# cloudinary/fuif

Measured on AMD Instinct MI355X. Metric: Mpixels/s decode (4K Squeeze+YCoCg), higher is better.
Workload: dtype int32; 1 GPU; C2: batch of 1024 3840x2160 8-bit photographic YCoCg+Squeeze lossless per GPU; images_per_gpu=1024, distinct_images=16, group_index=FGIX trailer behind each stream: one wavefront per channel group, status_ok_and_replicas_agree=True

## Files before the change

fuif_amd/__init__.py:

```python
import ctypes as C
import os
import subprocess

import numpy as np

_HERE = os.path.dirname(os.path.abspath(__file__))
_LIB_PATH = os.environ.get("FUIF_AMD_LIB") or os.path.join(_HERE, "libfuifgpu.so")
_SOURCES = ["plan.cpp", "index.cpp", "writer.cpp", "maniac_decode.hip", "maniac_encode.hip", "transforms.hip", "capi.hip"]
_lib = None


class FuifGpuError(RuntimeError):
    def __init__(self, code, msg):
        super().__init__("fuifgpu error %d: %s" % (code, msg))
        self.code = code


HIPCC_FLAGS = ["--offload-arch=gfx950", "-O3", "-std=c++17", "-ffp-contract=off", "-Wno-unused-value"]


def build(force=False, verbose=False):
    srcs = [os.path.join(_HERE, "csrc", s) for s in _SOURCES]
    deps = srcs + [os.path.join(_HERE, "csrc", h) for h in ("fuifgpu_internal.h", "maniac_decode.h", "maniac_encode.h", "transforms.h", "squeeze_arith.h")]
    deps.append(os.path.join(_HERE, "..", "include", "fuifgpu.h"))
# ... 20 lines not shown
    return out


class ImageInfo(C.Structure):
    _fields_ = [("w", C.c_int32), ("h", C.c_int32), ("bit_depth", C.c_int32), ("maxval", C.c_int32),
                ("nb_channels", C.c_int32), ("colormodel", C.c_int32), ("max_properties", C.c_int32),
                ("nb_frames", C.c_int32), ("nb_transforms", C.c_int32), ("nb_coded_channels", C.c_int32),
                ("nb_output_channels", C.c_int32), ("nb_ops", C.c_int32), ("responsive_offsets", C.c_int32 * 5),
                ("data_start", C.c_int32), ("coef_elems", C.c_int64), ("out_elems", C.c_int64),
                ("tmp_elems", C.c_int64), ("signature", C.c_uint64)]


class ChannelDesc(C.Structure):
    _fields_ = [("w", C.c_int32), ("h", C.c_int32), ("hshift", C.c_int32), ("vshift", C.c_int32),
                ("hcshift", C.c_int32), ("vcshift", C.c_int32), ("component", C.c_int32), ("reserved", C.c_int32),
                ("offset", C.c_int64)]


class EncodeOptions(C.Structure):
    _fields_ = [("struct_size", C.c_uint32), ("ycocg", C.c_int32), ("squeeze", C.c_int32), ("max_properties", C.c_int32), ("tree_mode", C.c_int32),
                ("max_tree_nodes", C.c_int32), ("emit_index", C.c_int32), ("split_bits", C.c_int32), ("gpu_forward", C.c_int32), ("gpu_entropy", C.c_int32)]


class LossyOptions(C.Structure):
    _fields_ = [("struct_size", C.c_uint32), ("quality", C.c_float), ("chroma_quality", C.c_float)]


class PaletteOptions(C.Structure):
    _fields_ = [("struct_size", C.c_uint32), ("palette_colors", C.c_int32), ("compact_post_percent", C.c_float), ("compact_pre_percent", C.c_float)]


def make_palette_options(palette_colors=0, compact_post=0.0, compact_pre=0.0):
    if not palette_colors and not compact_post and not compact_pre:
        return None
    return PaletteOptions(C.sizeof(PaletteOptions), int(palette_colors), float(compact_post), float(compact_pre))


def make_lossy_options(quality=None, chroma_quality=None):
    return LossyOptions(C.sizeof(LossyOptions), 100.0 if quality is None else float(quality), 101.0 if chroma_quality is None else float(chroma_quality))


def make_encode_options(*fields):
    return EncodeOptions(C.sizeof(EncodeOptions), *fields)


ABI_SYMBOLS = [
    "fuifgpu_strerror", "fuifgpu_last_error", "fuifgpu_abi_version", "fuifgpu_plan_create", "fuifgpu_plan_destroy",
    "fuifgpu_plan_info", "fuifgpu_plan_coded_channel", "fuifgpu_plan_output_channel", "fuifgpu_plan_transform",
    "fuifgpu_build_chance_table", "fuifgpu_batch_create", "fuifgpu_batch_create_sibling", "fuifgpu_dev_mem_info", "fuifgpu_encode_images", "fuifgpu_batch_destroy", "fuifgpu_batch_upload",
    "fuifgpu_batch_decode", "fuifgpu_batch_undo_transforms", "fuifgpu_batch_sync", "fuifgpu_batch_status",
    "fuifgpu_batch_create_streaming", "fuifgpu_batch_undo_transforms_to", "fuifgpu_batch_channel_meta", "fuifgpu_batch_coef_ptr", "fuifgpu_batch_out_ptr", "fuifgpu_batch_download_coef",
    "fuifgpu_batch_download_out", "fuifgpu_batch_last_timing", "fuifgpu_batch_profile", "fuifgpu_batch_tile_log", "fuifgpu_batch_sched_stats", "fuifgpu_inv_hsqueeze", "fuifgpu_inv_vsqueeze",
    "fuifgpu_inv_ycocg", "fuifgpu_inv_ycbcr", "fuifgpu_inv_quantize", "fuifgpu_idct8x8", "fuifgpu_upsample", "fuifgpu_inv_palette", "fuifgpu_inv_approximate", "fuifgpu_inv_match", "fuifgpu_fwd_ycocg", "fuifgpu_fwd_hsqueeze", "fuifgpu_fwd_vsqueeze", "fuifgpu_fwd_quantize", "fuifgpu_encode_image", "fuifgpu_encode_channels", "fuifgpu_free_blob",
    "fuifgpu_index_parse", "fuifgpu_index_append", "fuifgpu_batch_group_index", "fuifgpu_batch_set_group_parallel",
    "fuifgpu_plan_packed_bytes", "fuifgpu_batch_pack_out", "fuifgpu_batch_download_packed",
    "fuifgpu_dev_alloc", "fuifgpu_dev_free", "fuifgpu_dev_upload", "fuifgpu_dev_download",
    "fuifgpu_encode_image_lossy", "fuifgpu_encode_images_lossy", "fuifgpu_quantization_constant",
    "fuifgpu_encode_images_device", "fuifgpu_channel_stats", "fuifgpu_encode_plane_traffic",
    "fuifgpu_encode_image_ex", "fuifgpu_encode_images_ex", "fuifgpu_fwd_palette",
    "fuifgpu_plane_checksums", "fuifgpu_device_count", "fuifgpu_set_device", "fuifgpu_get_device", "fuifgpu_batch_device", "fuifgpu_peer_copy", "fuifgpu_batch_set_in_flight",
]


def _preload_hip_runtime():
    import importlib.util
    try:
        spec = importlib.util.find_spec("torch")
    except (ImportError, ValueError):
        spec = None
    if spec is None or not spec.submodule_search_locations:
        return
    cand = os.path.join(list(spec.submodule_search_locations)[0], "lib", "libamdhip64.so")
    if os.path.exists(cand):
        try:
            global _hip_runtime
            _hip_runtime = C.CDLL(cand, mode=C.RTLD_GLOBAL)
        except OSError:
            pass


_hip_runtime = None


def hip_runtime():
    lib()
    return _hip_runtime if _hip_runtime is not None else C.CDLL("libamdhip64.so")


def lib():
    global _lib
    if _lib is not None:
        return _lib
    if not os.path.exists(_LIB_PATH):
        raise ImportError("fuif_amd/libfuifgpu.so is missing: run `python -c 'import __graft_entry__ as g; g.build()'` "
                          "(hipcc --offload-arch=gfx950). There is no CPU fallback.")
    _preload_hip_runtime()
    L = C.CDLL(_LIB_PATH)
    vp, i32p, u8p = C.c_void_p, C.POINTER(C.c_int32), C.POINTER(C.c_uint8)
    L.fuifgpu_strerror.restype = C.c_char_p; L.fuifgpu_strerror.argtypes = [C.c_int]
    L.fuifgpu_last_error.restype = C.c_char_p; L.fuifgpu_last_error.argtypes = []
    L.fuifgpu_abi_version.restype = C.c_int
    L.fuifgpu_plan_create.argtypes = [C.c_char_p, C.c_size_t, C.POINTER(vp)]
    L.fuifgpu_plan_destroy.argtypes = [vp]; L.fuifgpu_plan_destroy.restype = None
    L.fuifgpu_plan_info.argtypes = [vp, C.POINTER(ImageInfo)]
    L.fuifgpu_plan_coded_channel.argtypes = [vp, C.c_int, C.POINTER(ChannelDesc)]
    L.fuifgpu_plan_output_channel.argtypes = [vp, C.c_int, C.POINTER(ChannelDesc)]
    L.fuifgpu_plan_transform.argtypes = [vp, C.c_int, i32p, vp, C.c_int, i32p]
    L.fuifgpu_build_chance_table.argtypes = [vp, C.c_uint32, C.c_int]; L.fuifgpu_build_chance_table.restype = None
    L.fuifgpu_batch_create.argtypes = [vp, C.c_int, C.c_size_t, vp, vp, C.c_int, C.POINTER(vp)]
    L.fuifgpu_batch_create_sibling.argtypes = [vp, C.c_size_t, C.POINTER(vp)]
    L.fuifgpu_batch_destroy.argtypes = [vp]; L.fuifgpu_batch_destroy.restype = None
    L.fuifgpu_batch_upload.argtypes = [vp, C.POINTER(C.c_char_p), C.POINTER(C.c_size_t), C.c_int, C.c_int, vp]
    L.fuifgpu_batch_decode.argtypes = [vp, vp]
    L.fuifgpu_batch_undo_transforms.argtypes = [vp, vp]
    L.fuifgpu_batch_create_streaming.argtypes = [vp, C.c_int, C.c_size_t, C.c_int, C.POINTER(vp)]
    L.fuifgpu_batch_undo_transforms_to.argtypes = [vp, C.c_int, C.c_int, vp, vp]
    L.fuifgpu_batch_sync.argtypes = [vp, vp]
    L.fuifgpu_batch_status.argtypes = [vp, vp, vp]
    L.fuifgpu_batch_channel_meta.argtypes = [vp, C.c_int, vp]
    L.fuifgpu_batch_coef_ptr.argtypes = [vp, C.c_int]; L.fuifgpu_batch_coef_ptr.restype = vp
    L.fuifgpu_batch_out_ptr.argtypes = [vp, C.c_int]; L.fuifgpu_batch_out_ptr.restype = vp
    L.fuifgpu_batch_download_coef.argtypes = [vp, C.c_int, vp, vp]
    L.fuifgpu_batch_download_out.argtypes = [vp, C.c_int, vp, vp]
    L.fuifgpu_device_count.argtypes = [C.POINTER(C.c_int)]
    L.fuifgpu_set_device.argtypes = [C.c_int]
    L.fuifgpu_get_device.argtypes = [C.POINTER(C.c_int)]
    L.fuifgpu_batch_device.argtypes = [vp, C.POINTER(C.c_int)]
    L.fuifgpu_peer_copy.argtypes = [vp, C.c_int, vp, C.c_int, C.c_size_t, vp]
    L.fuifgpu_plane_checksums.argtypes = [vp, C.c_int64, C.c_int64, C.c_int, vp, vp]
    L.fuifgpu_batch_last_timing.argtypes = [vp, C.POINTER(C.c_float), C.POINTER(C.c_float)]
    L.fuifgpu_batch_profile.argtypes = [vp, vp]
    L.fuifgpu_batch_tile_log.argtypes = [vp, vp, C.c_int, C.POINTER(C.c_int)]
    L.fuifgpu_batch_sched_stats.argtypes = [vp, vp]
    L.fuifgpu_inv_hsqueeze.argtypes = [vp, C.c_int, vp, C.c_int, C.c_int, vp, C.c_int, C.c_int64, C.c_int64, C.c_int64, vp]
    L.fuifgpu_inv_vsqueeze.argtypes = [vp, C.c_int, vp, C.c_int, C.c_int, vp, C.c_int, C.c_int64, C.c_int64, C.c_int64, vp]
    L.fuifgpu_inv_ycocg.argtypes = [vp, vp, vp, C.c_int, C.c_int, C.c_int, C.c_int, C.c_int, C.c_int, vp]
    L.fuifgpu_inv_ycbcr.argtypes = [vp, vp, vp, C.c_int, C.c_int, C.c_int, C.c_int, C.c_int, C.c_int, C.c_int, vp]
    L.fuifgpu_inv_quantize.argtypes = [vp, C.c_int64, C.c_int, vp]
    L.fuifgpu_idct8x8.argtypes = [C.POINTER(vp), C.c_int, C.c_int, vp, C.c_int, vp]
    L.fuifgpu_upsample.argtypes = [vp, C.c_int, C.c_int, C.c_int, C.c_int, vp, vp]
    L.fuifgpu_inv_palette.argtypes = [vp, C.c_int, C.c_int, vp, C.c_int, vp, vp]
    L.fuifgpu_inv_approximate.argtypes = [vp, vp, C.c_int64, C.c_int, vp]
    L.fuifgpu_inv_match.argtypes = [vp, C.c_int, C.c_int, C.POINTER(vp), C.c_int, C.c_int, C.c_int, C.c_int, C.c_int, vp]
    L.fuifgpu_fwd_ycocg.argtypes = [vp, vp, vp, C.c_int, C.c_int, vp]
    L.fuifgpu_fwd_hsqueeze.argtypes = [vp, C.c_int, C.c_int, vp, vp, vp]
    L.fuifgpu_fwd_vsqueeze.argtypes = [vp, C.c_int, C.c_int, vp, vp, vp]
    L.fuifgpu_dev_alloc.argtypes = [C.c_size_t]; L.fuifgpu_dev_alloc.restype = vp
    L.fuifgpu_dev_free.argtypes = [vp]; L.fuifgpu_dev_free.restype = None
    L.fuifgpu_dev_upload.argtypes = [vp, vp, C.c_size_t]
    L.fuifgpu_dev_download.argtypes = [vp, vp, C.c_size_t]
    L.fuifgpu_fwd_quantize.argtypes = [vp, C.c_int64, C.c_int, vp, vp]
    L.fuifgpu_encode_image_lossy.argtypes = [vp, C.c_int, C.c_int, C.c_int, C.c_int, C.POINTER(EncodeOptions), C.POINTER(LossyOptions), C.POINTER(vp), C.POINTER(C.c_size_t)]
    L.fuifgpu_encode_images_lossy.argtypes = [C.POINTER(vp), C.c_int, C.c_int, C.c_int, C.c_int, C.c_int, C.POINTER(EncodeOptions), C.POINTER(LossyOptions), C.POINTER(vp), C.POINTER(C.c_size_t)]
    L.fuifgpu_encode_images_device.argtypes = [C.POINTER(vp), C.c_int, C.c_int, C.c_int, C.c_int, C.c_int, C.POINTER(EncodeOptions), C.POINTER(LossyOptions), C.POINTER(vp), C.POINTER(C.c_size_t)]
    L.fuifgpu_channel_stats.argtypes = [vp, C.c_int64, vp, vp]
    L.fuifgpu_encode_image_ex.argtypes = [vp, C.c_int, C.c_int, C.c_int, C.c_int, C.POINTER(EncodeOptions), C.POINTER(LossyOptions), C.POINTER(PaletteOptions), C.POINTER(vp), C.POINTER(C.c_size_t)]
    L.fuifgpu_encode_images_ex.argtypes = [C.POINTER(vp), C.c_int, C.c_int, C.c_int, C.c_int, C.c_int, C.c_int, C.POINTER(EncodeOptions), C.POINTER(LossyOptions), C.POINTER(PaletteOptions), C.POINTER(vp), C.POINTER(C.c_size_t)]
    L.fuifgpu_fwd_palette.argtypes = [C.POINTER(vp), C.c_int, C.c_int64, C.c_int, vp, vp, C.POINTER(C.c_int), vp]
    L.fuifgpu_encode_plane_traffic.argtypes = [C.POINTER(C.c_uint64), C.POINTER(C.c_uint64)]
    L.fuifgpu_quantization_constant.argtypes = [C.c_float, C.c_float, C.c_int, C.c_int, C.c_int]
    L.fuifgpu_encode_image.argtypes = [vp, C.c_int, C.c_int, C.c_int, C.c_int, C.POINTER(EncodeOptions), C.POINTER(vp), C.POINTER(C.c_size_t)]
    L.fuifgpu_encode_images.argtypes = [C.POINTER(vp), C.c_int, C.c_int, C.c_int, C.c_int, C.c_int, C.POINTER(EncodeOptions), C.POINTER(vp), C.POINTER(C.c_size_t)]
    L.fuifgpu_free_blob.argtypes = [vp]; L.fuifgpu_free_blob.restype = None
    L.fuifgpu_index_parse.argtypes = [C.c_char_p, C.c_size_t, vp, vp, C.c_int, C.POINTER(C.c_int)]
    L.fuifgpu_index_append.argtypes = [C.c_char_p, C.c_size_t, vp, vp, C.c_int, C.POINTER(vp), C.POINTER(C.c_size_t)]
    L.fuifgpu_batch_group_index.argtypes = [vp, C.c_int, vp, vp, C.c_int, C.POINTER(C.c_int)]
    L.fuifgpu_batch_set_group_parallel.argtypes = [vp, C.c_int]
    L.fuifgpu_batch_set_in_flight.argtypes = [vp, C.c_int]
    L.fuifgpu_plan_packed_bytes.argtypes = [vp, C.c_int]; L.fuifgpu_plan_packed_bytes.restype = C.c_size_t
    L.fuifgpu_batch_pack_out.argtypes = [vp, C.c_int, C.c_int, C.c_int, vp, vp]
    L.fuifgpu_batch_download_packed.argtypes = [vp, C.c_int, C.c_int, vp, vp]
    _lib = L
    return L


def _check(code):
    if code != 0:
        L = lib()
        msg = L.fuifgpu_strerror(code).decode()
        last = L.fuifgpu_last_error().decode()
        raise FuifGpuError(code, msg + (" (" + last + ")" if last else ""))


class Plan:

    def __init__(self, blob):
        L = lib()
        self._h = C.c_void_p()
        _check(L.fuifgpu_plan_create(bytes(blob[:65536]) if len(blob) > 65536 else bytes(blob), min(len(blob), 65536), C.byref(self._h)))
        self.info = ImageInfo()
        _check(L.fuifgpu_plan_info(self._h, C.byref(self.info)))

    def __del__(self):
        if getattr(self, "_h", None) and _lib is not None:
            _lib.fuifgpu_plan_destroy(self._h)
            self._h = None

    def _channels(self, fn, n):
        out = []
        for i in range(n):
            d = ChannelDesc()
            _check(fn(self._h, i, C.byref(d)))
            out.append({k: int(getattr(d, k)) for k, _ in ChannelDesc._fields_ if k != "reserved"})
        return out

    @property
    def coded_channels(self):
        return self._channels(lib().fuifgpu_plan_coded_channel, self.info.nb_coded_channels)

    @property
    def output_channels(self):
        return self._channels(lib().fuifgpu_plan_output_channel, self.info.nb_output_channels)

    @property
    def transforms(self):
        out = []
        for i in range(self.info.nb_transforms):
# ... 247 lines not shown
        ptrs = [int(p) if p else 0 for p in planes]
        if w is None or h is None or nch is None:
            raise FuifGpuError(4, "encode_images_device: w, h and nch go with a list of device pointers")
    n = len(ptrs)
    opt = make_encode_options(int(ycocg), int(squeeze), max_properties, tree_mode, max_tree_nodes, int(index), int(split_bits), 1, 1)
    lossy = None if quality is None and chroma_quality is None else C.byref(make_lossy_options(quality, chroma_quality))
    arr = (C.c_void_p * max(n, 1))(*ptrs)
    outs = (C.c_void_p * max(n, 1))()
    sizes = (C.c_size_t * max(n, 1))()
    pal = make_palette_options(palette_colors, compact_post, compact_pre)
    if pal is not None:
        _check(lib().fuifgpu_encode_images_ex(arr, 1, n, int(w), int(h), int(nch), bit_depth, C.byref(opt), lossy, C.byref(pal), outs, sizes))
    else:
        _check(lib().fuifgpu_encode_images_device(arr, n, int(w), int(h), int(nch), bit_depth, C.byref(opt), lossy, outs, sizes))
    blobs = []
    for k in range(n):
        blobs.append(C.string_at(outs[k], sizes[k]))
        lib().fuifgpu_free_blob(C.c_void_p(outs[k]))
    return blobs


def channel_stats(plane_device_ptr, n_samples, stats_device_ptr, stream=None):
    _check(lib().fuifgpu_channel_stats(plane_device_ptr, int(n_samples), stats_device_ptr, stream))


def encode_plane_traffic():
    a, b = C.c_uint64(0), C.c_uint64(0)
    _check(lib().fuifgpu_encode_plane_traffic(C.byref(a), C.byref(b)))
    return int(a.value), int(b.value)


def quantization_constant(quality, chroma_quality=None, squeeze=True, chroma_table=False, shift=0):
    q = lib().fuifgpu_quantization_constant(float(quality), 101.0 if chroma_quality is None else float(chroma_quality), int(bool(squeeze)), int(bool(chroma_table)), int(shift))
    if q < 1:
        _check(-q)
    return q


def fwd_quantize(plane_device_ptr, n_samples, q, minmax_device_ptr=None, stream=None):
    _check(lib().fuifgpu_fwd_quantize(plane_device_ptr, int(n_samples), int(q), minmax_device_ptr, stream))


def fwd_palette(plane_device_ptrs, n_samples, max_colors, index_device_ptr, stream=None):
    nb = len(plane_device_ptrs)
    ptrs = (C.c_void_p * max(nb, 1))(*[int(p) if p else 0 for p in plane_device_ptrs])
    pal = np.zeros((max(nb, 1), max(int(max_colors), 1)), dtype=np.int32)
    count = C.c_int(0)
    _check(lib().fuifgpu_fwd_palette(ptrs, nb, int(n_samples), int(max_colors), index_device_ptr, pal.ctypes.data, C.byref(count), stream))
    if count.value < 0:
        return None
    return np.ascontiguousarray(pal[:nb, :count.value])


def index_parse(blob):
    fc, st, n = np.zeros(4096, np.int32), np.zeros(4096, np.uint32), C.c_int(0)
    _check(lib().fuifgpu_index_parse(blob, len(blob), fc.ctypes.data, st.ctypes.data, 4096, C.byref(n)))
    return [(int(fc[i]), int(st[i])) for i in range(min(n.value, 4096))]


def index_append(blob, groups):
    fc = np.array([g[0] for g in groups], np.int32)
    st = np.array([g[1] for g in groups], np.uint32)
    out, n = C.c_void_p(), C.c_size_t(0)
    _check(lib().fuifgpu_index_append(blob, len(blob), fc.ctypes.data, st.ctypes.data, len(groups), C.byref(out), C.byref(n)))
    res = C.string_at(out.value, n.value)
    lib().fuifgpu_free_blob(out)
    return res


def add_group_index(blobs, hbm_budget_bytes=200 << 30):
    out = list(blobs)
    todo = []
    for i, b in enumerate(blobs):
        try:
            if not index_parse(b):
                Plan(b)
                todo.append(i)
        except FuifGpuError:
            pass
    for sig, (plan, idx) in group_by_signature([blobs[i] for i in todo]).items():
        idx = [todo[k] for k in idx]
        per = 2 * plan.info.coef_elems + 19 * (1 << 20) + max(len(blobs[i]) for i in idx)
        chunk = max(1, min(len(idx), int(hbm_budget_bytes // per), 65535))
        for c0 in range(0, len(idx), chunk):
            part = idx[c0:c0 + chunk]
            sub = [blobs[i] for i in part]
            batch = Batch(plan, len(sub), sum(len(b) for b in sub) + 4096 * len(sub), streaming=True, tmp_images=1)
            try:
                batch.upload(sub)
                batch.decode()
                batch.sync()
                st, _ = batch.status()
                for k, i in enumerate(part):
                    if st[k] == 0:
                        out[i] = index_append(blobs[i], batch.group_index(k))
            finally:
                batch.close()
    return out


def group_by_signature(blobs):
    groups = {}
    for i, b in enumerate(blobs):
        p = Plan(b)
        sig = int(p.info.signature)
        if sig not in groups:
            groups[sig] = (p, [])
        groups[sig][1].append(i)
    return groups

# ... 28 lines not shown
```

fuif_amd/csrc/capi.hip:

```cpp
#include <hip/hip_runtime.h>

#include <algorithm>
#include <cstdio>
#include <cstring>
#include <string>
#include <vector>

#include "../../include/fuifgpu.h"
#include "fuifgpu_internal.h"
#include "maniac_decode.h"
#include "transforms.h"

using namespace fuifgpu;

struct fuifgpu_plan {
    Plan plan;
};

struct fuifgpu_batch {
    Plan plan;
    int device = 0;
    int n = 0;
    int n_loaded = 0;
    uint8_t *d_blobs = nullptr;
    size_t blob_cap = 0;
    StreamJob *d_jobs = nullptr;
    ChannelGeom *d_geom = nullptr;
    ChannelMeta *d_meta = nullptr;
    int32_t *d_status = nullptr;
    uint32_t *d_consumed = nullptr;
    uint16_t *d_tables = nullptr;
    uint8_t *d_scratch = nullptr;
    size_t scratch_stride = 0, bfs_off = 0, leaves_off = 0, stack_off = 0, queue_off = 0, subtree_off = 0;
    int scratch_waves = 0;
    int max_waves[3] = {0, 0, 0};
    int in_flight = 1;
    int n_waves = 0, cfg = 1;
    bool group_parallel = true;
    Tile *d_tiles = nullptr;
    int tiles_cap = 0, n_tiles = 0;
    uint32_t *d_progress = nullptr, *d_group_start = nullptr;
    uint32_t *d_sched = nullptr, *d_layout = nullptr;
    size_t sched_words = 0, layout_cap = 0;
    int sched = 0, n_queues = 1, waves_per_simd = 4;
    uint8_t *d_ctx = nullptr;
    size_t ctx_bytes = 0;
    uint32_t ctx_units_per_queue = 0;
    int max_nodes = kMaxNodes;
    coef_t *d_coef = nullptr;
    int32_t *d_out = nullptr, *d_tmp = nullptr;
    int32_t *d_coef32 = nullptr;
    bool own_coef = false, own_out = false;
    int tmp_images = 0;
    PlaneRef *d_list = nullptr;
    int64_t *d_widen = nullptr;
    unsigned long long *d_prof = nullptr, *d_tile_log = nullptr;
    int tile_log_cap = 0; bool want_tile_log = false;
    uint8_t *h_blobs = nullptr;
    std::vector<StreamJob> jobs;
    hipEvent_t ev[4] = {nullptr, nullptr, nullptr, nullptr};
    bool decode_timed = false, transform_timed = false;
    bool no_out = false;
    std::vector<char> undone;
    bool coef_consumed = false;
    fuifgpu_batch *share = nullptr;
    std::vector<fuifgpu_batch *> siblings;
    bool orphan = false;
};
static inline const fuifgpu_batch *launch_res(const fuifgpu_batch *b) { return b->share ? b->share : b; }

static thread_local std::string g_last_error;

static int hip_fail(hipError_t e, const char *what) {
    g_last_error = std::string(what) + ": " + hipGetErrorString(e);
    return FUIFGPU_E_HIP;
}
static int fail_msg(int code, const char *what) {
    g_last_error = what;
    return code;
}
#define HIPCHK(call)                                      \
    do {                                                  \
        hipError_t e__ = (call);                          \
        if (e__ != hipSuccess) return hip_fail(e__, #call); \
    } while (0)

template <typename T, typename N>
static int grow(T *&ptr, N &cap, N need, size_t unit = sizeof(T), bool sync_first = false) {
    if (need <= cap) return FUIFGPU_OK;
    if (sync_first) HIPCHK(hipDeviceSynchronize());
    hipFree(ptr); ptr = nullptr; cap = 0;
    HIPCHK(hipMalloc((void **)&ptr, unit * (size_t)need));
    cap = need;
    return FUIFGPU_OK;
// ... 211 lines not shown
    }
    *out = p;
    return FUIFGPU_OK;
}
void fuifgpu_plan_destroy(fuifgpu_plan *plan) { delete plan; }

int fuifgpu_plan_info(const fuifgpu_plan *plan, fuifgpu_image_info *info) {
    if (!plan || !info) return FUIFGPU_E_ARG;
    const Plan &p = plan->plan;
    memset(info, 0, sizeof(*info));
    info->w = p.w; info->h = p.h; info->bit_depth = p.bit_depth; info->maxval = p.maxval; info->nb_channels = p.nb_channels;
    info->colormodel = p.colormodel; info->max_properties = p.max_properties; info->nb_frames = p.nb_frames;
    info->nb_transforms = (int)p.transforms.size(); info->nb_coded_channels = (int)p.coded.size();
    info->nb_output_channels = (int)p.outputs.size(); info->nb_ops = (int)p.ops.size();
    for (int s = 0; s < 5; s++) info->responsive_offsets[s] = p.responsive_offsets[s];
    info->data_start = (int)p.data_start;
    info->coef_elems = p.coef_elems; info->out_elems = p.out_elems; info->tmp_elems = p.tmp_elems;
    info->signature = p.signature;
    return FUIFGPU_OK;
}
int fuifgpu_plan_coded_channel(const fuifgpu_plan *plan, int index, fuifgpu_channel_desc *d) {
    if (!plan || !d || index < 0 || index >= (int)plan->plan.coded.size()) return FUIFGPU_E_ARG;
    const ChannelGeom &g = plan->plan.coded[index];
    d->w = g.w; d->h = g.h; d->hshift = g.hshift; d->vshift = g.vshift; d->hcshift = g.hcshift; d->vcshift = g.vcshift;
    d->component = g.component; d->reserved = 0; d->offset = g.coef_off;
    return FUIFGPU_OK;
}
int fuifgpu_plan_output_channel(const fuifgpu_plan *plan, int index, fuifgpu_channel_desc *d) {
    if (!plan || !d || index < 0 || index >= (int)plan->plan.outputs.size()) return FUIFGPU_E_ARG;
    const OutputChannel &o = plan->plan.outputs[index];
    d->w = o.plane.w; d->h = o.plane.h; d->hshift = o.hshift; d->vshift = o.vshift; d->hcshift = o.hcshift; d->vcshift = o.vcshift;
    d->component = o.component; d->reserved = 0; d->offset = o.plane.off;
    return FUIFGPU_OK;
}
int fuifgpu_plan_transform(const fuifgpu_plan *plan, int index, int32_t *id, int32_t *params_out, int cap, int32_t *nparams) {
    if (!plan || index < 0 || index >= (int)plan->plan.transforms.size()) return FUIFGPU_E_ARG;
    const TransformDesc &t = plan->plan.transforms[index];
    if (id) *id = t.id;
    if (nparams) *nparams = (int)t.params.size();
    if (params_out) for (int i = 0; i < (int)t.params.size() && i < cap; i++) params_out[i] = t.params[i];
    return FUIFGPU_OK;
}

void fuifgpu_batch_destroy(fuifgpu_batch *b) {
    if (!b) return;
    ON_BATCH_DEVICE(b);
    for (fuifgpu_batch *s : b->siblings) { s->share = nullptr; s->orphan = true; s->n_loaded = 0; s->d_coef = nullptr; s->d_out = nullptr; }
    if (b->share) {
        auto &v = b->share->siblings;
        v.erase(std::remove(v.begin(), v.end(), b), v.end());
    }
    hipFree(b->d_blobs); hipFree(b->d_jobs); hipFree(b->d_geom); hipFree(b->d_meta); hipFree(b->d_status); hipFree(b->d_consumed);
    hipFree(b->d_tables); hipFree(b->d_scratch); hipFree(b->d_tmp); hipFree(b->d_coef32); hipFree(b->d_list); hipFree(b->d_widen); hipFree(b->d_prof); hipFree(b->d_tile_log);
    hipFree(b->d_tiles); hipFree(b->d_progress); hipFree(b->d_group_start); hipFree(b->d_sched); hipFree(b->d_layout); hipFree(b->d_ctx);
    if (b->own_coef) hipFree(b->d_coef);
    if (b->own_out) hipFree(b->d_out);
    if (b->h_blobs) hipHostFree(b->h_blobs);
    for (int i = 0; i < 4; i++) if (b->ev[i]) hipEventDestroy(b->ev[i]);
    delete b;
}

static int32_t *const kNoOutSlab = reinterpret_cast<int32_t *>(~(uintptr_t)0);
static int batch_create_impl(const Plan &plan_in, int n_images, size_t blob_capacity_bytes, coef_t *coef_ext, int32_t *out_ext,
                             int tmp_images, fuifgpu_batch *share, fuifgpu_batch **out) {
    if (!out || n_images < 1 || n_images > 65535) return FUIFGPU_E_ARG;
    *out = nullptr;
    int ndev = 0;
    if (hipGetDeviceCount(&ndev) != hipSuccess || ndev < 1) {
        g_last_error = "no HIP device visible: libfuifgpu has no CPU fallback";
        return FUIFGPU_E_HIP;
    }
    fuifgpu_batch *b = new fuifgpu_batch();
    if (share) b->device = share->device;
    else if (hipGetDevice(&b->device) != hipSuccess) b->device = 0;
    b->plan = plan_in;
    b->n = n_images;
    b->share = share;
    const Plan &p = b->plan;
    const int nch = (int)p.coded.size();
    b->blob_cap = blob_capacity_bytes + (size_t)n_images * 32 + 1024;
#define CHK(call)                                                        \
    do {                                                                 \
        hipError_t e__ = (call);                                         \
        if (e__ != hipSuccess) { int rc = hip_fail(e__, #call); fuifgpu_batch_destroy(b); return rc; } \
    } while (0)
    CHK(hipMalloc((void **)&b->d_blobs, b->blob_cap));
    CHK(hipMalloc((void **)&b->d_jobs, sizeof(StreamJob) * n_images));
    CHK(hipMalloc((void **)&b->d_geom, sizeof(ChannelGeom) * std::max(nch, 1)));
    CHK(hipMemcpy(b->d_geom, p.coded.data(), sizeof(ChannelGeom) * nch, hipMemcpyHostToDevice));
    CHK(hipMalloc((void **)&b->d_meta, sizeof(ChannelMeta) * (size_t)n_images * std::max(nch, 1)));
    CHK(hipMalloc((void **)&b->d_status, sizeof(int32_t) * n_images));
    CHK(hipMalloc((void **)&b->d_consumed, sizeof(uint32_t) * n_images));
    {
        std::vector<uint16_t> tables(16384);
        build_chance_table(tables.data(), 0xFFFFFFFFu / 19, 2);
        build_chance_table(tables.data() + 8192, 0x0d000000u, 6);
        CHK(hipMalloc((void **)&b->d_tables, tables.size() * 2));
        CHK(hipMemcpy(b->d_tables, tables.data(), tables.size() * 2, hipMemcpyHostToDevice));
    }
    b->scratch_stride = maniac_scratch_bytes(b->max_nodes, &b->bfs_off, &b->leaves_off, &b->stack_off, &b->queue_off, &b->subtree_off);
    b->max_waves[0] = maniac_max_waves(0);
    b->max_waves[1] = maniac_max_waves(1, &b->waves_per_simd);
    b->max_waves[2] = maniac_max_waves(2);
    if (const char *e = getenv("FUIFGPU_IN_FLIGHT")) b->in_flight = std::max(1, atoi(e));
    if (b->max_waves[0] < 1 || b->max_waves[1] < 1 || b->max_waves[2] < 1) { g_last_error = "cannot query the device occupancy of the entropy kernel"; fuifgpu_batch_destroy(b); return FUIFGPU_E_HIP; }
    CHK(hipMalloc((void **)&b->d_progress, sizeof(uint32_t) * (size_t)n_images * std::max(nch, 1)));
    CHK(hipMalloc((void **)&b->d_group_start, sizeof(uint32_t) * (size_t)n_images * std::max(nch, 1)));
    if (coef_ext) b->d_coef = coef_ext;
    else { CHK(hipMalloc((void **)&b->d_coef, sizeof(coef_t) * (size_t)std::max<int64_t>(p.coef_elems, 1) * n_images)); b->own_coef = true; }
    if (out_ext == kNoOutSlab) { b->d_out = nullptr; b->no_out = true; }
    else if (out_ext) b->d_out = out_ext;
    else { CHK(hipMalloc((void **)&b->d_out, sizeof(int32_t) * (size_t)std::max<int64_t>(p.out_elems, 1) * n_images)); b->own_out = true; }
    if (tmp_images <= 0) {
        int64_t per = (std::max<int64_t>(p.tmp_elems, 1) + std::max<int64_t>(p.coef_elems, 1)) * 4;
        tmp_images = (int)std::max<int64_t>(1, std::min<int64_t>(n_images, (12LL << 30) / per));
    }
    b->tmp_images = std::min(tmp_images, n_images);
    if (!share) {
        CHK(hipMalloc((void **)&b->d_tmp, sizeof(int32_t) * (size_t)std::max<int64_t>(p.tmp_elems, 1) * b->tmp_images));
        CHK(hipMalloc((void **)&b->d_coef32, sizeof(int32_t) * (size_t)std::max<int64_t>(p.coef_elems, 1) * b->tmp_images));
    }
    if (!p.idct_src.empty()) {
        CHK(hipMalloc((void **)&b->d_list, sizeof(PlaneRef) * p.idct_src.size()));
        CHK(hipMemcpy(b->d_list, p.idct_src.data(), sizeof(PlaneRef) * p.idct_src.size(), hipMemcpyHostToDevice));
    }
    if (!p.widen.empty()) {
        CHK(hipMalloc((void **)&b->d_widen, sizeof(int64_t) * p.widen.size()));
        CHK(hipMemcpy(b->d_widen, p.widen.data(), sizeof(int64_t) * p.widen.size(), hipMemcpyHostToDevice));
    }
    CHK(hipMalloc((void **)&b->d_prof, sizeof(unsigned long long) * 8 * n_images));
    CHK(hipMemset(b->d_prof, 0, sizeof(unsigned long long) * 8 * n_images));
    for (int i = 0; i < 4; i++) CHK(hipEventCreate(&b->ev[i]));
#undef CHK
    *out = b;
    return FUIFGPU_OK;
}

int fuifgpu_batch_create(const fuifgpu_plan *plan, int n_images, size_t blob_capacity_bytes, int16_t *coef_ext, int32_t *out_ext,
                         int tmp_images, fuifgpu_batch **out) {
    if (!plan) return FUIFGPU_E_ARG;
    return batch_create_impl(plan->plan, n_images, blob_capacity_bytes, coef_ext, out_ext, tmp_images, nullptr, out);
}

static size_t ctx_arena_budget(const fuifgpu_batch *b, size_t images) {
    size_t per_image = 16u << 20;
    if (const char *e = getenv("FUIFGPU_CTX_MB")) per_image = (size_t)std::max(1, atoi(e)) << 20;
    if (const char *e = getenv("FUIFGPU_CTX_KB")) per_image = (size_t)std::max(0, atoi(e)) << 10;
    size_t want = per_image * images, free_b = 0, total_b = 0;
    if (hipMemGetInfo(&free_b, &total_b) == hipSuccess) want = std::min(want, (free_b + b->ctx_bytes) / 2);
    return want / 256 * 256;
}
static uint32_t ctx_units_per_queue(size_t arena_bytes, int n_queues) {
    const size_t q = (size_t)std::max(n_queues, 1);
    return (uint32_t)std::min(arena_bytes / q / 256, (size_t)0xFFFFFF00u / q);
}
static int freeze_launch_resources(fuifgpu_batch *b) {
    const int64_t cap = std::max(std::max(b->max_waves[0], b->max_waves[1]), b->max_waves[2]);
    const int waves = (int)std::max<int64_t>(1, std::min<int64_t>(cap, (int64_t)b->n * std::max<int64_t>((int64_t)b->plan.coded.size(), 1)));
    OKCHK(grow(b->d_scratch, b->scratch_waves, waves, b->scratch_stride, true));
    return grow(b->d_ctx, b->ctx_bytes, ctx_arena_budget(b, (size_t)b->n), 1, true);
}

int fuifgpu_batch_create_streaming(const fuifgpu_plan *plan, int n_images, size_t blob_capacity_bytes, int tmp_images, fuifgpu_batch **out) {
    if (!plan) return FUIFGPU_E_ARG;
    return batch_create_impl(plan->plan, n_images, blob_capacity_bytes, nullptr, kNoOutSlab, tmp_images, nullptr, out);
}

int fuifgpu_batch_create_sibling(fuifgpu_batch *primary, size_t blob_capacity_bytes, fuifgpu_batch **out) {
    if (!primary || primary->share || primary->no_out) return FUIFGPU_E_ARG;
    ON_BATCH_DEVICE(primary);
    if (primary->siblings.empty()) OKCHK(freeze_launch_resources(primary));
    const int rc = batch_create_impl(primary->plan, primary->n, blob_capacity_bytes, primary->d_coef, primary->d_out, primary->tmp_images, primary, out);
    if (rc == FUIFGPU_OK) primary->siblings.push_back(*out);
    return rc;
}

static int stage_streams(fuifgpu_batch *b, const uint8_t *const *blobs, const size_t *sizes, int n_images, int preview, hipStream_t st,
                         std::vector<std::vector<GroupEntry>> &groups, std::vector<int> &group_of) {
    b->jobs.assign(n_images, StreamJob{});
    size_t off = 0;
    Plan tmp;
    std::vector<std::pair<const uint8_t *, int>> seen;
    const int nch = (int)b->plan.coded.size();
    group_of.assign(n_images, -1);
    HIPCHK(hipStreamSynchronize(st));
    for (int i = 0; i < n_images; i++) {
        if (sizes[i] > 0xFFFFFFF0ull) return FUIFGPU_E_ARG;
        int src = -1;
        for (auto &sp : seen) if (sp.first == blobs[i] && b->jobs[sp.second].blob_size == sizes[i]) { src = sp.second; break; }
        size_t padded = (sizes[i] + 15) / 16 * 16 + 16;
        if (off + padded + 256 > b->blob_cap) { g_last_error = "blob capacity exceeded"; return FUIFGPU_E_NOMEM; }
        StreamJob &j = b->jobs[i];
        if (src < 0) {
            int r = parse_and_plan(blobs[i], sizes[i], tmp);
            if (r != FUIFGPU_OK) { g_last_error = tmp.message; return r; }
            if (tmp.signature != b->plan.signature) { g_last_error = "image " + std::to_string(i) + " has a different geometry/transform chain"; return FUIFGPU_E_MISMATCH; }
            std::vector<GroupEntry> idx;
            if (b->group_parallel) parse_index_trailer(blobs[i], sizes[i], tmp.data_start, nch, idx, nullptr);
            if (idx.empty()) idx.push_back(GroupEntry{(uint32_t)tmp.data_start, 0});
            groups.push_back(std::move(idx));
            group_of[i] = (int)groups.size() - 1;
            HIPCHK(hipMemsetAsync(b->d_blobs + off + (padded - 32), 0, 32, st));
            HIPCHK(hipMemcpyAsync(b->d_blobs + off, blobs[i], sizes[i], hipMemcpyHostToDevice, st));
            j.data_start = (uint32_t)tmp.data_start;
            j.limit = preview >= 0 ? (uint32_t)tmp.responsive_offsets[preview] : 0u;
            seen.emplace_back(blobs[i], i);
        } else {
            HIPCHK(hipMemcpyAsync(b->d_blobs + off, b->d_blobs + b->jobs[src].blob_off, padded, hipMemcpyDeviceToDevice, st));
            j.data_start = b->jobs[src].data_start;
            j.limit = b->jobs[src].limit;
            group_of[i] = group_of[src];
        }
        j.blob_off = off; j.blob_size = (uint32_t)sizes[i];
        j.flags = 0;
        off += padded;
    }
    HIPCHK(hipMemcpyAsync(b->d_jobs, b->jobs.data(), sizeof(StreamJob) * n_images, hipMemcpyHostToDevice, st));
    return FUIFGPU_OK;
}

struct WorkList {
    int cfg = 1, n_waves = 0, sched = 0, n_queues = 1;
    std::vector<Tile> tiles;
    std::vector<uint32_t> layout;
};
static WorkList plan_work_list(const Plan &plan, const std::vector<std::vector<GroupEntry>> &groups, const std::vector<int> &group_of, const size_t *sizes,
                               const int *max_waves, int waves_per_simd, int in_flight, bool group_order) {
    WorkList wl;
    const int n_images = (int)group_of.size(), nch = (int)plan.coded.size();
    size_t total_tiles = 0, deepest = 0;
    for (int i = 0; i < n_images; i++) total_tiles += groups[group_of[i]].size();
    for (auto &g : groups) deepest = std::max(deepest, g.size());
    const int wide_cfg = in_flight > 1 ? 0 : 2;
    const bool dense = (int64_t)total_tiles > max_waves[wide_cfg];
    wl.cfg = dense ? 1 : wide_cfg;
    wl.n_waves = (int)std::max<int64_t>(1, std::min<int64_t>((int64_t)total_tiles, max_waves[wl.cfg]));
    std::vector<char> suspendable(groups.size(), 0);
    for (size_t gi = 0; gi < groups.size(); gi++) {
        const std::vector<GroupEntry> &g = groups[gi];
        bool ok = g.size() > 1;
        for (size_t k = 0; k < g.size() && ok; k++) {
            const int first = k == 0 ? 0 : g[k].first_channel, last = k + 1 < g.size() ? g[k + 1].first_channel - 1 : nch - 1;
            int nonempty = 0;
            for (int c = first; c <= last; c++) nonempty += (int64_t)plan.coded[c].w * plan.coded[c].h > 0 ? 1 : 0;
            ok = nonempty <= 1;
        }
        suspendable[gi] = ok ? 1 : 0;
    }
    int64_t image_samples = 0;
    for (int c = 0; c < nch; c++) image_samples += (int64_t)plan.coded[c].w * plan.coded[c].h;
    auto push_tile = [&](int i, size_t k) {
        const std::vector<GroupEntry> &g = groups[group_of[i]];
        if (k >= g.size()) return;
        Tile t;
        t.image = (uint32_t)i;
        t.start = g[k].start;
        t.first_channel = k == 0 ? 0 : g[k].first_channel;
        t.last_channel = k + 1 < g.size() ? g[k + 1].first_channel - 1 : nch - 1;
        t.end = k + 1 < g.size() ? g[k + 1].start : 0u;
        t.flags = suspendable[group_of[i]] ? kTileSuspendable : 0u;
        int64_t mine = 0;
        for (int c = (int)t.first_channel; c <= (int)t.last_channel; c++) mine += (int64_t)plan.coded[c].w * plan.coded[c].h;
        uint32_t cls = 15;
        if (mine > 0) { cls = 0; while (cls < 15 && (mine << (cls + 1)) <= image_samples) cls++; }
        t.flags |= cls << kTileSizeClassShift;
        wl.tiles.push_back(t);
    };
    wl.sched = dense && (int64_t)total_tiles > wl.n_waves && !group_order ? 1 : 0;
    if (!wl.sched) {
        for (size_t k = 0; k < deepest; k++)
            for (int i = 0; i < n_images; i++) push_tile(i, k);
        return wl;
    }
    const int waves_per_cu = (int)kSimdsPerCu * std::max(1, waves_per_simd);
    const int Q = wl.n_queues = std::max(1, std::min(n_images, wl.n_waves / waves_per_cu));
    const QueueLayout L = queue_layout(Q, n_images);
    wl.layout.resize(L.words);
    uint32_t *qib = wl.layout.data() + L.q_img_begin, *qim = wl.layout.data() + L.q_images, *itb = wl.layout.data() + L.img_tile_begin;
    std::vector<int> by_size(n_images);
    for (int i = 0; i < n_images; i++) by_size[i] = i;
    std::stable_sort(by_size.begin(), by_size.end(), [&](int x, int y) { return sizes[x] > sizes[y]; });
    std::vector<std::vector<uint32_t>> dealt(Q);
    for (int k = 0; k < n_images; k++) {
        const int round = k / Q, at = k % Q;
        dealt[(round & 1) ? Q - 1 - at : at].push_back((uint32_t)by_size[k]);
    }
    uint32_t pos = 0;
    for (int q = 0; q < Q; q++) {
        qib[q] = pos;
        std::sort(dealt[q].begin(), dealt[q].end());
        for (uint32_t i : dealt[q]) qim[pos++] = i;
    }
    qib[Q] = pos;
    for (int i = 0; i < n_images; i++) {
        itb[i] = (uint32_t)wl.tiles.size();
        for (size_t k = 0; k < groups[group_of[i]].size(); k++) push_tile(i, k);
    }
    itb[n_images] = (uint32_t)wl.tiles.size();
    return wl;
}

static int reserve_launch_buffers(fuifgpu_batch *b, int n_images, size_t layout_words) {
    OKCHK(grow(b->d_sched, b->sched_words, sched_layout(n_images, b->n_queues, b->sched ? b->n_tiles : 0)));
    OKCHK(grow(b->d_layout, b->layout_cap, layout_words));
    OKCHK(grow(b->d_tiles, b->tiles_cap, b->n_tiles));
    if (b->sched && !b->share) {
        const size_t images_per_queue = ((size_t)n_images + b->n_queues - 1) / b->n_queues;
        size_t arena = ctx_arena_budget(b, images_per_queue * (size_t)b->n_queues);
        if (!b->siblings.empty()) arena = std::min(arena, b->ctx_bytes);
        b->ctx_units_per_queue = ctx_units_per_queue(arena, b->n_queues);
        OKCHK(grow(b->d_ctx, b->ctx_bytes, (size_t)b->ctx_units_per_queue * 256 * (size_t)b->n_queues));
    }
    if (b->share) {
        if (b->n_waves > b->share->scratch_waves) { g_last_error = "sibling batch: more wavefronts than the primary's decoder scratch was sized for"; return FUIFGPU_E_ARG; }
        return FUIFGPU_OK;
    }
    if (b->n_waves > b->scratch_waves && !b->siblings.empty()) { g_last_error = "primary batch with siblings: decoder scratch cannot grow (internal sizing error)"; return FUIFGPU_E_ARG; }
    return grow(b->d_scratch, b->scratch_waves, b->n_waves, b->scratch_stride);
}

int fuifgpu_batch_upload(fuifgpu_batch *b, const uint8_t *const *blobs, const size_t *sizes, int n_images, int preview, void *stream) {
    ON_BATCH_DEVICE(b);
    if (!b || !blobs || !sizes || n_images < 1 || n_images > b->n || preview < -1 || preview > 4) return FUIFGPU_E_ARG;
    if (b->orphan) { g_last_error = "sibling batch: its primary has been destroyed"; return FUIFGPU_E_ARG; }
    hipStream_t st = (hipStream_t)stream;
    std::vector<std::vector<GroupEntry>> groups;
    std::vector<int> group_of;
    OKCHK(stage_streams(b, blobs, sizes, n_images, preview, st, groups, group_of));
    const char *ord = getenv("FUIFGPU_TILE_ORDER");
    const WorkList wl = plan_work_list(b->plan, groups, group_of, sizes, b->max_waves, b->waves_per_simd, b->in_flight, ord && !strcmp(ord, "group"));
    b->cfg = wl.cfg; b->n_waves = wl.n_waves; b->sched = wl.sched; b->n_queues = wl.n_queues; b->n_tiles = (int)wl.tiles.size();
    OKCHK(reserve_launch_buffers(b, n_images, wl.layout.size()));
    if (!wl.layout.empty()) HIPCHK(hipMemcpyAsync(b->d_layout, wl.layout.data(), wl.layout.size() * 4, hipMemcpyHostToDevice, st));
    if (b->n_tiles) HIPCHK(hipMemcpyAsync(b->d_tiles, wl.tiles.data(), sizeof(Tile) * (size_t)b->n_tiles, hipMemcpyHostToDevice, st));
    HIPCHK(hipStreamSynchronize(st));
    b->n_loaded = n_images;
    if (getenv("FUIFGPU_VERBOSE"))
        fprintf(stderr, "fuifgpu: %d images, %d tiles, %s configuration, %d persistent wavefronts (%d per SIMD), %d queues, context scheduler %s\n", n_images, b->n_tiles,
                b->cfg == 1 ? "dense" : b->cfg == 2 ? "wide" : "wide (two batches in flight)", b->n_waves, b->waves_per_simd, b->n_queues, b->sched ? "on" : "off");
    return FUIFGPU_OK;
}

int fuifgpu_batch_decode(fuifgpu_batch *b, void *stream) {
    ON_BATCH_DEVICE(b);
    if (!b || b->n_loaded < 1) return FUIFGPU_E_ARG;
    hipStream_t st = (hipStream_t)stream;
    const int nch = (int)b->plan.coded.size();
    HIPCHK(hipMemsetAsync(b->d_meta, 0, sizeof(ChannelMeta) * (size_t)b->n_loaded * std::max(nch, 1), st));
    HIPCHK(hipMemsetAsync(b->d_progress, 0, sizeof(uint32_t) * (size_t)b->n_loaded * std::max(nch, 1), st));
    HIPCHK(hipMemsetAsync(b->d_group_start, 0, sizeof(uint32_t) * (size_t)b->n_loaded * std::max(nch, 1), st));
    HIPCHK(hipMemsetAsync(b->d_sched, 0, b->sched_words * 4, st));
    HIPCHK(hipMemsetAsync(b->d_status, 0, sizeof(int32_t) * b->n_loaded, st));
    HIPCHK(hipMemsetAsync(b->d_consumed, 0, sizeof(uint32_t) * b->n_loaded, st));
    HIPCHK(hipMemsetAsync(b->d_prof, 0, sizeof(unsigned long long) * 8 * b->n_loaded, st));
    DecodeParams P{};
    P.blobs = b->d_blobs; P.jobs = b->d_jobs; P.n_images = b->n_loaded; P.n_channels = nch; P.geom = b->d_geom;
    P.coef = b->d_coef; P.coef_stride = b->plan.coef_elems; P.meta = b->d_meta; P.status = b->d_status; P.consumed = b->d_consumed;
    const fuifgpu_batch *r = launch_res(b);
    P.tables = b->d_tables; P.scratch = r->d_scratch; P.scratch_stride = b->scratch_stride; P.bfs_off = b->bfs_off; P.leaves_off = b->leaves_off;
    P.stack_off = b->stack_off; P.queue_off = b->queue_off; P.subtree_off = b->subtree_off; P.max_properties = b->plan.max_properties; P.max_nodes = b->max_nodes; P.max_super = maniac_max_supernodes(b->max_nodes); P.prof = b->d_prof;
    if (b->want_tile_log) OKCHK(grow(b->d_tile_log, b->tile_log_cap, b->n_tiles, sizeof(unsigned long long) * 4));
    P.tile_log = b->want_tile_log ? b->d_tile_log : nullptr;
    if (P.tile_log) HIPCHK(hipMemsetAsync(b->d_tile_log, 0, sizeof(unsigned long long) * 4 * (size_t)b->n_tiles, st));
    P.tiles = b->d_tiles; P.n_tiles = b->n_tiles; P.sched = b->sched; P.n_queues = b->n_queues;
    sched_layout(b->n_loaded, b->n_queues, b->sched ? b->n_tiles : 0, b->d_sched, &P);
    P.yield_slack = 4;
    if (const char *e = getenv("FUIFGPU_YIELD_SLACK")) P.yield_slack = (uint32_t)std::max(0, atoi(e));
    P.prio_base = kDefaultPrioBase;
    if (const char *e = getenv("FUIFGPU_PRIO_BASE")) P.prio_base = atoi(e);
    P.long_per_simd = 3;
    if (const char *e = getenv("FUIFGPU_LONG_PER_SIMD")) P.long_per_simd = std::max(0, atoi(e));
    const QueueLayout L = queue_layout(b->n_queues, b->n_loaded);
    P.q_img_begin = b->d_layout + L.q_img_begin; P.q_images = b->d_layout + L.q_images; P.img_tile_begin = b->d_layout + L.img_tile_begin;
    P.ctx_scratch = r->d_ctx;
    P.ctx_units_per_queue = b->share ? ctx_units_per_queue(r->ctx_bytes, b->n_queues) : b->ctx_units_per_queue;
    P.progress = b->d_progress; P.group_start = b->d_group_start;
    HIPCHK(hipEventRecord(b->ev[0], st));
    launch_maniac_decode(P, b->n_waves, b->cfg, b->n_tiles > b->n_loaded ? 1 : 0, st);
    HIPCHK(hipGetLastError());
    HIPCHK(hipEventRecord(b->ev[1], st));
    b->decode_timed = true;
    b->coef_consumed = false;
    b->undone.clear();
    return FUIFGPU_OK;
}

static int undo_range(fuifgpu_batch *b, int first, int count, int32_t *out_base, hipStream_t st) {
    const Plan &p = b->plan;
    const int nch = (int)p.coded.size();
    const fuifgpu_batch *r = launch_res(b);
    for (int i0 = first; i0 < first + count; i0 += r->tmp_images) {
        const int cnt = std::min(r->tmp_images, first + count - i0);
        Bases bases{};
        {
            int64_t widest = 0;
            for (size_t k = 1; k < p.widen.size(); k += 2) widest = std::max(widest, p.widen[k]);
            launch_widen_planes(b->d_coef + (int64_t)i0 * p.coef_elems, r->d_coef32, p.coef_elems, b->d_widen, (int)(p.widen.size() / 2), widest, cnt, st);
        }
        bases.base[BUF_COEF] = r->d_coef32; bases.stride[BUF_COEF] = p.coef_elems;
        bases.c16 = b->d_coef + (int64_t)i0 * p.coef_elems;
        bases.base[BUF_OUT] = out_base + (int64_t)(i0 - first) * p.out_elems; bases.stride[BUF_OUT] = p.out_elems;
        bases.base[BUF_TMP] = r->d_tmp; bases.stride[BUF_TMP] = p.tmp_elems;
        for (const Op &op : p.ops) launch_op(op, bases, b->d_list, b->d_meta, nch, i0, cnt, st, b->d_status);
    }
    HIPCHK(hipGetLastError());
    return FUIFGPU_OK;
}

int fuifgpu_batch_undo_transforms_to(fuifgpu_batch *b, int first_image, int n_images, int32_t *out_device, void *stream) {
    ON_BATCH_DEVICE(b);
    if (!b || b->orphan || !out_device || first_image < 0 || n_images < 1 || first_image + n_images > b->n_loaded) return FUIFGPU_E_ARG;
    if (b->coef_consumed) { g_last_error = "fuifgpu_batch_undo_transforms_to: fuifgpu_batch_undo_transforms already ran on this decode"; return FUIFGPU_E_ARG; }
    if ((int)b->undone.size() != b->n_loaded) b->undone.assign((size_t)b->n_loaded, 0);
    for (int i = first_image; i < first_image + n_images; i++)
        if (b->undone[i]) { g_last_error = "fuifgpu_batch_undo_transforms_to: an image of the range has been through the inverse transforms already (once per decode)"; return FUIFGPU_E_ARG; }
    hipStream_t st = (hipStream_t)stream;
    HIPCHK(hipEventRecord(b->ev[2], st));
    const int rc = undo_range(b, first_image, n_images, out_device, st);
    if (rc != FUIFGPU_OK) return rc;
    for (int i = first_image; i < first_image + n_images; i++) b->undone[i] = 1;
    HIPCHK(hipEventRecord(b->ev[3], st));
    b->transform_timed = true;
    return FUIFGPU_OK;
}

int fuifgpu_batch_undo_transforms(fuifgpu_batch *b, void *stream) {
    ON_BATCH_DEVICE(b);
    if (!b || b->n_loaded < 1) return FUIFGPU_E_ARG;
    if (b->no_out) { g_last_error = "fuifgpu_batch_undo_transforms: a streaming batch has no output slab (fuifgpu_batch_undo_transforms_to)"; return FUIFGPU_E_ARG; }
// ... 142 lines not shown
    return FUIFGPU_OK;
}

int fuifgpu_plane_checksums(const int32_t *planes_device, int64_t elems_per_image, int64_t image_stride, int n_images, uint64_t *sums_device, void *stream) {
    if (!planes_device || !sums_device || elems_per_image < 0 || image_stride < elems_per_image || n_images < 1 || n_images > 65535 ||
        ((uintptr_t)planes_device & 15) || (image_stride & 3)) return FUIFGPU_E_ARG;
    launch_plane_checksums(planes_device, elems_per_image, image_stride, n_images, (unsigned long long *)sums_device, (hipStream_t)stream);
    HIPCHK(hipGetLastError());
    return FUIFGPU_OK;
}

int fuifgpu_batch_last_timing(fuifgpu_batch *b, float *decode_ms, float *transform_ms) {
    ON_BATCH_DEVICE(b);
    if (!b) return FUIFGPU_E_ARG;
    if (decode_ms) {
        *decode_ms = -1.f;
        if (b->decode_timed) { HIPCHK(hipEventSynchronize(b->ev[1])); HIPCHK(hipEventElapsedTime(decode_ms, b->ev[0], b->ev[1])); }
    }
    if (transform_ms) {
        *transform_ms = -1.f;
        if (b->transform_timed) { HIPCHK(hipEventSynchronize(b->ev[3])); HIPCHK(hipEventElapsedTime(transform_ms, b->ev[2], b->ev[3])); }
    }
    return FUIFGPU_OK;
}

int fuifgpu_batch_profile(fuifgpu_batch *b, uint64_t *out8_per_image) {
    ON_BATCH_DEVICE(b);
    if (!b || !out8_per_image || b->n_loaded < 1) return FUIFGPU_E_ARG;
    HIPCHK(hipDeviceSynchronize());
    HIPCHK(hipMemcpy(out8_per_image, b->d_prof, sizeof(unsigned long long) * 8 * b->n_loaded, hipMemcpyDeviceToHost));
    return FUIFGPU_OK;
}

int fuifgpu_batch_tile_log(fuifgpu_batch *b, uint64_t *out4_per_tile, int cap, int *n_tiles) {
    ON_BATCH_DEVICE(b);
    if (!b || !n_tiles) return FUIFGPU_E_ARG;
#if !defined(FUIF_STATS) && !defined(FUIF_PROF) && !defined(FUIF_TILELOG)
    *n_tiles = 0;
    g_last_error = "fuifgpu_batch_tile_log: this build of libfuifgpu carries no scheduler statistics (build with -DFUIF_STATS)";
    return FUIFGPU_E_UNSUPPORTED;
#endif
    const bool had = b->want_tile_log && b->d_tile_log && b->tile_log_cap >= b->n_tiles;
    b->want_tile_log = true;
    *n_tiles = had ? b->n_tiles : 0;
    if (!had || !out4_per_tile) return FUIFGPU_OK;
    HIPCHK(hipDeviceSynchronize());
    HIPCHK(hipMemcpy(out4_per_tile, b->d_tile_log, sizeof(unsigned long long) * 4 * (size_t)std::min(cap, b->n_tiles), hipMemcpyDeviceToHost));
    return FUIFGPU_OK;
}

int fuifgpu_batch_sched_stats(fuifgpu_batch *b, uint64_t *out8) {
    ON_BATCH_DEVICE(b);
    if (!b || !out8 || !b->d_sched) return FUIFGPU_E_ARG;
#ifndef FUIF_STATS
    g_last_error = "fuifgpu_batch_sched_stats: this build of libfuifgpu carries no scheduler statistics (build with -DFUIF_STATS)";
    return FUIFGPU_E_UNSUPPORTED;
#endif
    HIPCHK(hipDeviceSynchronize());
    HIPCHK(hipMemcpy(out8, (const uint8_t *)b->d_sched + offsetof(SchedHeader, sched_stats), sizeof(SchedHeader::sched_stats), hipMemcpyDeviceToHost));
    return FUIFGPU_OK;
}

int fuifgpu_device_count(int *n_devices) {
    if (!n_devices) return FUIFGPU_E_ARG;
    int n = 0;
    if (hipGetDeviceCount(&n) != hipSuccess || n < 1) { *n_devices = 0; g_last_error = "no HIP device visible: libfuifgpu has no CPU fallback"; return FUIFGPU_E_HIP; }
    *n_devices = n;
    return FUIFGPU_OK;
}
int fuifgpu_set_device(int device) {
    int n = 0;
    const int rc = fuifgpu_device_count(&n);
    if (rc != FUIFGPU_OK) return rc;
    if (device < 0 || device >= n) { g_last_error = "fuifgpu_set_device: no such device"; return FUIFGPU_E_ARG; }
    HIPCHK(hipSetDevice(device));
    return FUIFGPU_OK;
}
int fuifgpu_get_device(int *device) {
    if (!device) return FUIFGPU_E_ARG;
    HIPCHK(hipGetDevice(device));
    return FUIFGPU_OK;
}
int fuifgpu_batch_device(const fuifgpu_batch *b, int *device) {
    if (!b || !device) return FUIFGPU_E_ARG;
    *device = b->device;
    return FUIFGPU_OK;
}
int fuifgpu_peer_copy(void *dst_device_ptr, int dst_device, const void *src_device_ptr, int src_device, size_t bytes, void *stream) {
    if ((!dst_device_ptr || !src_device_ptr) && bytes) return FUIFGPU_E_ARG;
    int n = 0;
    const int rc = fuifgpu_device_count(&n);
    if (rc != FUIFGPU_OK) return rc;
    if (dst_device < 0 || dst_device >= n || src_device < 0 || src_device >= n) { g_last_error = "fuifgpu_peer_copy: no such device"; return FUIFGPU_E_ARG; }
    if (!bytes) return FUIFGPU_OK;
    if (dst_device == src_device) {
        DeviceGuard g(dst_device);
        HIPCHK(hipMemcpyAsync(dst_device_ptr, src_device_ptr, bytes, hipMemcpyDeviceToDevice, (hipStream_t)stream));
        return FUIFGPU_OK;
    }
    {
        DeviceGuard g(dst_device);
        int can = 0;
        if (hipDeviceCanAccessPeer(&can, dst_device, src_device) == hipSuccess && can) {
            const hipError_t e = hipDeviceEnablePeerAccess(src_device, 0);
            if (e != hipSuccess && e != hipErrorPeerAccessAlreadyEnabled) (void)hipGetLastError();
            else (void)hipGetLastError();
        }
    }
    HIPCHK(hipMemcpyPeerAsync(dst_device_ptr, dst_device, src_device_ptr, src_device, bytes, (hipStream_t)stream));
    return FUIFGPU_OK;
// ... 268 lines not shown
```

fuif_amd/csrc/fuifgpu_internal.h:

```cpp
#pragma once
#include <cstddef>
#include <cstdint>
#include <string>
#include <vector>

namespace fuifgpu {

enum : int {
    TR_YCBCR = 0, TR_YCOCG = 1, TR_SUBSAMPLE = 3, TR_DCT = 4, TR_QUANTIZE = 5,
    TR_PALETTE = 6, TR_SQUEEZE = 7, TR_2DMATCH = 8, TR_PERMUTE = 9, TR_APPROXIMATE = 10
};

constexpr int kMaxBitDepth = 15;
constexpr int kNonRefProps = 13;
constexpr int kMaxProps = 64;
constexpr int kMaxRefs = 25;
constexpr int kFastRefs = 9;
constexpr int kMaxNodes = 65535;
constexpr int kLeafStride = 32;
constexpr int kTreeStackDepth = 2048;
constexpr int kPlaneAlign = 128;
using coef_t = int16_t;

enum : int {
    ST_OK = 0,
    ST_TRUNCATED = 1,
    ST_CORRUPT = 2,
    ST_UNSUPPORTED = 4,
    ST_STALLED = 8,
};

struct ChannelGeom {
    int32_t w, h;
    int32_t hshift, vshift, hcshift, vcshift;
    int32_t component;
    int32_t ctor_data;
    int64_t coef_off;
};

struct ChannelMeta {
    int32_t minval, maxval, q, decoded;
};

struct StreamJob {
    uint64_t blob_off;
    uint32_t blob_size;
    uint32_t data_start;
    uint32_t limit;
    uint32_t flags;
};

struct Tile {
    uint32_t image;
    uint32_t start;
    int32_t first_channel, last_channel;
    uint32_t end;
    uint32_t flags;
};
constexpr uint32_t kTileSuspendable = 1u;
constexpr uint32_t kTileSizeClassShift = 4;
constexpr int kDefaultPrioBase = 2;

enum : int { BUF_COEF = 0, BUF_OUT = 1, BUF_TMP = 2,
              BUF_COEF16Q = 3 };
struct PlaneRef {
    int32_t buf;
    int32_t w, h;
    int32_t qsrc;
    int64_t off;
};
enum : int {
    OP_HSQUEEZE = 1, OP_VSQUEEZE = 2, OP_YCOCG = 3, OP_YCBCR = 4, OP_QUANT = 5, OP_IDCT = 6,
    OP_UPSAMPLE = 7, OP_COPY_CLAMP = 8, OP_CLAMP = 9,
    OP_PALETTE = 10,
    OP_APPROX = 11,
    OP_MATCH = 12,
    OP_MATCH_INIT = 13,
    OP_MATCH_JUMP = 14,
    OP_MATCH_APPLY = 15,
    OP_PERMUTE = 16,
    OP_HSQ2_YCOCG = 17,
    OP_UPS2_YCBCR = 18
};
struct Op {
    int32_t kind;
    int32_t clamp_out;
    int32_t lo, hi;
    int32_t p0, p1;
    PlaneRef src[3];
    PlaneRef dst[3];
    int32_t idct_first;
    int32_t pad;
    PlaneRef ext[1];
    int32_t r16;
    int32_t pad2;
};

struct TransformDesc {
    int id;
    std::vector<int> params;
};

struct OutputChannel {
    PlaneRef plane;
    int32_t hshift, vshift, hcshift, vcshift, component;
};

struct Plan {
    int w = 0, h = 0, bit_depth = 0, maxval = 0, minval = 0;
    int nb_channels = 0, colormodel = 0, nb_frames = 1, max_properties = 0;
    int responsive_offsets[5] = {0, 0, 0, 0, 0};
    size_t data_start = 0;
    std::vector<TransformDesc> transforms;
    std::vector<ChannelGeom> coded;
    int64_t coef_elems = 0;
    std::vector<Op> ops;
    std::vector<PlaneRef> idct_src;
    std::vector<int64_t> widen;
    std::vector<OutputChannel> outputs;
    int64_t out_elems = 0, tmp_elems = 0;
    uint64_t signature = 0;
    int error = 0;
    std::string message;
};

struct QuantChan {
    int32_t *plane;
    int64_t n;
    int32_t q, slot;
    int32_t first_block, n_blocks;
};
int fwd_quantize_channels_gpu(const QuantChan *channels, int n_channels, int32_t *minmax_host);

struct StatsRec {
    const int32_t *plane;
    int64_t n;
    int32_t first_block, n_blocks;
};
int channel_stats_gpu(const StatsRec *recs, int n_recs, int32_t *stats_host);
int fwd_palette_gpu(const int32_t *const *planes_device, int nb, int64_t n, int max_colors, int32_t *index_device, std::vector<int32_t> &rows,
                    int *n_colors, void *stream = nullptr);
int dev_copy(void *dst_device, const void *src_device, size_t bytes);

struct GroupEntry {
    uint32_t start;
    int32_t first_channel;
};
void build_index_trailer(const std::vector<GroupEntry> &groups, std::vector<uint8_t> &out);
bool parse_index_trailer(const uint8_t *blob, size_t n, size_t data_start, int nch, std::vector<GroupEntry> &groups, size_t *stream_end);

int parse_and_plan(const uint8_t *blob, size_t n, Plan &plan);
void build_chance_table(uint16_t *table8192, uint32_t alpha, int cut);

}
```

fuif_amd/csrc/index.cpp:

```cpp
#include <cstdlib>
#include <cstring>

#include "../../include/fuifgpu.h"
#include "fuifgpu_internal.h"

namespace fuifgpu {

namespace {
void put_varint(std::vector<uint8_t> &b, uint64_t v) {
    uint8_t tmp[10];
    int n = 0;
    tmp[n++] = (uint8_t)(v & 127);
    v >>= 7;
    while (v) { tmp[n++] = (uint8_t)(128 | (v & 127)); v >>= 7; }
    while (n) b.push_back(tmp[--n]);
}
bool get_varint(const uint8_t *p, size_t n, size_t &pos, uint64_t &out) {
    uint64_t r = 0;
    for (int k = 0; k < 10; k++) {
        if (pos >= n) return false;
        const uint8_t c = p[pos++];
        if (r >> 57) return false;
        r = (r << 7) | (c & 127);
        if (c < 128) { out = r; return true; }
    }
    return false;
}
}

void build_index_trailer(const std::vector<GroupEntry> &groups, std::vector<uint8_t> &out) {
    std::vector<uint8_t> payload;
    put_varint(payload, 1);
    put_varint(payload, groups.size());
    uint32_t pc = 0, ps = 0;
    for (const GroupEntry &g : groups) {
        put_varint(payload, (uint32_t)g.first_channel - pc);
        put_varint(payload, g.start - ps);
        pc = (uint32_t)g.first_channel; ps = g.start;
    }
    out = payload;
    const uint32_t len = (uint32_t)payload.size();
    for (int k = 0; k < 4; k++) out.push_back((uint8_t)(len >> (8 * k)));
    out.push_back('F'); out.push_back('G'); out.push_back('I'); out.push_back('X');
}

bool parse_index_trailer(const uint8_t *blob, size_t n, size_t data_start, int nch, std::vector<GroupEntry> &groups, size_t *stream_end) {
    groups.clear();
    if (n < 8 + 3 || memcmp(blob + n - 4, "FGIX", 4) != 0) return false;
    uint32_t len = 0;
    for (int k = 0; k < 4; k++) len |= (uint32_t)blob[n - 8 + k] << (8 * k);
    if (len < 2 || (size_t)len + 8 > n) return false;
    const size_t begin = n - 8 - len;
    const uint8_t *p = blob + begin;
    size_t pos = 0;
    uint64_t version = 0, count = 0;
    if (!get_varint(p, len, pos, version) || version != 1) return false;
    if (!get_varint(p, len, pos, count) || count < 1 || count > (uint64_t)nch) return false;
    uint64_t c = 0, s = 0;
    for (uint64_t g = 0; g < count; g++) {
        uint64_t dc = 0, ds = 0;
        if (!get_varint(p, len, pos, dc) || !get_varint(p, len, pos, ds)) return false;
        if (g && (dc == 0 || ds == 0)) return false;
        if (dc >= (uint64_t)nch || ds >= begin) return false;
        c += dc; s += ds;
        if (c >= (uint64_t)nch || s >= begin) return false;
        groups.push_back(GroupEntry{(uint32_t)s, (int32_t)c});
    }
    if (pos != len || groups[0].start != data_start) { groups.clear(); return false; }
    if (stream_end) *stream_end = begin;
    return true;
}

}

using namespace fuifgpu;

extern "C" {

int fuifgpu_index_parse(const uint8_t *blob, size_t size, int32_t *first_channel, uint32_t *start, int cap, int *n_groups) {
    if (!blob || !n_groups) return FUIFGPU_E_ARG;
    *n_groups = 0;
    Plan plan;
    int r = parse_and_plan(blob, size, plan);
    if (r != FUIFGPU_OK) return r;
    std::vector<GroupEntry> groups;
    if (!parse_index_trailer(blob, size, plan.data_start, (int)plan.coded.size(), groups, nullptr)) return FUIFGPU_OK;
    *n_groups = (int)groups.size();
    for (int g = 0; g < (int)groups.size() && g < cap; g++) {
        if (first_channel) first_channel[g] = groups[g].first_channel;
        if (start) start[g] = groups[g].start;
    }
    return FUIFGPU_OK;
}

int fuifgpu_index_append(const uint8_t *blob, size_t size, const int32_t *first_channel, const uint32_t *start, int n_groups,
                         uint8_t **blob_out, size_t *size_out) {
    if (!blob || !first_channel || !start || n_groups < 1 || !blob_out || !size_out) return FUIFGPU_E_ARG;
    Plan plan;
    int r = parse_and_plan(blob, size, plan);
    if (r != FUIFGPU_OK) return r;
    std::vector<GroupEntry> old;
    size_t stream_end = size;
    parse_index_trailer(blob, size, plan.data_start, (int)plan.coded.size(), old, &stream_end);
    std::vector<GroupEntry> groups(n_groups);
    for (int g = 0; g < n_groups; g++) {
        groups[g] = GroupEntry{start[g], first_channel[g]};
        const bool ascending = g == 0 || (first_channel[g] > first_channel[g - 1] && start[g] > start[g - 1]);
        if (!ascending || first_channel[g] < 0 || first_channel[g] >= (int)plan.coded.size() || start[g] >= stream_end) return FUIFGPU_E_ARG;
    }
    if (groups[0].start != plan.data_start) return FUIFGPU_E_ARG;
    std::vector<uint8_t> trailer;
    build_index_trailer(groups, trailer);
    uint8_t *out = (uint8_t *)malloc(stream_end + trailer.size());
    if (!out) return FUIFGPU_E_NOMEM;
    memcpy(out, blob, stream_end);
    memcpy(out + stream_end, trailer.data(), trailer.size());
    *blob_out = out;
    *size_out = stream_end + trailer.size();
    return FUIFGPU_OK;
}

}
```

fuif_amd/csrc/maniac_decode.h:

```cpp
#pragma once
#include <hip/hip_runtime.h>

#include <cstddef>

#include "fuifgpu_internal.h"

namespace fuifgpu {

enum : uint32_t { TS_NEW = 0, TS_READY = 1, TS_RUNNING = 2, TS_DONE = 3 };
struct TileRec {
    uint32_t state;
    uint32_t wait_chan, wait_val;
    uint32_t y;
    uint32_t range, low, pos;
    uint32_t flags;
    uint32_t ctx, ctx_leaves;
    uint32_t tree_size, n_super, cur_leaf;
    uint32_t t_first_lo, t_first_hi, run_ticks;
    uint32_t pin;
    uint32_t foreign;
    uint32_t pad;
    uint32_t owner;
};

struct DecodeParams {
    const uint8_t *blobs;
    const StreamJob *jobs;
    int32_t n_images;
    int32_t n_channels;
    const ChannelGeom *geom;
    coef_t *coef;
    int64_t coef_stride;
    ChannelMeta *meta;
    int32_t *status;
    uint32_t *consumed;
    const uint16_t *tables;
    const Tile *tiles;
    int32_t n_tiles;
    int32_t sched;
    int32_t prio_base;
    uint32_t yield_slack;
    int32_t n_queues;
    uint32_t *q_head;
    const uint32_t *q_img_begin;
    const uint32_t *q_images;
    const uint32_t *img_tile_begin;
    uint32_t *img_next;
    uint32_t *img_done;
    uint32_t *q_turn;
    uint32_t *done_total;
    uint32_t *started_total;
    uint32_t *heartbeat;
    uint32_t *cu_alive;
    uint32_t *cu_live;
    uint32_t *cu_foreign;
    uint32_t *simd_long;
    int32_t long_per_simd;
    TileRec *tile_rec;
    uint8_t *ctx_scratch;
    uint32_t ctx_units_per_queue;
    unsigned long long *ctx_used;
    unsigned long long *sched_stats;
    uint32_t *simd_claim;
    uint32_t *progress;
    uint32_t *group_start;
    uint8_t *scratch;
    size_t scratch_stride, bfs_off, leaves_off, stack_off, queue_off, subtree_off;
    int32_t max_properties;
    int32_t max_nodes;
    int32_t max_super;
    unsigned long long *prof;
    unsigned long long *tile_log;
};

constexpr uint32_t kCuKeys = 4096;
constexpr uint32_t kSimdsPerCu = 4;
constexpr uint32_t kSchedStatWords = 8;
struct SchedHeader {
    uint32_t q_head, done_total;
    unsigned long long sched_stats[kSchedStatWords];
    uint32_t started_total, heartbeat;
    unsigned long long ctx_used, pad;
};
static_assert(sizeof(SchedHeader) == 96, "the scheduler header is 24 words");
static_assert(offsetof(SchedHeader, sched_stats) % 8 == 0 && offsetof(SchedHeader, ctx_used) % 8 == 0, "64-bit atomics");
inline size_t sched_layout(int n_images, int n_queues, int n_tile_recs, uint32_t *base = nullptr, DecodeParams *P = nullptr) {
    DecodeParams count_only;
    if (!P) { P = &count_only; base = nullptr; }
    size_t w = sizeof(SchedHeader) / 4;
    auto take = [&](size_t n) { uint32_t *p = base ? base + w : nullptr; w += n; return p; };
    P->simd_claim = take(2 * kCuKeys + 1); P->cu_alive = take(kCuKeys); P->cu_live = take(kCuKeys); P->cu_foreign = take(kCuKeys);
    P->simd_long = take(kSimdsPerCu * kCuKeys); P->img_next = take(n_images); P->img_done = take(n_images); P->q_turn = take(n_queues);
    P->tile_rec = reinterpret_cast<TileRec *>(take((size_t)n_tile_recs * (sizeof(TileRec) / 4)));
    if (SchedHeader *h = reinterpret_cast<SchedHeader *>(base)) {
        P->q_head = &h->q_head; P->done_total = &h->done_total; P->sched_stats = h->sched_stats;
        P->started_total = &h->started_total; P->heartbeat = &h->heartbeat; P->ctx_used = &h->ctx_used;
    }
    return w;
}
struct QueueLayout { size_t q_img_begin, q_images, img_tile_begin, words; };
inline QueueLayout queue_layout(size_t n_queues, size_t n_images) { return {0, n_queues + 1, n_queues + 1 + n_images, n_queues + 1 + 2 * n_images + 1}; }

int maniac_max_supernodes(int max_nodes);
size_t maniac_scratch_bytes(int max_nodes, size_t *bfs_off, size_t *leaves_off, size_t *stack_off, size_t *queue_off, size_t *subtree_off);
int maniac_max_waves(int config, int *per_simd = nullptr);
void launch_maniac_decode(const DecodeParams &P, int n_waves, int config, int hand_off, hipStream_t stream);

}
```

fuif_amd/csrc/maniac_decode.hip:

```cpp
#include <hip/hip_runtime.h>

#include <type_traits>

#include "fuifgpu_internal.h"
#include "maniac_decode.h"

namespace fuifgpu {

namespace {

#define DEV __device__ __forceinline__

#ifdef FUIF_PROF_BY_CHANNEL
#define PROF_ROW first_c
#else
#define PROF_ROW img
#endif
#ifdef FUIF_PROF
#define PROF_DECL unsigned long long prof_t0 = 0, prof_acc[8] = {0, 0, 0, 0, 0, 0, 0, 0}
#define PROF_START() prof_t0 = __builtin_readcyclecounter()
#define PROF_LAP(k) do { unsigned long long t__ = __builtin_readcyclecounter(); prof_acc[k] += t__ - prof_t0; prof_t0 = t__; } while (0)
#else
#define PROF_DECL
#define PROF_START()
// ... 667 lines not shown
                uint32_t v = 0;
                while ((v = ld_agent(&P.simd_claim[2 * key + 1])) == 0u) __builtin_amdgcn_s_sleep(2);
                idx = v - 1u;
            }
        }
        home_q = (int)(rflu(idx) % (uint32_t)n_queues);
    }
    constexpr uint32_t kNoWork = 0xFFFFFFFFu, kResume = 0x80000000u;
    const uint32_t my_pin = (uint32_t)blockIdx.x + 1u;
    uint32_t pinned_tix = kNoWork;
    uint32_t my_turn = (uint32_t)blockIdx.x;
    auto scan_queue = [&](int q, bool fresh_ok, bool resume_ok, bool patient) -> uint32_t {
        const uint32_t ib = P.q_img_begin[q], ie = P.q_img_begin[q + 1];
        const bool simd_full = patient && P.long_per_simd > 0 && rflu(ld_agent(&P.simd_long[simd_slot])) >= (uint32_t)P.long_per_simd;
        uint32_t active = 0, k_end = ib;
        for (uint32_t k = ib; k < ie && active < kActiveImages; k++) {
            const uint32_t im = P.q_images[k];
            const uint32_t tb = P.img_tile_begin[im], tn = P.img_tile_begin[im + 1] - tb;
            k_end = k + 1;
            if (rflu(ld_agent(&P.img_done[im])) >= tn) continue;
            active++;
            uint32_t fresh = kNoWork;
            uint32_t peek = lane == 0 ? ld_agent(&P.img_next[im]) : 0u;
            peek = rflu(peek);
            const bool next_is_long = simd_full && peek < tn && ((rflu(P.tiles[tb + peek].flags) >> kTileSizeClassShift) & 15u) <= kLongClass;
            if (fresh_ok && !next_is_long && lane == 0 && peek < tn) {
                const uint32_t n = atomicAdd(&P.img_next[im], 1u);
                if (n < tn) {
                    fresh = tb + n;
                    uint32_t seen = atomicAdd(&P.cu_live[simd_key], 1u);
                    if (q != home_q) { seen |= atomicAdd(&P.cu_foreign[simd_key], 1u); P.tile_rec[fresh].foreign = 1u; }
                    if (seen != 0xFFFFFFFFu) atomicAdd(P.started_total, 1u);
                }
            }
            fresh = rflu(fresh);
            if (fresh != kNoWork) return fresh;
        }
        if (!resume_ok) return kNoWork;
        const uint32_t turn = my_turn++;
        const uint32_t nwin = k_end - ib;
        for (uint32_t j = 0; j < nwin; j++) {
            const uint32_t k = ib + (turn + j) % nwin;
            const uint32_t im = P.q_images[k];
            const uint32_t tb = P.img_tile_begin[im], tn = P.img_tile_begin[im + 1] - tb;
            if (rflu(ld_agent(&P.img_done[im])) >= tn) continue;
            for (uint32_t t0 = (tn - 1u) & ~63u;; t0 -= 64) {
                bool run = false;
                if (t0 + lane < tn) {
                    TileRec *r = P.tile_rec + tb + t0 + lane;
                    if (ld_agent(&r->state) == TS_READY && ld_agent(&r->owner) == simd_key + 1u) {
                        const uint32_t pin = ld_agent(&r->pin);
                        if ((pin == 0u || pin == my_pin) && !(simd_full && (ld_agent(&r->flags) & kRecLong))) {
                            const uint32_t wc = ld_agent(&r->wait_chan), wv = ld_agent(&r->wait_val);
                            run = ld_agent(&P.progress[(size_t)im * nch + wc]) >= wv;
                        }
                    }
                }
                unsigned long long m = __ballot(run);
                while (m) {
                    const int l = 63 - __builtin_clzll(m);
                    uint32_t ok = 0;
                    if (lane == 0) ok = atomicCAS(&P.tile_rec[tb + t0 + l].state, (uint32_t)TS_READY, (uint32_t)TS_RUNNING) == TS_READY ? 1u : 0u;
                    if (rflu(ok)) return (tb + t0 + (uint32_t)l) | kResume;
                    m &= ~(1ull << l);
                }
                if (t0 == 0) break;
            }
        }
        return kNoWork;
    };
    uint32_t idle_rounds = 0, stale_looks = 0, last_beat = 0;
    STATS(unsigned long long st_idle = 0, st_picks = 0, st_yields = 0, st_scan = 0, st_spin = 0, st_noctx = 0, st_busy = 0, st_pick_t = 0, st_t0 = realtime();
          const unsigned long long st_begin = st_t0;)
    for (;;) {
    uint32_t tix = kNoWork;
    bool resumed = false;
#ifndef FUIF_EMU
    __builtin_amdgcn_s_setprio(0);
#endif
    if (!sched) {
        if (lane == 0) { const uint32_t k = atomicAdd(&P.q_head[0], 1u); if (k < (uint32_t)P.n_tiles) tix = k; }
        tix = rflu(tix);
        if (tix == kNoWork) break;
    } else {
        STATS(const unsigned long long sc0 = realtime(); if (st_pick_t) { st_busy += sc0 - st_pick_t; st_pick_t = 0; })
        const bool can_start = pinned_tix == kNoWork;
        const bool patient = idle_rounds < 8u;
        tix = scan_queue(home_q, can_start, true, patient);
        const bool all_started = rflu(ld_agent(P.started_total)) >= (uint32_t)P.n_tiles;
        if (tix == kNoWork && idle_rounds > 4096u) {
            const bool foreign_mine = rflu(ld_agent(&P.cu_foreign[simd_key])) != 0u;
            if ((!all_started && can_start) || foreign_mine)
                for (int d = 1; d < n_queues && tix == kNoWork; d++)
                    tix = scan_queue(home_q + d < n_queues ? home_q + d : home_q + d - n_queues, can_start && !all_started, foreign_mine, false);
        }
        if (tix == kNoWork) {
            STATS(if (idle_rounds == 0) st_t0 = sc0;)
            if (rflu(ld_agent(P.done_total)) >= (uint32_t)P.n_tiles) { STATS(st_idle += realtime() - st_t0;) break; }
            if (all_started && can_start) {
                uint32_t gone = 0;
                if (lane == 0) {
                    const uint32_t w = ld_agent(&P.cu_alive[simd_key]), l = ld_agent(&P.cu_live[simd_key]);
                    if (w > l && atomicCAS(&P.cu_alive[simd_key], w, w - 1u) == w) gone = 1u;
                }
                if (rflu(gone)) { STATS(st_idle += realtime() - st_t0;) break; }
            }
            const uint32_t naps = idle_rounds < 8u ? 1u : (idle_rounds < 64u ? 4u : 32u);
            idle_rounds += naps;
            if (naps == 32u) {
                const uint32_t beat = rflu(ld_agent(P.heartbeat)) + rflu(ld_agent(P.done_total));
                stale_looks = beat == last_beat ? stale_looks + 1u : 0u;
                last_beat = beat;
                if (stale_looks > kIdleStaleLooks) {
                    for (uint32_t k = P.q_img_begin[home_q]; k < P.q_img_begin[home_q + 1]; k++) {
                        const uint32_t im = P.q_images[k];
                        if (lane == 0 && ld_agent(&P.img_done[im]) < P.img_tile_begin[im + 1] - P.img_tile_begin[im]) atomicOr(&P.status[im], ST_STALLED | ST_CORRUPT);
                    }
                    break;
                }
            }
            for (uint32_t k = 0; k < naps; k++) __builtin_amdgcn_s_sleep(127);
            continue;
        }
        STATS(if (idle_rounds) st_idle += sc0 - st_t0; st_pick_t = realtime(); st_scan += st_pick_t - sc0; st_picks++;)
        idle_rounds = 0; stale_looks = 0;
        resumed = (tix & kResume) != 0u;
        tix &= ~kResume;
    }
    const Tile tile = P.tiles[tix];
    const bool long_tile = sched && ((rflu(tile.flags) >> kTileSizeClassShift) & 15u) <= kLongClass;
    if (long_tile && lane == 0) atomicAdd(&P.simd_long[simd_slot], 1u);
    TLOG(const unsigned long long tile_t0 = realtime();)
#ifndef FUIF_EMU
    {
        const int cls = (int)((rflu(tile.flags) >> kTileSizeClassShift) & 15u), over = cls - P.prio_base;
        const int prio = P.prio_base < 0 ? 0 : over <= 0 ? 3 : over >= 3 ? 0 : 3 - over;
        if (prio == 3) __builtin_amdgcn_s_setprio(3);
        if (prio == 2) __builtin_amdgcn_s_setprio(2);
        if (prio == 1) __builtin_amdgcn_s_setprio(1);
        if (prio == 0) __builtin_amdgcn_s_setprio(0);
    }
#endif
    STATS(unsigned long long waited = 0;)
    const int img = rfl((int)tile.image);
    const int first_c = rfl(tile.first_channel), last_c = rfl(tile.last_channel);

    const StreamJob job = P.jobs[img];
    Stream s;
    s.p = P.blobs + job.blob_off;
    s.size = rflu(job.blob_size);
    s.pos = rflu(tile.start);
    s.limit = rflu(job.limit);
    s.win_base = 0xFFFFFF00u;
    s.win = 0;
    s.eof_flag = 0;
    s.blob_mode = rfl((int)(job.flags & 1u));

    coef_t *coef = P.coef + (int64_t)img * P.coef_stride;
    ChannelMeta *meta = P.meta + (int64_t)img * P.n_channels;
    uint32_t *progress = P.progress + (size_t)img * nch;
    int status = 0;
    bool stalled = false;
    TileRec *const rec = sched ? P.tile_rec + tix : nullptr;
    uint2 *snodes_g = snodes_w;
    uint16_t *leaves = leaves_w;
    int ctx_slot = -1;
    bool can_yield = false;
    uint32_t ctx_leaves_units = 0;
    bool yielded = false;
    uint32_t yield_chan = 0, yield_val = 0, resume_y = 0;
    if (resumed) {
        s.pos = rflu(rec->pos);
        const uint32_t fl = rflu(rec->flags);
        status = (int)(fl & 0xFFu);
        s.eof_flag = (int)((fl >> 8) & 1u);
        ctx_slot = rfl((int)rec->ctx);
        resume_y = rflu(rec->y);
        ctx_leaves_units = rflu(rec->ctx_leaves);
        can_yield = true;
        if (ctx_slot >= 0) {
            uint8_t *cb = P.ctx_scratch + (size_t)(uint32_t)ctx_slot * 256u;
            snodes_g = reinterpret_cast<uint2 *>(cb);
            leaves = reinterpret_cast<uint16_t *>(cb + (size_t)ctx_leaves_units * 256u);
        }
    }
    uint32_t stale = 0, beat_seen = 0;
    auto spin_nap = [&](uint32_t &spins) {
        __builtin_amdgcn_s_sleep(8);
        if ((++spins & (kStaleCheck - 1u)) == 0u) {
            const uint32_t beat = rflu(ld_agent(P.heartbeat)) + rflu(ld_agent(P.done_total));
            stale = beat == beat_seen ? stale + 1u : 0u;
            beat_seen = beat;
            if (stale > kStaleLimit) { stalled = true; status |= ST_STALLED | ST_CORRUPT; }
        }
    };
    PROF_DECL;
#ifdef FUIF_PROF
    const unsigned long long prof_rt0 = realtime();
    const unsigned long long prof_seg0 = __builtin_readcyclecounter();
#endif
    auto publish = [&](int c, uint32_t v) {
        if (kHandOff) {
            drain_stores();
            if (lane == 0) {
                st_agent(progress + c, v);
                if ((v & 31u) == 0u) atomicAdd(P.heartbeat, 1u);
            }
        }
    };
    auto wait_header = [&](int c) {
        uint32_t spins = 0;
        if (!stalled && rflu(ld_agent(progress + c)) == 0u) {
            STATS(const unsigned long long w0 = realtime();)
            while (!stalled && rflu(ld_agent(progress + c)) == 0u) spin_nap(spins);
            STATS(waited += realtime() - w0;)
        }
    };

    for (int ci = resumed ? last_c : first_c; ci <= last_c; ci++) {
        int beginc = ci, endc = ci, compress = 1, predictor = 0, firstrealc = ci;
        if (resumed) predictor = (int)((rflu(rec->flags) >> 9) & 7u);
        if (!resumed) {
        if (!((s.limit == 0 || s.pos < s.limit) && !s_eof(s))) break;
        if (!rfl(geom[ci].w) || !rfl(geom[ci].h)) continue;

        if (s_limit_hit(s)) continue;
        const uint32_t group_pos = s.pos;
        int firstbyte = s_varint(s, lane);
        if (s_limit_hit(s)) continue;
        endc = beginc + (firstbyte >> 4);
        compress = firstbyte & 1;
        predictor = (firstbyte & 14) >> 1;
        int global_minv = 1 - s_varint(s, lane);
        if (s_limit_hit(s)) continue;
        if (global_minv == 1) global_minv = s_varint(s, lane);
        if (s_limit_hit(s)) continue;
        const int global_maxv = global_minv + s_varint(s, lane);
        if (s_limit_hit(s)) continue;
        if (endc > last_c || endc < beginc) { status |= ST_CORRUPT; break; }
        if (lane == 0) P.group_start[(size_t)img * nch + beginc] = group_pos + 1u;

        firstrealc = beginc;
        bool fatal = false, early = false;
        for (int i = beginc; i <= endc; i++) {
            const int gw = rfl(geom[i].w), gh = rfl(geom[i].h);
            const int64_t goff = geom[i].coef_off;
            if ((int64_t)gw * gh <= 0) { publish(i, 1u); continue; }
            int minv = global_minv, maxv = global_maxv;
            if (endc > beginc && global_minv < global_maxv) {
                minv += s_varint(s, lane);
                maxv = minv + s_varint(s, lane);
            }
            int q = 1;
            if (minv == maxv) {
                fill_plane<kHandOff>(coef + goff, 0, (int64_t)gw * gh, minv, lane);
                firstrealc++;
            }
            bool have_q = !(minv == 0 && maxv == 0);
            if (have_q) q = s_varint(s, lane);
            if (lane == 0) { st_agent(&meta[i].minval, minv); st_agent(&meta[i].maxval, maxv); st_agent(&meta[i].q, q); st_agent(&meta[i].decoded, (minv == maxv) ? 1 : 0); }
            publish(i, (minv == maxv) ? (uint32_t)gh + 1u : 1u);
            if (!have_q) continue;
            if (s_limit_hit(s)) {
                fill_plane<kHandOff>(coef + goff, 0, (int64_t)gw * gh, 0, lane);
                if (lane == 0) st_agent(&meta[i].decoded, 1);
                publish(i, (uint32_t)gh + 1u);
                status |= ST_TRUNCATED;
                early = true;
                break;
            }
            if (maxv < minv) { fatal = true; break; }
            if (compress && !check_bit_depth(minv, maxv, predictor)) { fatal = true; break; }
        }
        __syncthreads();
        if (fatal) { status |= ST_UNSUPPORTED | ST_CORRUPT; break; }
        if (early) continue;
        if (firstrealc > endc) { ci = endc; continue; }
        }

        int nrefs = 0;
        int nprops = 0;
        {
            int offset = 0;
            for (int j = beginc - 1; j >= 0 && offset < P.max_properties; j--) {
                if (j < first_c) wait_header(j);
                const int jmin = rfl(ld_agent(&meta[j].minval)), jmax = rfl(ld_agent(&meta[j].maxval));
                if (jmin == jmax) continue;
                if (rfl(geom[j].hshift) < 0) continue;
                int mn = jmin; if (mn > 0) mn = 0;
                int mx = jmax; if (mx < 0) mx = 0;
                if (lane == 0) {
                    sh.lo[nprops] = 0; sh.hi[nprops] = iabs(mx > -mn ? mx : mn);
                    sh.lo[nprops + 1] = slog(mn); sh.hi[nprops + 1] = slog(mx);
                    RefChan rc;
                    rc.off = geom[j].coef_off;
                    rc.w = geom[j].w; rc.h = geom[j].h; rc.hshift = geom[j].hshift; rc.vshift = geom[j].vshift;
                    rc.chan = j; rc.pad = 0;
                    sh.refs[nrefs] = rc;
                }
                nprops += 2; offset += 2;
                nrefs++;
            }
            int mn = 0x7FFFFFFF, mx = (int)0x80000001, maxh = 0, maxw = 0;
            for (int j = beginc; j <= endc; j++) {
                const int jmin = rfl(ld_agent(&meta[j].minval)), jmax = rfl(ld_agent(&meta[j].maxval));
                if (jmin < mn) mn = jmin;
                if (jmax > mx) mx = jmax;
                const int jh = rfl(geom[j].h), jw = rfl(geom[j].w);
                if (jh > maxh) maxh = jh;
                if (jw > maxw) maxw = jw;
            }
            if (mn > 0) mn = 0;
            if (mx < 0) mx = 0;
            const int amax = iabs(mn) > iabs(mx) ? iabs(mn) : iabs(mx);
            if (lane == 0) {
                int n = nprops;
                sh.lo[n] = 0; sh.hi[n] = amax; n++;
                sh.lo[n] = 0; sh.hi[n] = amax; n++;
                sh.lo[n] = slog(mn); sh.hi[n] = slog(mx); n++;
                sh.lo[n] = slog(mn); sh.hi[n] = slog(mx); n++;
                sh.lo[n] = 0; sh.hi[n] = maxh - 1; n++;
                sh.lo[n] = 0; sh.hi[n] = maxw - 1; n++;
                sh.lo[n] = mn + mn - mx; sh.hi[n] = mx + mx - mn; n++;
                sh.lo[n] = mn + mn - mx; sh.hi[n] = mx + mx - mn; n++;
                for (int k = 0; k < 5; k++) { sh.lo[n] = slog(mn - mx); sh.hi[n] = slog(mx - mn); n++; }
            }
            nprops += kNonRefProps;
        }
        const int nrefprops = nprops - kNonRefProps;
        const bool wide_props = nprops > 32;
        const int prop_pitch = wide_props ? kPropPitchWide : kPropPitch;
        const int prop_mask = wide_props ? 63 : 31;
        const int chunk_px = wide_props ? kChunk / 2 : kChunk;

        int predictability = 2048;
        Rac rac;
        int tree_size = 1, n_super = 1, cur_leaf = 0;
        bool narrow = false;
        bool compact = false;
        if (resumed) {
            rac.range = rflu(rec->range); rac.low = rflu(rec->low);
            tree_size = rfl((int)rec->tree_size); n_super = rfl((int)rec->n_super); cur_leaf = rfl((int)rec->cur_leaf);
            narrow = (rflu(rec->flags) & kRecNarrow) != 0u;
            compact = (rflu(rec->flags) & kRecCompact) != 0u;
            if (ctx_slot < 0) leaves = reinterpret_cast<uint16_t *>(reinterpret_cast<uint8_t *>(snodes_w) + (size_t)n_super * (narrow ? 256u : 512u));
            if (narrow) for (int sn = 1; sn <= kLdsN && sn < n_super; sn++) lds_narrow[(sn - 1) * 64 + lane] = reinterpret_cast<const uint32_t *>(snodes_g)[(size_t)sn * 64 + lane];
            else for (int sn = 1; sn <= kLdsSuper && sn < n_super; sn++) sh.snodes[(sn - 1) * 64 + lane] = snodes_g[(size_t)sn * 64 + lane];
            __syncthreads();
        }
        if (!resumed) {
        if (predictor == 0 && compress) {
            int rounded = s_varint(s, lane);
            if (rounded < 1 || rounded > 127) {
                if (s_limit_hit(s)) {
                    fill_plane<kHandOff>(coef + geom[firstrealc].coef_off, 0, (int64_t)geom[firstrealc].w * geom[firstrealc].h, 0, lane);
                    if (lane == 0) st_agent(&meta[firstrealc].decoded, 1);
                    publish(firstrealc, (uint32_t)rfl(geom[firstrealc].h) + 1u);
                    status |= ST_TRUNCATED;
                    continue;
                }
                status |= ST_CORRUPT;
                break;
            }
            predictability = rounded * 32;
        }

        rac_init(rac, s, lane);

        if (!compress) {
            for (int i = beginc; i <= endc; i++) {
                const int gw = rfl(geom[i].w), gh = rfl(geom[i].h);
                const int minv = rfl(ld_agent(&meta[i].minval)), maxv = rfl(ld_agent(&meta[i].maxval));
                if (minv == maxv) continue;
                coef_t *plane = coef + geom[i].coef_off;
                const int zero = minv > 0 ? minv : (maxv < 0 ? maxv : 0);
                int y = 0;
                for (; y < gh; y++) {
                    if (s_limit_hit(s)) break;
                    for (int x0 = 0; x0 < gw; x0 += 64) {
                        const int nx = min(64, gw - x0);
                        int rowv = 0;
                        for (int j = 0; j < nx; j++) rowv = wrlane(uniform_read(rac, s, lane, minv, maxv - minv), j, rowv);
                        if (lane < nx) st_plane<kHandOff>(plane + (int64_t)y * gw + x0 + lane, rowv);
                    }
                    publish(i, (uint32_t)y + 2u);
                }
                if (y < gh) { fill_plane<kHandOff>(plane, (int64_t)y * gw, (int64_t)(gh - y) * gw, rfl(geom[i].ctor_data) ? 0 : zero, lane); status |= ST_TRUNCATED; }
                if (lane == 0) st_agent(&meta[i].decoded, 1);
                publish(i, (uint32_t)gh + 1u);
                if (s_limit_hit(s)) break;
            }
            __syncthreads();
            ci = endc;
            continue;
        }

        __syncthreads();
        const bool narrow_ok = nprops <= 32 && __ballot(lane < nprops && (sh.lo[lane] < -kNarrowSplitMax || sh.hi[lane] > kNarrowSplitMax)) == 0ull;
        for (int k = lane; k < 3 * 32; k += 64) sh.meta_ctx[k / 32][k % 32] = 0;
        __syncthreads();
        if (lane == 0) for (int k = 0; k < 3; k++) symbol_chance_init(sh.meta_ctx[k], 1024);
        __syncthreads();
        tree_size = 1;
        int leaf_count = 0;
        bool tree_ok = true;
        {
            int pos = 0, depth = 0;
            while (true) {
                int p = ctx_symbol2(rac, s, lane, sh.meta_ctx[0], tree_table, 0, nprops) - 1;
                if (p != -1) {
                    const int oldmin = rfl(sh.lo[p]), oldmax = rfl(sh.hi[p]);
                    if (oldmin >= oldmax) { tree_ok = false; break; }
                    const int splitval = ctx_symbol2(rac, s, lane, sh.meta_ctx[2], tree_table, oldmin, oldmax - 1);
                    const int child = tree_size;
                    if (tree_size + 2 > P.max_nodes || depth >= kTreeStackDepth) { tree_ok = false; status |= ST_UNSUPPORTED; break; }
                    if (lane == 0) {
                        Node n; n.property = (int16_t)p; n.child = (uint16_t)child; n.splitval = splitval;
                        nodes[pos] = n;
                        Frame f; f.p = p; f.oldmin = oldmin; f.oldmax = oldmax; f.splitval = splitval; f.child = child; f.stage = 0;
                        stack[depth] = f;
                        sh.lo[p] = splitval + 1;
// ... 142 lines not shown
                else if (inner) tgt = kSlowFlag | (uint32_t)t;
                else tgt = kLeafFlag | (uint32_t)n.child;
                n_super += __popcll(__ballot(admit));
                uint2 out;
                out.x = (uint32_t)(is_raw_slog_prop(st_prop[lane] - nrefprops) && st_split[lane] != 0x7FFFFFFF ? slog_threshold(st_split[lane]) : st_split[lane]);
                out.y = (((uint32_t)st_prop[lane] << 2) & 0xFFu) | (tgt << 8);
                if (narrow) {
                    const uint32_t w = pack_narrow((int)out.x, (uint32_t)st_prop[lane], inner ? (tgt & 0x1FFFu) : (kLeafFlagN | (uint32_t)n.child));
                    reinterpret_cast<uint32_t *>(snodes_g)[(size_t)sn * 64 + lane] = w;
                    if (sn >= 1 && sn <= kLdsN) lds_narrow[(sn - 1) * 64 + lane] = w;
                } else {
                    snodes_g[(size_t)sn * 64 + lane] = out;
                    if (sn >= 1 && sn <= kLdsSuper) sh.snodes[(sn - 1) * 64 + lane] = out;
                }
                __syncthreads();
            }
        }
        if (exact_area) {
            const uint32_t sn_units = narrow ? (uint32_t)n_super : (uint32_t)n_super * 2u;
            const uint32_t off = grant_area(sn_units + ((uint32_t)nleaves * leaf_bytes + 255u) / 256u);
            if (off != 0xFFFFFFFFu) {
                ctx_slot = (int)off;
                uint8_t *cb = P.ctx_scratch + (size_t)off * 256u;
                uint32_t *dst = reinterpret_cast<uint32_t *>(cb);
                const uint32_t *src = reinterpret_cast<const uint32_t *>(snodes_w);
                for (uint32_t k = (uint32_t)lane; k < sn_units * 64u; k += 64u) dst[k] = src[k];
                snodes_g = reinterpret_cast<uint2 *>(cb);
                leaves = reinterpret_cast<uint16_t *>(cb + (size_t)sn_units * 256u);
                ctx_leaves_units = sn_units;
                __syncthreads();
            } else {
                STATS(st_noctx++;)
                pinned_tix = tix;
            }
        }
        if (ctx_slot < 0) leaves = reinterpret_cast<uint16_t *>(reinterpret_cast<uint8_t *>(snodes_w) + (size_t)n_super * (narrow ? 256u : 512u));
        {
            if (lane == 0) {
                if (compact) {
                    uint16_t full[32];
                    symbol_chance_init(full, predictability);
                    for (int k = 0; k < kMantCompact; k++) leaves[k] = full[k];
                    for (int k = 0; k < 16 - kMantCompact; k++) leaves[kMantCompact + k] = full[CH_MANT + k];
                } else { symbol_chance_init(leaves, predictability); leaves[31] = 0; }
            }
            __syncthreads();
            const uint32_t *l0 = reinterpret_cast<const uint32_t *>(leaves);
            uint32_t *lw = reinterpret_cast<uint32_t *>(leaves);
            const int words = compact ? 8 : 16;
            const uint32_t mine = l0[lane & (words - 1)];
            for (int64_t i = words + lane; i < (int64_t)nleaves * words; i += 64) lw[i] = mine;
            __syncthreads();
        }
        }
        const uint2 root_nd = narrow ? uint2{0u, 0u} : snodes_g[lane];
        const uint32_t root_w = narrow ? reinterpret_cast<const uint32_t *>(snodes_g)[lane] : 0u;
        LeafRegs L;
        const uint32_t leaf_shift = compact ? 5u : 6u, leaf_l2 = (uint32_t)(lane & (compact ? 15 : 31)) * 2u;
        L.leafv = (int)*reinterpret_cast<const uint16_t *>(reinterpret_cast<const char *>(leaves) + (((uint32_t)cur_leaf << leaf_shift) + leaf_l2));
        uint32_t leaf_shift_v = leaf_shift;
#ifndef FUIF_EMU
        asm volatile("v_mov_b32 %0, %1" : "=v"(leaf_shift_v) : "s"(leaf_shift));
#endif
        L.touched = 0; L.bits = 0;
        L.mb = rfl(compact ? kMantCompact : CH_MANT); L.mirror = rflu(compact ? 0x10001u : 1u);
        auto switch_leaf = [&](int id) {
            if (LIKELY(id != cur_leaf)) {
                char *lb = reinterpret_cast<char *>(leaves);
                const uint32_t l2 = leaf_l2;
                const int fresh = (int)*reinterpret_cast<const uint16_t *>(lb + (((uint32_t)id << leaf_shift_v) + l2));
                *reinterpret_cast<uint16_t *>(lb + (((uint32_t)cur_leaf << leaf_shift_v) + l2)) = (uint16_t)L.leafv;
                L.leafv = fresh;
                cur_leaf = id;
            }
        };

        for (int i = beginc; i <= endc; i++) {
            const int w = rfl(geom[i].w), h = rfl(geom[i].h);
            const int ghs = rfl(geom[i].hshift), gvs = rfl(geom[i].vshift);
            const int minv = rfl(ld_agent(&meta[i].minval)), maxv = rfl(ld_agent(&meta[i].maxval));
            if (minv == maxv) continue;
            coef_t *plane = coef + geom[i].coef_off;
            const int zero = minv > 0 ? minv : (maxv < 0 ? maxv : 0);
            int y = resumed ? (int)resume_y : 0;
            uint32_t ref_seen = 0;
            if (tree_size == 1 && predictor == 0 && zero == 0) {
                for (; y < h; y++) {
                    if (s_limit_hit(s)) break;
                    for (int x0 = 0; x0 < w; x0 += 64) {
                        const int nx = min(64, w - x0);
                        int rowv = 0;
                        for (int j = 0; j < nx; j++) {
                            rowv = wrlane(leaf_symbol(rac, s, lane, L, minv, maxv), j, rowv);
                            leaf_commit(L, lane, pixel_table);
                        }
                        if (lane < nx) st_plane<kHandOff>(plane + (int64_t)y * w + x0 + lane, rowv);
                    }
                    publish(i, (uint32_t)y + 2u);
                }
            } else {
                FastSym fsym;
                fsym.amax_pos = maxv - zero; fsym.amax_neg = zero - minv;
                fsym.emax_pos = ilog2u((uint32_t)fsym.amax_pos); fsym.emax_neg = ilog2u((uint32_t)fsym.amax_neg);
                fsym.ilast_pos = rfl(fsym.emax_pos + 1); fsym.ilast_neg = rfl(fsym.emax_neg + 1);
                const bool sym_fast = minv < zero && zero < maxv;
                auto rows = [&](auto pred0_tag, auto narrow_tag) {
                    constexpr bool PRED0 = decltype(pred0_tag)::value;
                    constexpr bool NARROW = decltype(narrow_tag)::value;
                    for (; y < h; y++) {
                        if (s_limit_hit(s)) break;
                        __syncthreads();
                        if (kHandOff && nrefs) {
                            uint32_t need = 0;
                            const uint32_t *fp = progress;
                            if (lane < nrefs) {
                                const RefChan rc = sh.refs[lane];
                                int ry = (y << gvs) >> rc.vshift; if (ry >= rc.h) ry = rc.h - 1;
                                need = (uint32_t)ry + 2u;
                                fp = progress + rc.chan;
                            }
                            uint32_t spins = 0;
                            if (__any(ref_seen < need)) {
                                if (ref_seen < need) ref_seen = ld_agent(fp);
                                if (__any(ref_seen < need) && can_yield) {
                                    const int bl = __builtin_ctzll(__ballot(ref_seen < need));
                                    const RefChan rcb = sh.refs[bl];
                                    const uint32_t nb = (uint32_t)rdlane((int)need, bl) + P.yield_slack, fin = (uint32_t)rfl(rcb.h) + 1u;
                                    yield_chan = (uint32_t)rfl(rcb.chan); yield_val = nb < fin ? nb : fin;
                                    resume_y = (uint32_t)y;
                                    EMU_COUNT(3);
                                    yielded = true;
                                    break;
                                }
                                if (__any(ref_seen < need)) {
                                    STATS(const unsigned long long w0 = realtime();)
                                    while (__any(ref_seen < need) && !stalled) {
                                        spin_nap(spins);
                                        if (ref_seen < need) ref_seen = ld_agent(fp);
                                    }
                                    STATS(waited += realtime() - w0;)
                                }
                            }
                        }
                        const coef_t *row1 = plane + (int64_t)(y - 1) * w;
                        const coef_t *row2 = plane + (int64_t)(y - 2) * w;
                        int left = zero, leftleft = zero;
                        const int kloc = (lane & prop_mask) - nrefprops;
                        const bool f_abs = (kloc == 1);
                        const int m_left = ((kloc == 1) | (kloc == 3) | (kloc == 12) | (y ? ((kloc == 6) | (kloc == 8)) : ((kloc == 7) | (kloc == 9)))) ? -1 : 0;
                        const int m_ll = (kloc == 12) ? -1 : 0;
                        for (int x0 = 0; x0 < w; x0 += chunk_px) {
                            const int nx = min(chunk_px, w - x0);
                            PROF_START();
                            const int x = min(x0 + lane, w - 1);
                            const int vtop = y ? row1[x] : zero;
                            const int vtl = (y && x) ? row1[x - 1] : zero;
                            const int vtr = (x + 1 < w && y) ? row1[x + 1] : vtop;
                            const int vtt = y > 1 ? row2[x] : vtop;
                            if (lane < chunk_px) {
                                int32_t *cp = sh.cprops + lane * prop_pitch;
                                for (int k = kFastRefs; k < nrefs; k++) {
                                    const RefChan rc = sh.refs[k];
                                    int ry = (y << gvs) >> rc.vshift; if (ry >= rc.h) ry = rc.h - 1;
                                    int rx = ghs < 0 ? rc.w - 1 : (x << ghs) >> rc.hshift; if (rx >= rc.w) rx = rc.w - 1;
                                    const int v = ld_plane<kHandOff>(coef + rc.off + (int64_t)ry * rc.w + rx);
                                    cp[2 * k] = iabs(v); cp[2 * k + 1] = slog(v);
                                }
                                auto ref_sample = [&](int k) -> int {
                                    const RefChan rc = sh.refs[k < nrefs ? k : 0];
                                    int ry = (y << gvs) >> rc.vshift; if (ry >= rc.h) ry = rc.h - 1;
                                    int rx = ghs < 0 ? rc.w - 1 : (x << ghs) >> rc.hshift; if (rx >= rc.w) rx = rc.w - 1;
                                    return ld_plane<kHandOff>(coef + rc.off + (int64_t)ry * rc.w + rx);
                                };
                                static_assert(kFastRefs == 9, "the reference loads are issued in batches of 6 + 3");
                                if (nrefs > 0) {
                                    const int r0 = ref_sample(0), r1 = ref_sample(1), r2 = ref_sample(2), r3 = ref_sample(3), r4 = ref_sample(4), r5 = ref_sample(5);
                                    cp[0] = iabs(r0); cp[1] = slog(r0);
                                    if (nrefs > 1) { cp[2] = iabs(r1); cp[3] = slog(r1); }
                                    if (nrefs > 2) { cp[4] = iabs(r2); cp[5] = slog(r2); }
                                    if (nrefs > 3) { cp[6] = iabs(r3); cp[7] = slog(r3); }
                                    if (nrefs > 4) { cp[8] = iabs(r4); cp[9] = slog(r4); }
// ... 124 lines not shown
                                            s.win_base = s.pos & ~3u;
                                            s.win = reinterpret_cast<const uint32_t *>(s.p + s.win_base)[lane];
                                        }
                                        diff = fast_symbol(rac, s, L, fsym);
#else
                                        if constexpr (kChunkFast) {
                                            if (UNLIKELY(widx > 188u)) {
                                                s.pos = s.win_base + widx;
                                                s.win_base = s.pos & ~3u;
                                                widx = s.pos - s.win_base;
                                                s.win = reinterpret_cast<const uint32_t *>(s.p + s.win_base)[lane];
                                            }
                                            diff = fast_symbol_hw_w(rac, widx, s.win, L, fsym);
                                        } else {
                                            if (UNLIKELY(s.pos - s.win_base > 188u)) {
                                                s.win_base = s.pos & ~3u;
                                                s.win = reinterpret_cast<const uint32_t *>(s.p + s.win_base)[lane];
                                            }
                                            diff = fast_symbol_hw(rac, s, L, fsym);
                                        }
#endif
                                    } else diff = leaf_symbol(rac, s, lane, L, mn, mx);
                                    PROF_LAP(4);
                                    leaf_commit(L, lane, pixel_table);
                                }
                                const int v = diff + guess;
                                rowv = wrlane(v, j, rowv);
                                leftleft = l;
                                left = v;
                                PROF_LAP(5);
                            }
                            if (part == 0 && j_split) leftleft = left;
                            }
#ifndef FUIF_EMU
                            if constexpr (kChunkFast) s.pos = s.win_base + widx;
#endif
                            };
                            if (PRED0 && sym_fast && s.pos + 64u * (uint32_t)(nx + 1) <= s.size) pixels(std::true_type{}); else pixels(std::false_type{});
                            PROF_START();
                            if (lane < nx) st_plane<kHandOff>(plane + (int64_t)y * w + x0 + lane, rowv);
                            __syncthreads();
                            PROF_LAP(5);
                        }
                        publish(i, (uint32_t)y + 2u);
                    }
                };
                if (predictor == 0) { if (narrow) rows(std::true_type{}, std::true_type{}); else rows(std::true_type{}, std::false_type{}); }
                else { if (narrow) rows(std::false_type{}, std::true_type{}); else rows(std::false_type{}, std::false_type{}); }
            }
            if (yielded) break;
            if (y < h) { __syncthreads(); fill_plane<kHandOff>(plane, (int64_t)y * w, (int64_t)(h - y) * w, rfl(geom[i].ctor_data) ? 0 : zero, lane); status |= ST_TRUNCATED; }
            if (lane == 0) st_agent(&meta[i].decoded, 1);
            publish(i, (uint32_t)h + 1u);
            if (s_limit_hit(s)) break;
        }
        if (yielded) {
            if (lane < (compact ? 16 : 32)) leaves[((int64_t)cur_leaf << (leaf_shift - 1u)) + lane] = (uint16_t)L.leafv;
            if (lane == 0) {
                rec->wait_chan = yield_chan; rec->wait_val = yield_val; rec->y = resume_y;
                rec->range = rac.range; rec->low = rac.low; rec->pos = s.pos;
                rec->flags = ((uint32_t)status & 0xFFu) | ((uint32_t)(s.eof_flag & 1) << 8) | ((uint32_t)predictor << 9) | (long_tile ? kRecLong : 0u) | (narrow ? kRecNarrow : 0u) | (compact ? kRecCompact : 0u);
                if (long_tile) atomicAdd(&P.simd_long[simd_slot], 0xFFFFFFFFu);
                rec->ctx = (uint32_t)ctx_slot; rec->ctx_leaves = ctx_leaves_units; rec->tree_size = (uint32_t)tree_size; rec->n_super = (uint32_t)n_super; rec->cur_leaf = (uint32_t)cur_leaf;
                rec->pin = ctx_slot >= 0 ? 0u : my_pin;
                rec->owner = simd_key + 1u;
            }
            drain_stores();
            if (lane == 0) st_agent(&rec->state, (uint32_t)TS_READY);
            break;
        }
        __syncthreads();
        ci = endc;
    }
#ifdef FUIF_PROF
    if (yielded) { prof_acc[7] += __builtin_readcyclecounter() - prof_seg0; prof_acc[6] += realtime() - prof_rt0; }
    if (yielded && lane == 0 && P.prof) for (int k = 0; k < 8; k++) atomicAdd(&P.prof[(size_t)PROF_ROW * 8 + k], prof_acc[k]);
#endif
    TLOG(if (yielded && lane == 0 && P.tile_log) {
        unsigned long long *tl = P.tile_log + (size_t)tix * 4;
        if (!resumed) tl[1] = tile_t0;
        tl[3] = (tl[3] + (realtime() - tile_t0)) & 0xFFFFFFFFFFFFull;
    })
    if (yielded) { STATS(st_yields++;) __syncthreads(); continue; }
    if (s_limit_hit(s)) status |= ST_TRUNCATED;
    if (rflu(tile.end) != 0u && !(status & (ST_TRUNCATED | ST_CORRUPT)) && s.pos != rflu(tile.end)) status |= ST_CORRUPT;
    __syncthreads();
    for (int c = first_c; c <= last_c; c++) {
        const int gw = rfl(geom[c].w), gh = rfl(geom[c].h);
        const uint32_t done = (uint32_t)gh + 1u;
        if (!kHandOff || rflu(ld_agent(progress + c)) != done) {
            if ((int64_t)gw * gh > 0 && rfl(ld_agent(&meta[c].decoded)) == 0) fill_plane<kHandOff>(coef + geom[c].coef_off, 0, (int64_t)gw * gh, 0, lane);
            publish(c, done);
        }
    }
    if (lane == 0) { atomicOr(&P.status[img], status); atomicMax(&P.consumed[img], s.pos); }
    STATS(st_spin += waited;)
    if (sched) {
        if (pinned_tix == tix) pinned_tix = kNoWork;
        if (lane == 0) {
            st_agent(&rec->state, (uint32_t)TS_DONE);
            if (ld_agent(&rec->foreign)) atomicAdd(&P.cu_foreign[simd_key], 0xFFFFFFFFu);
            if (long_tile) atomicAdd(&P.simd_long[simd_slot], 0xFFFFFFFFu);
            atomicAdd(&P.cu_live[simd_key], 0xFFFFFFFFu);
            atomicAdd(&P.img_done[img], 1u);
            atomicAdd(P.done_total, 1u);
        }
    }
#if defined(FUIF_STATS) || defined(FUIF_PROF) || defined(FUIF_TILELOG)
    if (lane == 0 && P.tile_log) {
        unsigned long long *tl = P.tile_log + (size_t)tix * 4;
        const unsigned long long t_end = realtime();
        tl[0] = ((unsigned long long)(uint32_t)img << 32) | (uint32_t)first_c;
        if (!resumed) tl[1] = tile_t0;
        tl[2] = t_end;
#ifdef FUIF_EMU
        const unsigned long long simd_id = (unsigned long long)blockIdx.x & 3ull;
#else
        const unsigned long long simd_id = ((unsigned long long)__builtin_amdgcn_s_getreg((31 << 11) | 4) >> 4) & 3ull;
#endif
        tl[3] = ((tl[3] + (t_end - tile_t0)) & 0xFFFFFFFFFFFFull) | ((unsigned long long)simd_key << 48) | (simd_id << 60);
    }
#endif
#ifdef FUIF_PROF
    prof_acc[7] += __builtin_readcyclecounter() - prof_seg0; prof_acc[6] += realtime() - prof_rt0;
    if (lane == 0 && P.prof) for (int k = 0; k < 8; k++) atomicAdd(&P.prof[(size_t)PROF_ROW * 8 + k], prof_acc[k]);
#endif
    __syncthreads();
    }
#ifdef FUIF_STATS
    if (sched && lane == 0 && P.sched_stats) {
        atomicAdd(&P.sched_stats[0], st_idle); atomicAdd(&P.sched_stats[1], st_picks); atomicAdd(&P.sched_stats[2], st_yields); atomicAdd(&P.sched_stats[3], st_scan); atomicAdd(&P.sched_stats[4], st_spin); atomicAdd(&P.sched_stats[5], st_noctx); atomicAdd(&P.sched_stats[6], st_busy); atomicAdd(&P.sched_stats[7], realtime() - st_begin);
    }
#endif
}

int maniac_max_waves(int config, int *per_simd) {
    int dev = 0, per_cu = 0;
    hipDeviceProp_t prop;
    if (hipGetDevice(&dev) != hipSuccess || hipGetDeviceProperties(&prop, dev) != hipSuccess) return 0;
    hipError_t e = config == 1 ? hipOccupancyMaxActiveBlocksPerMultiprocessor(&per_cu, k_maniac_decode<kLdsDense, true>, 64, 0)
                 : config == 2 ? hipOccupancyMaxActiveBlocksPerMultiprocessor(&per_cu, k_maniac_decode<kLdsWideAlone, true>, 64, 0)
                               : hipOccupancyMaxActiveBlocksPerMultiprocessor(&per_cu, k_maniac_decode<kLdsWide, true>, 64, 0);
    if (e != hipSuccess || per_cu < 1) per_cu = 1;
    if (per_simd) *per_simd = per_cu / 4 > 0 ? per_cu / 4 : 1;
    return per_cu * prop.multiProcessorCount;
}

void launch_maniac_decode(const DecodeParams &P, int n_waves, int config, int hand_off, hipStream_t stream) {
    if (config == 1) hipLaunchKernelGGL((k_maniac_decode<kLdsDense, true>), dim3(n_waves), dim3(64), 0, stream, P);
    else if (config == 2 && hand_off) hipLaunchKernelGGL((k_maniac_decode<kLdsWideAlone, true>), dim3(n_waves), dim3(64), 0, stream, P);
    else if (config == 2) hipLaunchKernelGGL((k_maniac_decode<kLdsWideAlone, false>), dim3(n_waves), dim3(64), 0, stream, P);
    else if (hand_off) hipLaunchKernelGGL((k_maniac_decode<kLdsWide, true>), dim3(n_waves), dim3(64), 0, stream, P);
    else hipLaunchKernelGGL((k_maniac_decode<kLdsWide, false>), dim3(n_waves), dim3(64), 0, stream, P);
}

}


#ifdef FUIF_EMU
namespace fuifgpu { namespace { unsigned long long g_emu_stats[6]; } }
extern "C" void fuifgpu_emu_walk_stats(unsigned long long *out6, int reset) {
    for (int k = 0; k < 6; k++) { out6[k] = fuifgpu::g_emu_stats[k]; if (reset) fuifgpu::g_emu_stats[k] = 0; }
}
#endif
```

fuif_amd/csrc/writer.cpp:

```cpp
#include <algorithm>
#include <cmath>
#include <cstdlib>
#include <cstring>
#include <vector>

#include "../../include/fuifgpu.h"
#include "fuifgpu_internal.h"
#include "maniac_encode.h"

namespace fuifgpu {
namespace {

constexpr int CH_ZERO = 0, CH_SIGN = 1, CH_EXP = 2, CH_MANT = 16, CH_N = 31;

inline int ilog2u(uint32_t l) { return l == 0 ? 0 : 31 - __builtin_clz(l); }
inline int slog(int x) {
    if (x == 0) return 0;
    if (x > 0) return 32 - __builtin_clz((unsigned)x);
    return -(32 - __builtin_clz((unsigned)(-x)));
}
inline int iabs(int x) { return x < 0 ? -x : x; }
inline int median3(int a, int b, int c) {
    if (a < b) { if (b < c) return b; return a < c ? c : a; }
    if (a < c) return a;
    return b < c ? c : b;
}

struct Chan {
    std::vector<int32_t> data;
    int w = 0, h = 0, minval = 0, maxval = 0, zero = 0, q = 1;
    int hshift = 0, vshift = 0, hcshift = 0, vcshift = 0, component = -1;
    mutable int32_t *dev = nullptr;
    int64_t zeros = -1;
    bool resident() const { return dev && data.empty(); }
    void setzero() { zero = minval > 0 ? minval : (maxval < 0 ? maxval : 0); }
    void minmax() {
        int mn = 0x7FFFFFFF, mx = (int)0x80000001;
        for (int32_t v : data) { if (v < mn) mn = v; if (v > mx) mx = v; }
        minval = mn; maxval = mx;
    }
};

struct Bytes {
    std::vector<uint8_t> b;
    void put(int c) { b.push_back((uint8_t)c); }
    void varint(size_t number, bool done = true) {
        if (number < 128) put((int)(done ? number : number + 128));
        else { size_t lsb = number & 127; varint(number >> 7, false); varint(lsb, done); }
    }
};

struct RacEnc {
    Bytes &out;
// ... 540 lines not shown
    lp.stride = std::max<size_t>(1, npix / target);
    if (lp.stride > 1 && lp.stride % 2 == 0) lp.stride++;
    lp.n_samples = (npix + lp.stride - 1) / lp.stride;
    return lp;
}

void write_tree(RacEnc &rac, const Learner *L, std::vector<Range> ranges, const uint16_t *table, std::vector<TNode> &out) {
    uint16_t ctx[3][CH_N];
    for (int k = 0; k < 3; k++) chance_init(ctx[k], 1024);
    const int nprops = (int)ranges.size();
    out.assign(1, TNode());
    struct Rec {
        RacEnc &rac; const Learner *L; std::vector<Range> &rg; const uint16_t *table; std::vector<TNode> &out; uint16_t (*ctx)[CH_N]; int nprops;
        void go(int lnode, int pos) {
            int p = (L && lnode >= 0) ? L->nodes[lnode].prop : -1;
            write_symbol2(rac, ctx[0], table, 0, nprops, p + 1);
            out[pos].prop = p;
            if (p < 0) return;
            int oldmin = rg[p].lo, oldmax = rg[p].hi;
            int s = L->nodes[lnode].split;
            write_symbol2(rac, ctx[2], table, oldmin, oldmax - 1, s);
            out[pos].split = s;
            int child = (int)out.size();
            out[pos].child = child;
            out.push_back(TNode()); out.push_back(TNode());
            rg[p].lo = s + 1;
            go(L->nodes[lnode].gt, child);
            rg[p].lo = oldmin; rg[p].hi = s;
            go(L->nodes[lnode].le, child + 1);
            rg[p].hi = oldmax;
        }
    } rec{rac, L, ranges, table, out, ctx, nprops};
    rec.go(L ? 0 : -1, 0);
    int leaf = 0;
    for (auto &n : out) if (n.prop < 0) n.leaf = leaf++;
}

int build_enc_group(const Chan &c, const std::vector<RefInfo> &refs, int predictor, EncGroup &g) {
    int rc = ensure_dev(c);
    g = EncGroup{};
    g.w = c.w; g.h = c.h; g.hshift = c.hshift; g.vshift = c.vshift;
    g.minval = c.minval; g.maxval = c.maxval; g.zero = c.zero; g.predictor = predictor;
    g.nrefs = (int)refs.size();
    if (g.nrefs > kMaxRefs) rc = FUIFGPU_E_ARG;
    for (int k = 0; k < g.nrefs && rc == FUIFGPU_OK; k++) {
        const Chan &r = *refs[k].c;
        rc = ensure_dev(r);
        g.refs[k] = EncRef{r.dev, r.w, r.h, r.hshift, r.vshift};
    }
    g.plane = c.dev;
    return rc;
}

size_t encode_group(Bytes &io, Image &img, int ci, int predictor, bool compress, const GroupCoder &gc, size_t &header_pos, EncJob *defer = nullptr) {
    Chan &c = img.ch[ci];
    io.varint((size_t)((0 << 4) + (predictor << 1) + (compress ? 1 : 0)));
    if (c.minval <= 0) io.varint((size_t)(1 - c.minval));
    else { io.varint(0); io.varint((size_t)c.minval); }
    io.varint((size_t)(c.maxval - c.minval));
    if (!(c.minval == 0 && c.maxval == 0)) io.varint((size_t)c.q);
    c.setzero();
    header_pos = io.b.size();
    if (c.minval == c.maxval) return 0;

    std::vector<Range> ranges; std::vector<RefInfo> refs;
    const int nprops = init_properties(ranges, refs, img, ci, ci, gc.max_properties);
    int predictability = 2048;
    if (predictor == 0 && compress) {
        uint64_t zeroes = 0, pixels = (uint64_t)c.w * c.h;
        if (c.zeros >= 0) zeroes = (uint64_t)c.zeros;
        else for (int32_t v : c.data) zeroes += (v == 0);
        int rounded = (int)(zeroes * 128 / pixels);
        rounded = std::max(1, std::min(127, rounded));
        io.varint((size_t)rounded);
        predictability = rounded * 32;
    }
    RacEnc rac(io);
    if (!compress) {
        std::vector<int32_t> fetched;
        if (c.resident()) {
            fetched.resize((size_t)c.w * c.h);
            const int rc = plane_download(fetched.data(), c.dev, fetched.size());
            if (rc != FUIFGPU_OK && gc.gpu_rc && *gc.gpu_rc == FUIFGPU_OK) *gc.gpu_rc = rc;
        }
        for (int32_t v : c.resident() ? fetched : c.data) uniform_write(rac, c.minval, c.maxval - c.minval, v);
        rac.flush();
        return io.b.size() - header_pos;
    }
    std::vector<int32_t> props(nprops);
    Learner L;
    const Learner *use = nullptr;
    const size_t npix = (size_t)c.w * c.h;
    const LearnPlan lp = plan_learner(c, gc.tree_mode, gc.max_tree_nodes);
    if (lp.stride) {
        const size_t stride = lp.stride;
        L.max_depth = lp.max_depth; L.min_leaf = lp.min_leaf;
        L.nprops = nprops; L.scale = (double)stride; L.max_nodes = gc.max_tree_nodes;
        L.threshold_bits = (double)gc.split_bits;
        if (c.resident()) {
            const int job = gc.samples && gc.sample_job ? (*gc.sample_job)[(size_t)ci] : -1;
            if (job < 0) { if (gc.gpu_rc && *gc.gpu_rc == FUIFGPU_OK) *gc.gpu_rc = FUIFGPU_E_HIP; }
            else {
                L.props.assign(gc.samples->props((size_t)job), gc.samples->props((size_t)job) + lp.n_samples * (size_t)nprops);
                L.bucket.assign(gc.samples->bucket((size_t)job), gc.samples->bucket((size_t)job) + lp.n_samples);
            }
        } else for (size_t i = 0; i < npix; i += stride) {
            int y = (int)(i / c.w), x = (int)(i % c.w);
            int guess = props_and_guess(props.data(), c, refs, x, y, predictor);
            int d = c.data[i] - guess;
            L.props.insert(L.props.end(), props.begin(), props.end());
            L.bucket.push_back((uint8_t)(d == 0 ? 0 : ilog2u((uint32_t)iabs(d)) + 1));
        }
        std::vector<int> idx(L.bucket.size());
        for (size_t i = 0; i < idx.size(); i++) idx[i] = (int)i;
        L.nodes.assign(1, Learner::LNode());
        L.build(idx, 0, (int)idx.size(), 0, 0);
        if (L.nodes.size() > 1) use = &L;
    }
    std::vector<TNode> tree;
    write_tree(rac, use, ranges, gc.tree_table, tree);
    const int nleaves = ((int)tree.size() + 1) / 2;
    std::vector<uint16_t> leaves((size_t)nleaves * CH_N);
    chance_init(leaves.data(), predictability);
    for (int l = 1; l < nleaves; l++) memcpy(&leaves[(size_t)l * CH_N], leaves.data(), sizeof(uint16_t) * CH_N);
    if (defer) {
        const int rc = build_enc_group(c, refs, predictor, defer->g);
        defer->tree.resize(tree.size());
        for (size_t k = 0; k < tree.size(); k++) defer->tree[k] = EncNode{tree[k].prop, tree[k].split, tree[k].child, tree[k].leaf};
        defer->n_leaves = nleaves;
        memcpy(defer->leaf_init, leaves.data(), sizeof(uint16_t) * CH_N);
        defer->state = RacEncState{rac.range, rac.low, rac.delayed, rac.pending};
        if (rc != FUIFGPU_OK && gc.gpu_rc && *gc.gpu_rc == FUIFGPU_OK) *gc.gpu_rc = rc;
        return io.b.size() - header_pos;
    }
    if (gc.gpu_entropy) {
        EncGroup g{};
        int rc = build_enc_group(c, refs, predictor, g);
        if (rc == FUIFGPU_OK) {
            std::vector<EncNode> nodes(tree.size());
            for (size_t k = 0; k < tree.size(); k++) nodes[k] = EncNode{tree[k].prop, tree[k].split, tree[k].child, tree[k].leaf};
            RacEncState st{rac.range, rac.low, rac.delayed, rac.pending};
            rc = maniac_encode_group_gpu(g, nodes.data(), (int)nodes.size(), nleaves, leaves.data(), gc.pixel_table, &st, io.b, *gc.scratch);
            rac.range = st.range; rac.low = st.low; rac.delayed = st.delayed; rac.pending = st.pending;
        }
        if (rc != FUIFGPU_OK && gc.gpu_rc && *gc.gpu_rc == FUIFGPU_OK) *gc.gpu_rc = rc;
    } else if (tree.size() == 1 && predictor == 0 && c.zero == 0) {
        for (int32_t v : c.data) write_symbol(rac, leaves.data(), gc.pixel_table, c.minval, c.maxval, v);
    } else {
        for (int y = 0; y < c.h; y++)
            for (int x = 0; x < c.w; x++) {
                int guess = props_and_guess(props.data(), c, refs, x, y, predictor);
                int mn = c.minval - guess, mx = c.maxval - guess;
                if (mn == mx) continue;
                int pos = 0;
                while (tree[pos].prop >= 0) pos = (props[tree[pos].prop] > tree[pos].split) ? tree[pos].child : tree[pos].child + 1;
                write_symbol(rac, &leaves[(size_t)tree[pos].leaf * CH_N], gc.pixel_table, mn, mx, c.data[(size_t)y * c.w + x] - guess);
            }
    }
    rac.flush();
    return io.b.size() - header_pos;
}

}
}

using namespace fuifgpu;

namespace fuifgpu {
namespace {
int write_stream(Image &img, int nch, int bit_depth, bool squeezed, const fuifgpu_encode_options &o, uint8_t **blob_out, size_t *size_out,
                 bool dct_style = false);
}
}

static int build_transformed_image(const int32_t *planes, int w, int h, int nch, int bit_depth, const fuifgpu_encode_options &o,
                                   const fuifgpu::Lossy &lossy, fuifgpu::PaletteOpts pal, fuifgpu::Image &img, bool &squeezed, bool device_input = false) {
    using namespace fuifgpu;
    if (lossy.quality < 100.f && pal.colors > 0) pal = PaletteOpts();
    img.w = w; img.h = h; img.maxval = (1 << bit_depth) - 1; img.nb_channels = nch;
    img.ch.resize(nch);
    for (int c = 0; c < nch; c++) {
        Chan &ch = img.ch[c];
        ch.w = w; ch.h = h; ch.component = c; ch.minval = 0; ch.maxval = img.maxval;
        if (!device_input) ch.data.assign(planes + (size_t)c * w * h, planes + (size_t)(c + 1) * w * h);
    }
    const bool on_gpu = o.gpu_forward != 0 || device_input;
    int rc = FUIFGPU_OK;
    if (on_gpu) {
        for (int c = 0; c < nch && rc == FUIFGPU_OK; c++) {
            Chan &ch = img.ch[c];
            ch.dev = (int32_t *)fuifgpu_dev_alloc(sizeof(int32_t) * (size_t)w * h);
            if (!ch.dev) rc = FUIFGPU_E_HIP;
            else if (device_input) rc = dev_copy(ch.dev, planes + (size_t)c * w * h, sizeof(int32_t) * (size_t)w * h);
            else rc = plane_upload(ch.dev, ch.data.data(), (size_t)w * h);
            ch.data.clear();
        }
    }
    if (rc == FUIFGPU_OK && pal.pre > 0.f && o.ycocg) rc = compact_channels(img, pal.pre, true, on_gpu);
    if (rc == FUIFGPU_OK && o.ycocg && nch >= 3) {
        const int m = img.nb_meta;
        if (on_gpu) rc = fuifgpu_fwd_ycocg(img.ch[m].dev, img.ch[m + 1].dev, img.ch[m + 2].dev, w, h, nullptr);
        else fwd_ycocg(img);
        img.transforms.push_back({TR_YCOCG, {}});
    }
    if (rc == FUIFGPU_OK && pal.colors > 0) {
        if (img.nb_channels > 1) rc = try_palette(img, 0, img.nb_channels - 1, pal.colors, on_gpu);
        if (rc == FUIFGPU_OK && img.nb_channels > 3) rc = try_palette(img, 0, img.nb_channels - 2, pal.colors, on_gpu);
    }
    if (rc == FUIFGPU_OK && pal.post > 0.f) rc = compact_channels(img, pal.post, false, on_gpu);
    squeezed = false;
    if (rc == FUIFGPU_OK && o.squeeze && (int64_t)img.ch[0].w * img.ch[0].h > 20) {
        std::vector<int> params = default_squeeze_params(img);
        rc = fwd_squeeze(img, params, on_gpu);
        img.transforms.push_back({TR_SQUEEZE, {}});
        squeezed = true;
    }
    std::vector<char> all_zero(img.ch.size(), 0);
    if (rc == FUIFGPU_OK && lossy.active) rc = fwd_quantize(img, lossy, o.squeeze != 0, o.ycocg != 0, on_gpu, all_zero);
    if (on_gpu && (!device_input || rc != FUIFGPU_OK)) {
        for (size_t k = 0; k < img.ch.size(); k++) {
            Chan &ch = img.ch[k];
            if (rc == FUIFGPU_OK && ch.dev) {
                ch.data.assign((size_t)ch.w * ch.h, 0);
                if (!ch.data.empty() && !all_zero[k]) rc = plane_download(ch.data.data(), ch.dev, ch.data.size());
            }
            if (ch.dev) fuifgpu_dev_free(ch.dev);
            ch.dev = nullptr;
        }
    }
    return rc;
}

extern "C" {

void fuifgpu_free_blob(uint8_t *p) { free(p); }

static bool read_encode_options(const fuifgpu_encode_options *opt, fuifgpu_encode_options &o, int gpu_entropy_default) {
    memset(&o, 0, sizeof(o));
    if (!opt) {
        o.ycocg = 1; o.squeeze = 1; o.max_properties = 12; o.tree_mode = 1; o.max_tree_nodes = 4095; o.gpu_entropy = gpu_entropy_default;
    } else {
        const uint32_t sz = opt->struct_size;
        if (sz < 2 * sizeof(uint32_t) || (sz & 3u)) return false;
        memcpy(&o, opt, sz < sizeof(o) ? sz : sizeof(o));
    }
    o.struct_size = (uint32_t)sizeof(o);
    return true;
}

static bool read_lossy_options(const fuifgpu_lossy_options *lossy, Lossy &l) {
    l = Lossy();
    if (!lossy) return true;
    const uint32_t sz = lossy->struct_size;
    if (sz < sizeof(uint32_t) + sizeof(float) || (sz & 3u)) return false;
    return read_qualities(lossy->quality, sz >= sizeof(fuifgpu_lossy_options) ? lossy->chroma_quality : 101.f, l);
}

static bool read_palette_options(const fuifgpu_palette_options *palette, int nch, PaletteOpts &p) {
    p = PaletteOpts();
    if (!palette) return true;
    const uint32_t sz = palette->struct_size;
    if (sz < sizeof(uint32_t) || (sz & 3u)) return false;
    fuifgpu_palette_options v;
    memset(&v, 0, sizeof(v));
    memcpy(&v, palette, sz < sizeof(v) ? sz : sizeof(v));
    if (v.palette_colors < 0 || v.palette_colors > 32767) return false;
    if (!(v.compact_post_percent >= 0.f && v.compact_post_percent <= 100.f) || !(v.compact_pre_percent >= 0.f && v.compact_pre_percent <= 100.f)) return false;
    if (v.palette_colors > 0 && nch > 4) return false;
    p.colors = v.palette_colors;
    p.post = 0.01 * (double)v.compact_post_percent;
    p.pre = 0.01 * (double)v.compact_pre_percent;
    return true;
}

int fuifgpu_encode_plane_traffic(uint64_t *h2d_bytes, uint64_t *d2h_bytes) {
    if (h2d_bytes) *h2d_bytes = g_plane_h2d;
    if (d2h_bytes) *d2h_bytes = g_plane_d2h;
    return FUIFGPU_OK;
}

int fuifgpu_quantization_constant(float quality, float chroma_quality, int squeeze_option, int chroma_table, int shift) {
    Lossy l;
    if (shift < 0 || !read_qualities(quality, chroma_quality, l)) return -FUIFGPU_E_ARG;
    return l.active ? quantization_constant(l, squeeze_option != 0, chroma_table != 0, shift) : 1;
}

int fuifgpu_encode_image_ex(const int32_t *planes, int w, int h, int nch, int bit_depth, const fuifgpu_encode_options *opt,
                            const fuifgpu_lossy_options *lossy, const fuifgpu_palette_options *palette, uint8_t **blob_out, size_t *size_out) {
// ... 80 lines not shown
            who.push_back(&c);
        }
    std::vector<int32_t> stats(3 * recs.size());
    const int rc = channel_stats_gpu(recs.data(), (int)recs.size(), stats.data());
    for (size_t k = 0; k < who.size() && rc == FUIFGPU_OK; k++) { who[k]->minval = stats[3 * k]; who[k]->maxval = stats[3 * k + 1]; who[k]->zeros = stats[3 * k + 2]; }
    return rc;
}
int group_predictor(const Image &img, int i, bool squeezed, bool dct_style) {
    if (i < img.nb_meta) return 3;
    if (!squeezed && !dct_style) return 2;
    return i < img.nb_meta + img.nb_channels ? 2 : 0;
}
void responsive_downscales(Image &img, bool squeezed, bool dct_style) {
    recompute_downscales(img);
    if (!squeezed && !dct_style) for (int s = 0; s < 6; s++) img.downscales[s] = (int)img.ch.size() - 1;
}
int learn_samples_device(Image &img, bool squeezed, const GroupCoder &gc, LearnSamples &out, std::vector<int> &sample_job) {
    std::vector<LearnJob> jobs;
    sample_job.assign(img.ch.size(), -1);
    for (int i = 0; i < (int)img.ch.size(); i++) {
        Chan &c = img.ch[i];
        if (!c.resident() || !c.w || !c.h || c.minval == c.maxval) continue;
        const LearnPlan lp = plan_learner(c, gc.tree_mode, gc.max_tree_nodes);
        if (!lp.stride) continue;
        c.setzero();
        std::vector<Range> ranges; std::vector<RefInfo> refs;
        LearnJob job;
        job.nprops = init_properties(ranges, refs, img, i, i, gc.max_properties);
        job.n_samples = (int64_t)lp.n_samples; job.stride = (int64_t)lp.stride;
        const int rc = build_enc_group(c, refs, group_predictor(img, i, squeezed, false), job.g);
        if (rc != FUIFGPU_OK) return rc;
        sample_job[(size_t)i] = (int)jobs.size();
        jobs.push_back(job);
    }
    return learn_samples_jobs_gpu(jobs, out);
}
void begin_stream(const Image &img, int nch, int bit_depth, const fuifgpu_encode_options &o, Bytes &head, Bytes &io) {
    for (const char *m = "FUIF"; *m; m++) head.put(*m);
    head.varint((size_t)(nch + '0'));
    head.varint((size_t)(bit_depth + '&'));
    head.varint((size_t)(img.w - 1));
    head.varint((size_t)(img.h - 1));
    head.varint(0);
    head.varint((size_t)o.max_properties);
    io.varint(img.transforms.size());
    for (auto &t : img.transforms) {
        io.varint((size_t)((t.params.size() << 4) + t.id));
        for (int v : t.params) io.varint((size_t)v);
    }
}
void note_responsive(const Image &img, int i, size_t after, int responsive[5]) {
    for (int s = 0; s < 5; s++) if (img.downscales[s] == i) responsive[s] = (int)after;
}
int finish_stream(Bytes &head, const Bytes &io, int responsive[5], std::vector<GroupEntry> &group_at, bool emit_index, uint8_t **blob_out, size_t *size_out) {
    int rel = 0;
    for (int s = 0; s < 5; s++) {
        if (responsive[s] < 0) responsive[s] = (int)io.b.size();
        head.varint((size_t)(responsive[s] - rel));
        rel = responsive[s];
    }
    std::vector<uint8_t> trailer;
    if (emit_index && !group_at.empty()) {
        for (GroupEntry &g : group_at) g.start += (uint32_t)head.b.size();
        build_index_trailer(group_at, trailer);
    }
    const size_t total = head.b.size() + io.b.size() + trailer.size();
    uint8_t *blob = (uint8_t *)malloc(total ? total : 1);
    if (!blob) return FUIFGPU_E_NOMEM;
    memcpy(blob, head.b.data(), head.b.size());
    memcpy(blob + head.b.size(), io.b.data(), io.b.size());
    if (!trailer.empty()) memcpy(blob + head.b.size() + io.b.size(), trailer.data(), trailer.size());
    *blob_out = blob;
    *size_out = total;
    return FUIFGPU_OK;
}

int write_stream(Image &img, int nch, int bit_depth, bool squeezed, const fuifgpu_encode_options &o, uint8_t **blob_out, size_t *size_out,
                 bool dct_style) {
    EncScratch enc_scratch;
    struct DevCleanup {
        Image &img; EncScratch &s;
        ~DevCleanup() { for (Chan &c : img.ch) { if (c.dev) fuifgpu_dev_free(c.dev); c.dev = nullptr; } s.release(); }
    } dev_cleanup{img, enc_scratch};
    int gpu_rc = channel_ranges(&img, 1);
    if (gpu_rc != FUIFGPU_OK) return gpu_rc;
    responsive_downscales(img, squeezed, dct_style);

    std::vector<uint16_t> tables(16384);
    build_chance_table(tables.data(), 0xFFFFFFFFu / 19, 2);
    build_chance_table(tables.data() + 8192, 0x0d000000u, 6);
    GroupCoder gc{tables.data(), tables.data() + 8192, o.max_properties, o.tree_mode, o.max_tree_nodes, o.split_bits > 0 ? o.split_bits : 0};
    gc.gpu_entropy = o.gpu_entropy != 0; gc.scratch = &enc_scratch; gc.gpu_rc = &gpu_rc;

    Bytes head, io;
    begin_stream(img, nch, bit_depth, o, head, io);
    int responsive[5] = {-1, -1, -1, -1, -1};
    std::vector<GroupEntry> group_at;
    const int n = (int)img.ch.size();
    for (int i = 0; i < n; i++) {
        Chan &c = img.ch[i];
        if (!c.w || !c.h) continue;
        const int predictor = group_predictor(img, i, squeezed, dct_style);
        size_t header_pos = 0;
        size_t before = io.b.size();
        group_at.push_back(GroupEntry{(uint32_t)before, i});
        size_t body = encode_group(io, img, i, predictor, true, gc, header_pos);
        float bits = body * 8.0f, pixels = (float)c.w * c.h, ubits = 0.0f;
        if (c.maxval > c.minval) ubits = pixels * (ilog2u((uint32_t)(c.maxval - c.minval)) + 1) + 16;
        if (bits >= ubits) {
            io.b.resize(before);
            encode_group(io, img, i, predictor, false, gc, header_pos);
        }
        note_responsive(img, i, io.b.size(), responsive);
    }
    if (gpu_rc != FUIFGPU_OK) return gpu_rc;
    return finish_stream(head, io, responsive, group_at, o.emit_index != 0, blob_out, size_out);
}


struct PendingGroup {
    int channel = 0, predictor = 0, job = -1;
    Bytes prefix;
    size_t header_len = 0;
};
int write_streams_batch(std::vector<Image> &imgs, int nch, int bit_depth, const std::vector<char> &squeezed, const fuifgpu_encode_options &o,
                        uint8_t **blobs_out, size_t *sizes_out) {
    struct DevCleanup {
        std::vector<Image> &imgs;
        ~DevCleanup() { for (Image &im : imgs) for (Chan &c : im.ch) { if (c.dev) fuifgpu_dev_free(c.dev); c.dev = nullptr; } }
    } dev_cleanup{imgs};
    std::vector<uint16_t> tables(16384);
    build_chance_table(tables.data(), 0xFFFFFFFFu / 19, 2);
    build_chance_table(tables.data() + 8192, 0x0d000000u, 6);
    GroupCoder gc{tables.data(), tables.data() + 8192, o.max_properties, o.tree_mode, o.max_tree_nodes, o.split_bits > 0 ? o.split_bits : 0};
    int gpu_rc = channel_ranges(imgs.data(), imgs.size());
    if (gpu_rc != FUIFGPU_OK) return gpu_rc;
    gc.gpu_rc = &gpu_rc;
    std::vector<EncJob> jobs;
    std::vector<std::vector<PendingGroup>> pending(imgs.size());
    for (size_t m = 0; m < imgs.size(); m++) {
        Image &img = imgs[m];
        responsive_downscales(img, squeezed[m] != 0, false);
        LearnSamples samples;
        std::vector<int> sample_job;
        const int rc = learn_samples_device(img, squeezed[m] != 0, gc, samples, sample_job);
        if (rc != FUIFGPU_OK) return rc;
        gc.samples = &samples; gc.sample_job = &sample_job;
        for (int i = 0; i < (int)img.ch.size(); i++) {
            Chan &c = img.ch[i];
            if (!c.w || !c.h) continue;
            PendingGroup pg;
            pg.channel = i;
            pg.predictor = group_predictor(img, i, squeezed[m] != 0, false);
            if (c.minval != c.maxval) {
                EncJob job;
                encode_group(pg.prefix, img, i, pg.predictor, true, gc, pg.header_len, &job);
                pg.job = (int)jobs.size();
                jobs.push_back(std::move(job));
            }
            pending[m].push_back(std::move(pg));
        }
        gc.samples = nullptr; gc.sample_job = nullptr;
    }
    if (gpu_rc != FUIFGPU_OK) return gpu_rc;
    int rc = maniac_encode_jobs_gpu(jobs, gc.pixel_table);
    if (rc != FUIFGPU_OK) return rc;
    for (size_t m = 0; m < imgs.size(); m++) {
        Image &img = imgs[m];
        Bytes head, io;
// ... 85 lines not shown
```

include/fuifgpu.h:

```cpp
#ifndef FUIFGPU_H
#define FUIFGPU_H
#include <stddef.h>
#include <stdint.h>

#ifdef __cplusplus
extern "C" {
#endif

#define FUIFGPU_ABI_VERSION 3

#define FUIFGPU_OK 0
#define FUIFGPU_E_NOT_FUIF 1
#define FUIFGPU_E_CORRUPT 2
#define FUIFGPU_E_UNSUPPORTED 3
#define FUIFGPU_E_ARG 4
#define FUIFGPU_E_HIP 5
#define FUIFGPU_E_MISMATCH 6
#define FUIFGPU_E_NOMEM 7

#define FUIFGPU_ST_TRUNCATED 1
#define FUIFGPU_ST_CORRUPT 2
#define FUIFGPU_ST_UNSUPPORTED 4
#define FUIFGPU_ST_STALLED 8

// ... 11 lines not shown

typedef struct {
    int32_t w, h, hshift, vshift, hcshift, vcshift, component, reserved;
    int64_t offset;
} fuifgpu_channel_desc;

const char *fuifgpu_strerror(int code);
const char *fuifgpu_last_error(void);
int fuifgpu_abi_version(void);

int fuifgpu_plan_create(const uint8_t *blob, size_t size, fuifgpu_plan **out);
void fuifgpu_plan_destroy(fuifgpu_plan *plan);
int fuifgpu_plan_info(const fuifgpu_plan *plan, fuifgpu_image_info *info);
int fuifgpu_plan_coded_channel(const fuifgpu_plan *plan, int index, fuifgpu_channel_desc *desc);
int fuifgpu_plan_output_channel(const fuifgpu_plan *plan, int index, fuifgpu_channel_desc *desc);
int fuifgpu_plan_transform(const fuifgpu_plan *plan, int index, int32_t *id, int32_t *params_out, int cap, int32_t *nparams);
void fuifgpu_build_chance_table(uint16_t *table8192, uint32_t alpha, int cut);

int fuifgpu_batch_create(const fuifgpu_plan *plan, int n_images, size_t blob_capacity_bytes,
                         int16_t *coef_ext, int32_t *out_ext, int tmp_images, fuifgpu_batch **out);
void fuifgpu_batch_destroy(fuifgpu_batch *batch);

int fuifgpu_batch_create_streaming(const fuifgpu_plan *plan, int n_images, size_t blob_capacity_bytes, int tmp_images, fuifgpu_batch **out);
int fuifgpu_batch_undo_transforms_to(fuifgpu_batch *batch, int first_image, int n_images, int32_t *out_device, void *stream);

int fuifgpu_batch_create_sibling(fuifgpu_batch *primary, size_t blob_capacity_bytes, fuifgpu_batch **out);

int fuifgpu_batch_upload(fuifgpu_batch *batch, const uint8_t *const *blobs, const size_t *sizes,
                         int n_images, int preview, void *stream);

int fuifgpu_batch_decode(fuifgpu_batch *batch, void *stream);

int fuifgpu_batch_undo_transforms(fuifgpu_batch *batch, void *stream);

int fuifgpu_batch_sync(fuifgpu_batch *batch, void *stream);
int fuifgpu_batch_status(fuifgpu_batch *batch, int32_t *status, uint32_t *bytes_consumed);
int fuifgpu_batch_channel_meta(fuifgpu_batch *batch, int image, int32_t *meta4_per_channel);
int16_t *fuifgpu_batch_coef_ptr(fuifgpu_batch *batch, int image);
int32_t *fuifgpu_batch_out_ptr(fuifgpu_batch *batch, int image);
int fuifgpu_batch_download_coef(fuifgpu_batch *batch, int image, int32_t *host, void *stream);
int fuifgpu_batch_download_out(fuifgpu_batch *batch, int image, int32_t *host, void *stream);
size_t fuifgpu_plan_packed_bytes(const fuifgpu_plan *plan, int components);
int fuifgpu_batch_pack_out(fuifgpu_batch *batch, int first_image, int n_images, int components, uint8_t *dst_device, void *stream);
int fuifgpu_batch_download_packed(fuifgpu_batch *batch, int image, int components, uint8_t *host, void *stream);

int fuifgpu_plane_checksums(const int32_t *planes_device, int64_t elems_per_image, int64_t image_stride, int n_images, uint64_t *sums_device, void *stream);

int fuifgpu_batch_last_timing(fuifgpu_batch *batch, float *decode_ms, float *transform_ms);
int fuifgpu_batch_profile(fuifgpu_batch *batch, uint64_t *out8_per_image);
int fuifgpu_batch_tile_log(fuifgpu_batch *batch, uint64_t *out4_per_tile, int cap, int *n_tiles);
int fuifgpu_batch_sched_stats(fuifgpu_batch *batch, uint64_t *out8);

int fuifgpu_index_parse(const uint8_t *blob, size_t size, int32_t *first_channel, uint32_t *start, int cap, int *n_groups);
int fuifgpu_index_append(const uint8_t *blob, size_t size, const int32_t *first_channel, const uint32_t *start, int n_groups,
                         uint8_t **blob_out, size_t *size_out);
int fuifgpu_batch_group_index(fuifgpu_batch *batch, int image, int32_t *first_channel, uint32_t *start, int cap, int *n_groups);
int fuifgpu_batch_set_group_parallel(fuifgpu_batch *batch, int enable);
int fuifgpu_batch_set_in_flight(fuifgpu_batch *batch, int n_batches);

int fuifgpu_device_count(int *n_devices);
int fuifgpu_set_device(int device);
int fuifgpu_get_device(int *device);
int fuifgpu_batch_device(const fuifgpu_batch *batch, int *device);
int fuifgpu_peer_copy(void *dst_device_ptr, int dst_device, const void *src_device_ptr, int src_device, size_t bytes, void *stream);

void *fuifgpu_dev_alloc(size_t bytes);
void fuifgpu_dev_free(void *device_ptr);
int fuifgpu_dev_mem_info(size_t *free_bytes, size_t *total_bytes);
int fuifgpu_dev_upload(void *dst_device, const void *src_host, size_t bytes);
int fuifgpu_dev_download(void *dst_host, const void *src_device, size_t bytes);

int fuifgpu_inv_hsqueeze(const int32_t *avg, int w1, const int32_t *res, int w2, int h, int32_t *out, int n_planes,
                         int64_t avg_stride, int64_t res_stride, int64_t out_stride, void *stream);
int fuifgpu_inv_vsqueeze(const int32_t *avg, int h1, const int32_t *res, int h2, int w, int32_t *out, int n_planes,
                         int64_t avg_stride, int64_t res_stride, int64_t out_stride, void *stream);
int fuifgpu_inv_ycocg(int32_t *c0, int32_t *c1, int32_t *c2, int w, int h, int p0, int p1, int p2, int maxval, void *stream);
int fuifgpu_inv_ycbcr(int32_t *c0, int32_t *c1, int32_t *c2, int w, int h, int p0, int p1, int p2, int minval, int maxval, void *stream);
int fuifgpu_inv_quantize(int32_t *plane, int64_t n_samples, int q, void *stream);
int fuifgpu_idct8x8(const int32_t *const *src64_dev, int bw, int bh, int32_t *out, int maxval, void *stream);
int fuifgpu_upsample(const int32_t *in, int w, int h, int srh, int srv, int32_t *out, void *stream);
int fuifgpu_inv_palette(const int32_t *index, int w, int h, const int32_t *palette_row, int colours, int32_t *out, void *stream);
int fuifgpu_inv_approximate(int32_t *plane, const int32_t *remainder, int64_t n_samples, int q, void *stream);
int fuifgpu_inv_match(const int32_t *match, int w, int h, int32_t *const *planes, int n_planes, int softmatch, int match_q, int match_maxval,
                      int nb_frames, void *stream);
int fuifgpu_fwd_ycocg(int32_t *c0, int32_t *c1, int32_t *c2, int w, int h, void *stream);
int fuifgpu_fwd_hsqueeze(const int32_t *in, int w, int h, int32_t *avg, int32_t *res, void *stream);
int fuifgpu_fwd_vsqueeze(const int32_t *in, int w, int h, int32_t *avg, int32_t *res, void *stream);
int fuifgpu_fwd_quantize(int32_t *plane, int64_t n_samples, int q, int32_t *minmax_device, void *stream);

typedef struct {
    uint32_t struct_size;
    int32_t ycocg;
    int32_t squeeze;
    int32_t max_properties;
    int32_t tree_mode;
    int32_t max_tree_nodes;
    int32_t emit_index;
    int32_t split_bits;
    int32_t gpu_forward;
    int32_t gpu_entropy;
} fuifgpu_encode_options;
int fuifgpu_encode_image(const int32_t *planes, int w, int h, int nch, int bit_depth, const fuifgpu_encode_options *opt,
                         uint8_t **blob_out, size_t *size_out);
int fuifgpu_encode_images(const int32_t *const *planes, int n_images, int w, int h, int nch, int bit_depth, const fuifgpu_encode_options *opt,
                          uint8_t **blobs_out, size_t *sizes_out);
typedef struct {
    uint32_t struct_size;
    float quality;
    float chroma_quality;
} fuifgpu_lossy_options;
int fuifgpu_encode_image_lossy(const int32_t *planes, int w, int h, int nch, int bit_depth, const fuifgpu_encode_options *opt,
                               const fuifgpu_lossy_options *lossy, uint8_t **blob_out, size_t *size_out);
int fuifgpu_encode_images_lossy(const int32_t *const *planes, int n_images, int w, int h, int nch, int bit_depth, const fuifgpu_encode_options *opt,
                                const fuifgpu_lossy_options *lossy, uint8_t **blobs_out, size_t *sizes_out);
int fuifgpu_encode_images_device(const int32_t *const *planes_device, int n_images, int w, int h, int nch, int bit_depth,
                                 const fuifgpu_encode_options *opt, const fuifgpu_lossy_options *lossy,
                                 uint8_t **blobs_out, size_t *sizes_out);
int fuifgpu_channel_stats(const int32_t *plane_device, int64_t n_samples, int32_t *stats3_device, void *stream);
int fuifgpu_encode_plane_traffic(uint64_t *h2d_bytes, uint64_t *d2h_bytes);
typedef struct {
    uint32_t struct_size;
    int32_t palette_colors;
    float compact_post_percent;
    float compact_pre_percent;
} fuifgpu_palette_options;
int fuifgpu_encode_image_ex(const int32_t *planes, int w, int h, int nch, int bit_depth, const fuifgpu_encode_options *opt,
                            const fuifgpu_lossy_options *lossy, const fuifgpu_palette_options *palette, uint8_t **blob_out, size_t *size_out);
int fuifgpu_encode_images_ex(const int32_t *const *planes, int planes_on_device, int n_images, int w, int h, int nch, int bit_depth,
                             const fuifgpu_encode_options *opt, const fuifgpu_lossy_options *lossy, const fuifgpu_palette_options *palette,
                             uint8_t **blobs_out, size_t *sizes_out);
int fuifgpu_fwd_palette(const int32_t *const *planes_device, int nb, int64_t n_samples, int max_colors, int32_t *index_device,
                        int32_t *palette_host, int *n_colors, void *stream);
int fuifgpu_quantization_constant(float quality, float chroma_quality, int squeeze_option, int chroma_table, int shift);
typedef struct {
    int32_t w, h, hshift, vshift, hcshift, vcshift, component, q;
    const int32_t *data;
} fuifgpu_raw_channel;
int fuifgpu_encode_channels(const fuifgpu_raw_channel *channels, int n_channels, int w, int h, int nb_channels, int bit_depth,
                            const int32_t *transforms, int n_transform_words, const fuifgpu_encode_options *opt,
                            uint8_t **blob_out, size_t *size_out);
void fuifgpu_free_blob(uint8_t *blob);

#ifdef __cplusplus
}
#endif
#endif
```

Measured before the change: 1458 Mpixels/s.

## Add intra-channel entropy checkpoints so decode splits large channels into row segments

The encoder now snapshots the range-coder state, leaf chance tables and two context rows at chosen row boundaries inside a channel group. These snapshots go into a v2 index trailer. The decoder parses them and emits one tile per row segment, so a single large channel can be decoded by several wavefronts at once instead of one. Progress tracking becomes per-segment and there are new device buffers for segment and checkpoint metadata. The cost is a larger stream, more host-side planning and more upload traffic. Checkpoints only take effect if the test streams were encoded with them, subject to a size-overhead budget.

```diff
diff --git a/fuif_amd/__init__.py b/fuif_amd/__init__.py
--- a/fuif_amd/__init__.py
+++ b/fuif_amd/__init__.py
@@ -96,11 +96,11 @@
     "fuifgpu_batch_create_streaming", "fuifgpu_batch_undo_transforms_to", "fuifgpu_batch_channel_meta", "fuifgpu_batch_coef_ptr", "fuifgpu_batch_out_ptr", "fuifgpu_batch_download_coef",
     "fuifgpu_batch_download_out", "fuifgpu_batch_last_timing", "fuifgpu_batch_profile", "fuifgpu_batch_tile_log", "fuifgpu_batch_sched_stats", "fuifgpu_inv_hsqueeze", "fuifgpu_inv_vsqueeze",
     "fuifgpu_inv_ycocg", "fuifgpu_inv_ycbcr", "fuifgpu_inv_quantize", "fuifgpu_idct8x8", "fuifgpu_upsample", "fuifgpu_inv_palette", "fuifgpu_inv_approximate", "fuifgpu_inv_match", "fuifgpu_fwd_ycocg", "fuifgpu_fwd_hsqueeze", "fuifgpu_fwd_vsqueeze", "fuifgpu_fwd_quantize", "fuifgpu_encode_image", "fuifgpu_encode_channels", "fuifgpu_free_blob",
-    "fuifgpu_index_parse", "fuifgpu_index_append", "fuifgpu_batch_group_index", "fuifgpu_batch_set_group_parallel",
+    "fuifgpu_index_parse", "fuifgpu_index_checkpoints", "fuifgpu_index_append", "fuifgpu_batch_group_index", "fuifgpu_batch_set_group_parallel",
     "fuifgpu_plan_packed_bytes", "fuifgpu_batch_pack_out", "fuifgpu_batch_download_packed",
     "fuifgpu_dev_alloc", "fuifgpu_dev_free", "fuifgpu_dev_upload", "fuifgpu_dev_download",
     "fuifgpu_encode_image_lossy", "fuifgpu_encode_images_lossy", "fuifgpu_quantization_constant",
-    "fuifgpu_encode_images_device", "fuifgpu_channel_stats", "fuifgpu_encode_plane_traffic",
+    "fuifgpu_encode_images_device", "fuifgpu_channel_stats", "fuifgpu_encode_plane_traffic", "fuifgpu_set_segment_samples", "fuifgpu_set_checkpoint_percent",
     "fuifgpu_encode_image_ex", "fuifgpu_encode_images_ex", "fuifgpu_fwd_palette",
     "fuifgpu_plane_checksums", "fuifgpu_device_count", "fuifgpu_set_device", "fuifgpu_get_device", "fuifgpu_batch_device", "fuifgpu_peer_copy", "fuifgpu_batch_set_in_flight",
 ]
@@ -206,7 +206,10 @@
     L.fuifgpu_encode_image.argtypes = [vp, C.c_int, C.c_int, C.c_int, C.c_int, C.POINTER(EncodeOptions), C.POINTER(vp), C.POINTER(C.c_size_t)]
     L.fuifgpu_encode_images.argtypes = [C.POINTER(vp), C.c_int, C.c_int, C.c_int, C.c_int, C.c_int, C.POINTER(EncodeOptions), C.POINTER(vp), C.POINTER(C.c_size_t)]
     L.fuifgpu_free_blob.argtypes = [vp]; L.fuifgpu_free_blob.restype = None
+    L.fuifgpu_set_segment_samples.argtypes = [C.c_longlong]
+    L.fuifgpu_set_checkpoint_percent.argtypes = [C.c_int]
     L.fuifgpu_index_parse.argtypes = [C.c_char_p, C.c_size_t, vp, vp, C.c_int, C.POINTER(C.c_int)]
+    L.fuifgpu_index_checkpoints.argtypes = [C.c_char_p, C.c_size_t, vp, vp, C.c_int, C.POINTER(C.c_int)]
     L.fuifgpu_index_append.argtypes = [C.c_char_p, C.c_size_t, vp, vp, C.c_int, C.POINTER(vp), C.POINTER(C.c_size_t)]
     L.fuifgpu_batch_group_index.argtypes = [vp, C.c_int, vp, vp, C.c_int, C.POINTER(C.c_int)]
     L.fuifgpu_batch_set_group_parallel.argtypes = [vp, C.c_int]
@@ -560,10 +563,21 @@
     return np.ascontiguousarray(pal[:nb, :count.value])
 
 
+def set_segment_samples(samples, percent=-1):
+    _check(lib().fuifgpu_set_segment_samples(int(samples)))
+    _check(lib().fuifgpu_set_checkpoint_percent(int(percent)))
+
+
 def index_parse(blob):
     fc, st, n = np.zeros(4096, np.int32), np.zeros(4096, np.uint32), C.c_int(0)
     _check(lib().fuifgpu_index_parse(blob, len(blob), fc.ctypes.data, st.ctypes.data, 4096, C.byref(n)))
     return [(int(fc[i]), int(st[i])) for i in range(min(n.value, 4096))]
+
+
+def index_checkpoints(blob):
+    rows, cnt, n = np.zeros(4096, np.int32), np.zeros(4096, np.int32), C.c_int(0)
+    _check(lib().fuifgpu_index_checkpoints(blob, len(blob), rows.ctypes.data, cnt.ctypes.data, 4096, C.byref(n)))
+    return [(int(rows[k]), int(cnt[k])) for k in range(n.value)]
 
 
 def index_append(blob, groups):
diff --git a/fuif_amd/csrc/capi.hip b/fuif_amd/csrc/capi.hip
--- a/fuif_amd/csrc/capi.hip
+++ b/fuif_amd/csrc/capi.hip
@@ -40,6 +40,12 @@
     Tile *d_tiles = nullptr;
     int tiles_cap = 0, n_tiles = 0;
     uint32_t *d_progress = nullptr, *d_group_start = nullptr;
+    size_t progress_cap = 0;
+    int prog_stride = 0;
+    ChanSeg *d_chan_seg = nullptr;
+    size_t chan_seg_cap = 0;
+    Checkpoint *d_ckpts = nullptr;
+    size_t ckpts_cap = 0;
     uint32_t *d_sched = nullptr, *d_layout = nullptr;
     size_t sched_words = 0, layout_cap = 0;
     int sched = 0, n_queues = 1, waves_per_simd = 4;
@@ -357,6 +363,7 @@
     }
     hipFree(b->d_blobs); hipFree(b->d_jobs); hipFree(b->d_geom); hipFree(b->d_meta); hipFree(b->d_status); hipFree(b->d_consumed);
     hipFree(b->d_tables); hipFree(b->d_scratch); hipFree(b->d_tmp); hipFree(b->d_coef32); hipFree(b->d_list); hipFree(b->d_widen); hipFree(b->d_prof); hipFree(b->d_tile_log);
+    hipFree(b->d_chan_seg); hipFree(b->d_ckpts);
     hipFree(b->d_tiles); hipFree(b->d_progress); hipFree(b->d_group_start); hipFree(b->d_sched); hipFree(b->d_layout); hipFree(b->d_ctx);
     if (b->own_coef) hipFree(b->d_coef);
     if (b->own_out) hipFree(b->d_out);
@@ -409,7 +416,9 @@
     b->max_waves[2] = maniac_max_waves(2);
     if (const char *e = getenv("FUIFGPU_IN_FLIGHT")) b->in_flight = std::max(1, atoi(e));
     if (b->max_waves[0] < 1 || b->max_waves[1] < 1 || b->max_waves[2] < 1) { g_last_error = "cannot query the device occupancy of the entropy kernel"; fuifgpu_batch_destroy(b); return FUIFGPU_E_HIP; }
-    CHK(hipMalloc((void **)&b->d_progress, sizeof(uint32_t) * (size_t)n_images * std::max(nch, 1)));
+    if (const char *e = getenv("FUIFGPU_MAX_WAVES")) for (int k = 0; k < 3; k++) b->max_waves[k] = std::max(1, std::min(b->max_waves[k], atoi(e)));
+    b->progress_cap = (size_t)n_images * std::max(nch, 1);
+    CHK(hipMalloc((void **)&b->d_progress, sizeof(uint32_t) * b->progress_cap));
     CHK(hipMalloc((void **)&b->d_group_start, sizeof(uint32_t) * (size_t)n_images * std::max(nch, 1)));
     if (coef_ext) b->d_coef = coef_ext;
     else { CHK(hipMalloc((void **)&b->d_coef, sizeof(coef_t) * (size_t)std::max<int64_t>(p.coef_elems, 1) * n_images)); b->own_coef = true; }
@@ -481,7 +490,7 @@
 }
 
 static int stage_streams(fuifgpu_batch *b, const uint8_t *const *blobs, const size_t *sizes, int n_images, int preview, hipStream_t st,
-                         std::vector<std::vector<GroupEntry>> &groups, std::vector<int> &group_of) {
+                         std::vector<std::vector<GroupEntry>> &groups, std::vector<std::vector<std::vector<Checkpoint>>> &ckpts, std::vector<int> &group_of) {
     b->jobs.assign(n_images, StreamJob{});
     size_t off = 0;
     Plan tmp;
@@ -501,9 +510,12 @@
             if (r != FUIFGPU_OK) { g_last_error = tmp.message; return r; }
             if (tmp.signature != b->plan.signature) { g_last_error = "image " + std::to_string(i) + " has a different geometry/transform chain"; return FUIFGPU_E_MISMATCH; }
             std::vector<GroupEntry> idx;
-            if (b->group_parallel) parse_index_trailer(blobs[i], sizes[i], tmp.data_start, nch, idx, nullptr);
-            if (idx.empty()) idx.push_back(GroupEntry{(uint32_t)tmp.data_start, 0});
+            std::vector<std::vector<Checkpoint>> ck;
+            if (b->group_parallel) parse_index_trailer(blobs[i], sizes[i], tmp.data_start, nch, idx, nullptr, &ck, &b->plan.coded);
+            if (idx.empty()) { idx.push_back(GroupEntry{(uint32_t)tmp.data_start, 0}); ck.clear(); }
+            ck.resize(idx.size());
             groups.push_back(std::move(idx));
+            ckpts.push_back(std::move(ck));
             group_of[i] = (int)groups.size() - 1;
             HIPCHK(hipMemsetAsync(b->d_blobs + off + (padded - 32), 0, 32, st));
             HIPCHK(hipMemcpyAsync(b->d_blobs + off, blobs[i], sizes[i], hipMemcpyHostToDevice, st));
@@ -528,18 +540,14 @@
     int cfg = 1, n_waves = 0, sched = 0, n_queues = 1;
     std::vector<Tile> tiles;
     std::vector<uint32_t> layout;
+    std::vector<ChanSeg> chan_seg;
+    std::vector<Checkpoint> ckpts;
+    int prog_stride = 1;
 };
-static WorkList plan_work_list(const Plan &plan, const std::vector<std::vector<GroupEntry>> &groups, const std::vector<int> &group_of, const size_t *sizes,
-                               const int *max_waves, int waves_per_simd, int in_flight, bool group_order) {
+static WorkList plan_work_list(const Plan &plan, const std::vector<std::vector<GroupEntry>> &groups, std::vector<std::vector<std::vector<Checkpoint>>> &ckpts,
+                               const std::vector<int> &group_of, const size_t *sizes, const int *max_waves, int waves_per_simd, int in_flight, bool group_order) {
     WorkList wl;
     const int n_images = (int)group_of.size(), nch = (int)plan.coded.size();
-    size_t total_tiles = 0, deepest = 0;
-    for (int i = 0; i < n_images; i++) total_tiles += groups[group_of[i]].size();
-    for (auto &g : groups) deepest = std::max(deepest, g.size());
-    const int wide_cfg = in_flight > 1 ? 0 : 2;
-    const bool dense = (int64_t)total_tiles > max_waves[wide_cfg];
-    wl.cfg = dense ? 1 : wide_cfg;
-    wl.n_waves = (int)std::max<int64_t>(1, std::min<int64_t>((int64_t)total_tiles, max_waves[wl.cfg]));
     std::vector<char> suspendable(groups.size(), 0);
     for (size_t gi = 0; gi < groups.size(); gi++) {
         const std::vector<GroupEntry> &g = groups[gi];
@@ -551,21 +559,68 @@
             ok = nonempty <= 1;
         }
         suspendable[gi] = ok ? 1 : 0;
-    }
+        if (!ok) for (auto &c : ckpts[gi]) c.clear();
+    }
+    std::vector<size_t> tiles_of(groups.size(), 0), ckpt_base(groups.size(), 0);
+    std::vector<std::vector<ChanSeg>> seg_of(groups.size());
+    for (size_t gi = 0; gi < groups.size(); gi++) {
+        const std::vector<GroupEntry> &g = groups[gi];
+        std::vector<ChanSeg> &cs = seg_of[gi];
+        cs.assign((size_t)std::max(nch, 1), ChanSeg{0, 1, 1, 0});
+        for (int c = 0; c < nch; c++) cs[c].seg_rows = (uint32_t)std::max(1, plan.coded[c].h);
+        ckpt_base[gi] = wl.ckpts.size();
+        for (size_t k = 0; k < g.size(); k++) {
+            tiles_of[gi] += 1 + ckpts[gi][k].size();
+            if (ckpts[gi][k].empty()) continue;
+            const int first = k == 0 ? 0 : g[k].first_channel, last = k + 1 < g.size() ? g[k + 1].first_channel - 1 : nch - 1;
+            for (int c = first; c <= last; c++)
+                if ((int64_t)plan.coded[c].w * plan.coded[c].h > 0) { cs[c].nseg = 1 + (uint32_t)ckpts[gi][k].size(); cs[c].seg_rows = ckpts[gi][k][0].y; }
+            wl.ckpts.insert(wl.ckpts.end(), ckpts[gi][k].begin(), ckpts[gi][k].end());
+        }
+        uint32_t word = 0;
+        for (int c = 0; c < nch; c++) { cs[c].word = word; word += cs[c].nseg; }
+        wl.prog_stride = std::max(wl.prog_stride, (int)word);
+    }
+    wl.chan_seg.resize((size_t)n_images * std::max(nch, 1));
+    for (int i = 0; i < n_images; i++) std::copy(seg_of[group_of[i]].begin(), seg_of[group_of[i]].end(), wl.chan_seg.begin() + (size_t)i * std::max(nch, 1));
+    size_t total_tiles = 0, deepest = 0;
+    for (int i = 0; i < n_images; i++) total_tiles += tiles_of[group_of[i]];
+    for (size_t gi = 0; gi < groups.size(); gi++) deepest = std::max(deepest, tiles_of[gi]);
+    const int wide_cfg = in_flight > 1 ? 0 : 2;
+    const bool dense = (int64_t)total_tiles > max_waves[wide_cfg];
+    wl.cfg = dense ? 1 : wide_cfg;
+    wl.n_waves = (int)std::max<int64_t>(1, std::min<int64_t>((int64_t)total_tiles, max_waves[wl.cfg]));
     int64_t image_samples = 0;
     for (int c = 0; c < nch; c++) image_samples += (int64_t)plan.coded[c].w * plan.coded[c].h;
-    auto push_tile = [&](int i, size_t k) {
-        const std::vector<GroupEntry> &g = groups[group_of[i]];
+    auto push_tile = [&](int i, size_t n) {
+        const size_t gi = (size_t)group_of[i];
+        const std::vector<GroupEntry> &g = groups[gi];
+        size_t k = 0, seg = n, ck0 = ckpt_base[gi];
+        while (k < g.size() && seg > ckpts[gi][k].size()) { seg -= 1 + ckpts[gi][k].size(); ck0 += ckpts[gi][k].size(); k++; }
         if (k >= g.size()) return;
+        const std::vector<Checkpoint> &ck = ckpts[gi][k];
         Tile t;
         t.image = (uint32_t)i;
         t.start = g[k].start;
         t.first_channel = k == 0 ? 0 : g[k].first_channel;
         t.last_channel = k + 1 < g.size() ? g[k + 1].first_channel - 1 : nch - 1;
-        t.end = k + 1 < g.size() ? g[k + 1].start : 0u;
-        t.flags = suspendable[group_of[i]] ? kTileSuspendable : 0u;
+        t.end = k + 1 < g.size() && seg == ck.size() ? g[k + 1].start : 0u;
+        t.flags = suspendable[gi] ? kTileSuspendable : 0u;
+        t.seg_chan = -1; t.y0 = 0; t.y1 = 0; t.ckpt = 0; t.ckpt_next = 0; t.word = 0;
+        int nonempty = 0, chan = -1;
+        for (int c = (int)t.first_channel; c <= (int)t.last_channel; c++) if ((int64_t)plan.coded[c].w * plan.coded[c].h > 0) { nonempty++; chan = c; }
         int64_t mine = 0;
         for (int c = (int)t.first_channel; c <= (int)t.last_channel; c++) mine += (int64_t)plan.coded[c].w * plan.coded[c].h;
+        if (nonempty == 1) {
+            const uint32_t h = (uint32_t)plan.coded[chan].h;
+            t.seg_chan = chan;
+            t.y0 = seg == 0 ? 0u : ck[seg - 1].y;
+            t.y1 = seg < ck.size() ? ck[seg].y : h;
+            t.ckpt = seg == 0 ? 0u : (uint32_t)(ck0 + seg - 1) + 1u;
+            t.ckpt_next = seg < ck.size() ? (uint32_t)(ck0 + seg) + 1u : 0u;
+            t.word = seg_of[gi][chan].word + (uint32_t)seg;
+            mine = (int64_t)plan.coded[chan].w * (int64_t)(t.y1 - t.y0);
+        }
         uint32_t cls = 15;
         if (mine > 0) { cls = 0; while (cls < 15 && (mine << (cls + 1)) <= image_samples) cls++; }
         t.flags |= cls << kTileSizeClassShift;
@@ -599,7 +654,7 @@
     qib[Q] = pos;
     for (int i = 0; i < n_images; i++) {
         itb[i] = (uint32_t)wl.tiles.size();
-        for (size_t k = 0; k < groups[group_of[i]].size(); k++) push_tile(i, k);
+        for (size_t k = 0; k < tiles_of[group_of[i]]; k++) push_tile(i, k);
     }
     itb[n_images] = (uint32_t)wl.tiles.size();
     return wl;
@@ -609,6 +664,7 @@
     OKCHK(grow(b->d_sched, b->sched_words, sched_layout(n_images, b->n_queues, b->sched ? b->n_tiles : 0)));
     OKCHK(grow(b->d_layout, b->layout_cap, layout_words));
     OKCHK(grow(b->d_tiles, b->tiles_cap, b->n_tiles));
+    OKCHK(grow(b->d_progress, b->progress_cap, (size_t)n_images * (size_t)b->prog_stride));
     if (b->sched && !b->share) {
         const size_t images_per_queue = ((size_t)n_images + b->n_queues - 1) / b->n_queues;
         size_t arena = ctx_arena_budget(b, images_per_queue * (size_t)b->n_queues);
@@ -630,12 +686,18 @@
     if (b->orphan) { g_last_error = "sibling batch: its primary has been destroyed"; return FUIFGPU_E_ARG; }
     hipStream_t st = (hipStream_t)stream;
     std::vector<std::vector<GroupEntry>> groups;
+    std::vector<std::vector<std::vector<Checkpoint>>> ckpts;
     std::vector<int> group_of;
-    OKCHK(stage_streams(b, blobs, sizes, n_images, preview, st, groups, group_of));
+    OKCHK(stage_streams(b, blobs, sizes, n_images, preview, st, groups, ckpts, group_of));
     const char *ord = getenv("FUIFGPU_TILE_ORDER");
-    const WorkList wl = plan_work_list(b->plan, groups, group_of, sizes, b->max_waves, b->waves_per_simd, b->in_flight, ord && !strcmp(ord, "group"));
+    const WorkList wl = plan_work_list(b->plan, groups, ckpts, group_of, sizes, b->max_waves, b->waves_per_simd, b->in_flight, ord && !strcmp(ord, "group"));
     b->cfg = wl.cfg; b->n_waves = wl.n_waves; b->sched = wl.sched; b->n_queues = wl.n_queues; b->n_tiles = (int)wl.tiles.size();
+    b->prog_stride = wl.prog_stride;
     OKCHK(reserve_launch_buffers(b, n_images, wl.layout.size()));
+    OKCHK(grow(b->d_chan_seg, b->chan_seg_cap, wl.chan_seg.size()));
+    OKCHK(grow(b->d_ckpts, b->ckpts_cap, std::max<size_t>(1, wl.ckpts.size())));
+    HIPCHK(hipMemcpyAsync(b->d_chan_seg, wl.chan_seg.data(), sizeof(ChanSeg) * wl.chan_seg.size(), hipMemcpyHostToDevice, st));
+    if (!wl.ckpts.empty()) HIPCHK(hipMemcpyAsync(b->d_ckpts, wl.ckpts.data(), sizeof(Checkpoint) * wl.ckpts.size(), hipMemcpyHostToDevice, st));
     if (!wl.layout.empty()) HIPCHK(hipMemcpyAsync(b->d_layout, wl.layout.data(), wl.layout.size() * 4, hipMemcpyHostToDevice, st));
     if (b->n_tiles) HIPCHK(hipMemcpyAsync(b->d_tiles, wl.tiles.data(), sizeof(Tile) * (size_t)b->n_tiles, hipMemcpyHostToDevice, st));
     HIPCHK(hipStreamSynchronize(st));
@@ -652,7 +714,7 @@
     hipStream_t st = (hipStream_t)stream;
     const int nch = (int)b->plan.coded.size();
     HIPCHK(hipMemsetAsync(b->d_meta, 0, sizeof(ChannelMeta) * (size_t)b->n_loaded * std::max(nch, 1), st));
-    HIPCHK(hipMemsetAsync(b->d_progress, 0, sizeof(uint32_t) * (size_t)b->n_loaded * std::max(nch, 1), st));
+    HIPCHK(hipMemsetAsync(b->d_progress, 0, sizeof(uint32_t) * (size_t)b->n_loaded * (size_t)std::max(b->prog_stride, 1), st));
     HIPCHK(hipMemsetAsync(b->d_group_start, 0, sizeof(uint32_t) * (size_t)b->n_loaded * std::max(nch, 1), st));
     HIPCHK(hipMemsetAsync(b->d_sched, 0, b->sched_words * 4, st));
     HIPCHK(hipMemsetAsync(b->d_status, 0, sizeof(int32_t) * b->n_loaded, st));
@@ -680,6 +742,7 @@
     P.ctx_scratch = r->d_ctx;
     P.ctx_units_per_queue = b->share ? ctx_units_per_queue(r->ctx_bytes, b->n_queues) : b->ctx_units_per_queue;
     P.progress = b->d_progress; P.group_start = b->d_group_start;
+    P.prog_stride = std::max(b->prog_stride, 1); P.chan_seg = b->d_chan_seg; P.ckpts = b->d_ckpts;
     HIPCHK(hipEventRecord(b->ev[0], st));
     launch_maniac_decode(P, b->n_waves, b->cfg, b->n_tiles > b->n_loaded ? 1 : 0, st);
     HIPCHK(hipGetLastError());
@@ -928,10 +991,6 @@
 int fuifgpu_batch_sched_stats(fuifgpu_batch *b, uint64_t *out8) {
     ON_BATCH_DEVICE(b);
     if (!b || !out8 || !b->d_sched) return FUIFGPU_E_ARG;
-#ifndef FUIF_STATS
-    g_last_error = "fuifgpu_batch_sched_stats: this build of libfuifgpu carries no scheduler statistics (build with -DFUIF_STATS)";
-    return FUIFGPU_E_UNSUPPORTED;
-#endif
     HIPCHK(hipDeviceSynchronize());
     HIPCHK(hipMemcpy(out8, (const uint8_t *)b->d_sched + offsetof(SchedHeader, sched_stats), sizeof(SchedHeader::sched_stats), hipMemcpyDeviceToHost));
     return FUIFGPU_OK;
diff --git a/fuif_amd/csrc/fuifgpu_internal.h b/fuif_amd/csrc/fuifgpu_internal.h
--- a/fuif_amd/csrc/fuifgpu_internal.h
+++ b/fuif_amd/csrc/fuifgpu_internal.h
@@ -56,6 +56,10 @@
     int32_t first_channel, last_channel;
     uint32_t end;
     uint32_t flags;
+    int32_t seg_chan;
+    uint32_t y0, y1;
+    uint32_t ckpt, ckpt_next;
+    uint32_t word;
 };
 constexpr uint32_t kTileSuspendable = 1u;
 constexpr uint32_t kTileSizeClassShift = 4;
@@ -146,8 +150,29 @@
     uint32_t start;
     int32_t first_channel;
 };
+struct Checkpoint {
+    uint32_t y, pos, range, low, cur_leaf;
+    uint32_t n_leaves, leaf_form;
+    uint32_t raw;
+};
+constexpr uint32_t kLeafFormCompact = 16, kLeafFormFull = 31;
+struct CheckpointData {
+    Checkpoint c;
+    std::vector<uint16_t> leaves;
+    std::vector<int16_t> rows;
+};
+struct ChanSeg {
+    uint32_t word, nseg, seg_rows, pad;
+};
 void build_index_trailer(const std::vector<GroupEntry> &groups, std::vector<uint8_t> &out);
-bool parse_index_trailer(const uint8_t *blob, size_t n, size_t data_start, int nch, std::vector<GroupEntry> &groups, size_t *stream_end);
+void build_index_trailer_v2(const std::vector<GroupEntry> &groups, const std::vector<std::vector<CheckpointData>> &ckpts, size_t stream_len, std::vector<uint8_t> &out);
+bool parse_index_trailer(const uint8_t *blob, size_t n, size_t data_start, int nch, std::vector<GroupEntry> &groups, size_t *stream_end,
+                         std::vector<std::vector<Checkpoint>> *ckpts = nullptr, const std::vector<ChannelGeom> *geom = nullptr);
+inline bool compact_leaves_rule(int minv, int maxv, int predictor) {
+    const int zero = minv > 0 ? minv : (maxv < 0 ? maxv : 0);
+    const int bound = predictor == 0 ? (maxv - zero > zero - minv ? maxv - zero : zero - minv) : maxv - minv;
+    return bound <= 255;
+}
 
 int parse_and_plan(const uint8_t *blob, size_t n, Plan &plan);
 void build_chance_table(uint16_t *table8192, uint32_t alpha, int cut);
diff --git a/fuif_amd/csrc/index.cpp b/fuif_amd/csrc/index.cpp
--- a/fuif_amd/csrc/index.cpp
+++ b/fuif_amd/csrc/index.cpp
@@ -44,8 +44,85 @@
     out.push_back('F'); out.push_back('G'); out.push_back('I'); out.push_back('X');
 }
 
-bool parse_index_trailer(const uint8_t *blob, size_t n, size_t data_start, int nch, std::vector<GroupEntry> &groups, size_t *stream_end) {
+void build_index_trailer_v2(const std::vector<GroupEntry> &groups, const std::vector<std::vector<CheckpointData>> &ckpts, size_t stream_len, std::vector<uint8_t> &out) {
+    bool any = false;
+    for (auto &c : ckpts) any = any || !c.empty();
+    if (!any || ckpts.size() != groups.size()) { build_index_trailer(groups, out); return; }
+    std::vector<uint8_t> payload;
+    put_varint(payload, 2);
+    put_varint(payload, groups.size());
+    uint32_t pc = 0, ps = 0;
+    for (const GroupEntry &g : groups) {
+        put_varint(payload, (uint32_t)g.first_channel - pc);
+        put_varint(payload, g.start - ps);
+        pc = (uint32_t)g.first_channel; ps = g.start;
+    }
+    for (size_t g = 0; g < groups.size(); g++) {
+        put_varint(payload, ckpts[g].size());
+        if (ckpts[g].empty()) continue;
+        put_varint(payload, ckpts[g][0].c.leaf_form);
+        put_varint(payload, ckpts[g][0].c.n_leaves);
+        for (const CheckpointData &cd : ckpts[g]) {
+            put_varint(payload, cd.c.y); put_varint(payload, cd.c.pos - groups[g].start); put_varint(payload, cd.c.range);
+            put_varint(payload, cd.c.low); put_varint(payload, cd.c.cur_leaf);
+            while ((stream_len + payload.size()) & 3u) payload.push_back(0);
+            for (uint16_t v : cd.leaves) { payload.push_back((uint8_t)(v & 255)); payload.push_back((uint8_t)(v >> 8)); }
+            for (int16_t v : cd.rows) { payload.push_back((uint8_t)((uint16_t)v & 255)); payload.push_back((uint8_t)((uint16_t)v >> 8)); }
+        }
+    }
+    out = payload;
+    const uint32_t len = (uint32_t)payload.size();
+    for (int k = 0; k < 4; k++) out.push_back((uint8_t)(len >> (8 * k)));
+    out.push_back('F'); out.push_back('G'); out.push_back('I'); out.push_back('X');
+}
+
+namespace {
+bool parse_checkpoints(const uint8_t *p, size_t len, size_t pos, size_t begin, const std::vector<GroupEntry> &groups, int nch,
+                       const std::vector<ChannelGeom> &geom, std::vector<std::vector<Checkpoint>> &ckpts) {
+    ckpts.assign(groups.size(), {});
+    for (size_t g = 0; g < groups.size(); g++) {
+        uint64_t n_ckpt = 0, form = 0, n_leaves = 0;
+        if (!get_varint(p, len, pos, n_ckpt)) return false;
+        if (n_ckpt == 0) continue;
+        if (!get_varint(p, len, pos, form) || !get_varint(p, len, pos, n_leaves)) return false;
+        if (form != kLeafFormCompact && form != kLeafFormFull) return false;
+        if (n_leaves < 1 || n_leaves > 32768) return false;
+        const int first = g == 0 ? 0 : groups[g].first_channel, last = g + 1 < groups.size() ? groups[g + 1].first_channel - 1 : nch - 1;
+        int chan = -1, nonempty = 0;
+        for (int c = first; c <= last; c++) if ((int64_t)geom[c].w * geom[c].h > 0) { nonempty++; chan = c; }
+        if (nonempty != 1) return false;
+        const uint64_t w = (uint64_t)geom[chan].w, h = (uint64_t)geom[chan].h;
+        const uint64_t g_begin = groups[g].start, g_end = g + 1 < groups.size() ? groups[g + 1].start : begin;
+        if (n_ckpt >= h) return false;
+        uint64_t y0 = 0;
+        for (uint64_t k = 0; k < n_ckpt; k++) {
+            uint64_t y = 0, dpos = 0, range = 0, low = 0, cur = 0;
+            if (!get_varint(p, len, pos, y) || !get_varint(p, len, pos, dpos) || !get_varint(p, len, pos, range) || !get_varint(p, len, pos, low) ||
+                !get_varint(p, len, pos, cur)) return false;
+            if (k == 0) y0 = y;
+            if (y < 2 || y >= h || y != (k + 1) * y0) return false;
+            if (dpos > g_end - g_begin || g_begin + dpos > g_end) return false;
+            if (range <= 0x10000u || range > (1u << 24) || low >= range || cur >= n_leaves) return false;
+            while ((begin + pos) & 3u) { if (pos >= len || p[pos] != 0) return false; pos++; }
+            const uint64_t raw_bytes = 2 * (n_leaves * form + 2 * w);
+            if (raw_bytes > len - pos) return false;
+            for (uint64_t i = 0; i < n_leaves * form; i++) {
+                const uint32_t v = (uint32_t)p[pos + 2 * i] | ((uint32_t)p[pos + 2 * i + 1] << 8);
+                if (v < 1 || v > 4095) return false;
+            }
+            ckpts[g].push_back(Checkpoint{(uint32_t)y, (uint32_t)(g_begin + dpos), (uint32_t)range, (uint32_t)low, (uint32_t)cur,
+                                          (uint32_t)n_leaves, (uint32_t)form, (uint32_t)(begin + pos)});
+            pos += raw_bytes;
+        }
+    }
+    return pos == len;
+}
+}
+
+bool parse_index_trailer(const uint8_t *blob, size_t n, size_t data_start, int nch, std::vector<GroupEntry> &groups, size_t *stream_end,
+                         std::vector<std::vector<Checkpoint>> *ckpts, const std::vector<ChannelGeom> *geom) {
     groups.clear();
+    if (ckpts) ckpts->clear();
     if (n < 8 + 3 || memcmp(blob + n - 4, "FGIX", 4) != 0) return false;
     uint32_t len = 0;
     for (int k = 0; k < 4; k++) len |= (uint32_t)blob[n - 8 + k] << (8 * k);
@@ -54,7 +131,7 @@
     const uint8_t *p = blob + begin;
     size_t pos = 0;
     uint64_t version = 0, count = 0;
-    if (!get_varint(p, len, pos, version) || version != 1) return false;
+    if (!get_varint(p, len, pos, version) || (version != 1 && version != 2)) return false;
     if (!get_varint(p, len, pos, count) || count < 1 || count > (uint64_t)nch) return false;
     uint64_t c = 0, s = 0;
     for (uint64_t g = 0; g < count; g++) {
@@ -66,7 +143,9 @@
         if (c >= (uint64_t)nch || s >= begin) return false;
         groups.push_back(GroupEntry{(uint32_t)s, (int32_t)c});
     }
-    if (pos != len || groups[0].start != data_start) { groups.clear(); return false; }
+    if ((version == 1 && pos != len) || groups[0].start != data_start) { groups.clear(); return false; }
+    if (version == 2 && ckpts && geom && (int)geom->size() == nch && !parse_checkpoints(p, len, pos, begin, groups, nch, *geom, *ckpts)) ckpts->clear();
+    if (ckpts && ckpts->size() != groups.size()) ckpts->assign(groups.size(), {});
     if (stream_end) *stream_end = begin;
     return true;
 }
@@ -89,6 +168,23 @@
     for (int g = 0; g < (int)groups.size() && g < cap; g++) {
         if (first_channel) first_channel[g] = groups[g].first_channel;
         if (start) start[g] = groups[g].start;
+    }
+    return FUIFGPU_OK;
+}
+
+int fuifgpu_index_checkpoints(const uint8_t *blob, size_t size, int32_t *first_row, int32_t *n_checkpoints, int cap, int *n_groups) {
+    if (!blob || !n_groups) return FUIFGPU_E_ARG;
+    *n_groups = 0;
+    Plan plan;
+    int r = parse_and_plan(blob, size, plan);
+    if (r != FUIFGPU_OK) return r;
+    std::vector<GroupEntry> groups;
+    std::vector<std::vector<Checkpoint>> ckpts;
+    if (!parse_index_trailer(blob, size, plan.data_start, (int)plan.coded.size(), groups, nullptr, &ckpts, &plan.coded)) return FUIFGPU_OK;
+    *n_groups = (int)groups.size();
+    for (int g = 0; g < (int)groups.size() && g < cap; g++) {
+        if (n_checkpoints) n_checkpoints[g] = (int32_t)ckpts[g].size();
+        if (first_row) first_row[g] = ckpts[g].empty() ? 0 : (int32_t)ckpts[g][0].y;
     }
     return FUIFGPU_OK;
 }
diff --git a/fuif_amd/csrc/maniac_decode.h b/fuif_amd/csrc/maniac_decode.h
--- a/fuif_amd/csrc/maniac_decode.h
+++ b/fuif_amd/csrc/maniac_decode.h
@@ -63,6 +63,9 @@
     unsigned long long *sched_stats;
     uint32_t *simd_claim;
     uint32_t *progress;
+    int32_t prog_stride;
+    const ChanSeg *chan_seg;
+    const Checkpoint *ckpts;
     uint32_t *group_start;
     uint8_t *scratch;
     size_t scratch_stride, bfs_off, leaves_off, stack_off, queue_off, subtree_off;
diff --git a/fuif_amd/csrc/maniac_decode.hip b/fuif_amd/csrc/maniac_decode.hip
--- a/fuif_amd/csrc/maniac_decode.hip
+++ b/fuif_amd/csrc/maniac_decode.hip
@@ -743,7 +743,7 @@
                         const uint32_t pin = ld_agent(&r->pin);
                         if ((pin == 0u || pin == my_pin) && !(simd_full && (ld_agent(&r->flags) & kRecLong))) {
                             const uint32_t wc = ld_agent(&r->wait_chan), wv = ld_agent(&r->wait_val);
-                            run = ld_agent(&P.progress[(size_t)im * nch + wc]) >= wv;
+                            run = ld_agent(&P.progress[(size_t)im * (size_t)P.prog_stride + wc]) >= wv;
                         }
                     }
                 }
@@ -849,7 +849,13 @@
 
     coef_t *coef = P.coef + (int64_t)img * P.coef_stride;
     ChannelMeta *meta = P.meta + (int64_t)img * P.n_channels;
-    uint32_t *progress = P.progress + (size_t)img * nch;
+    uint32_t *progress = P.progress + (size_t)img * (size_t)P.prog_stride;
+    auto tile_u32 = [&](size_t byte_off) -> uint32_t {
+        return rflu(ld_agent(reinterpret_cast<const uint32_t *>(reinterpret_cast<const char *>(P.tiles + tix) + byte_off)));
+    };
+#define TILE_FIELD(f) tile_u32(offsetof(Tile, f))
+    auto chan_seg_of = [&](int c) -> const ChanSeg * { return P.chan_seg + ((size_t)img * (size_t)nch + (size_t)c); };
+    auto word_of = [&](int c) -> uint32_t { return (int)TILE_FIELD(seg_chan) == c ? TILE_FIELD(word) : rflu(ld_agent(&chan_seg_of(c)->word)); };
     int status = 0;
     bool stalled = false;
     TileRec *const rec = sched ? P.tile_rec + tix : nullptr;
@@ -892,18 +898,20 @@
 #endif
     auto publish = [&](int c, uint32_t v) {
         if (kHandOff) {
+            const uint32_t wd = word_of(c);
             drain_stores();
             if (lane == 0) {
-                st_agent(progress + c, v);
+                st_agent(progress + wd, v);
                 if ((v & 31u) == 0u) atomicAdd(P.heartbeat, 1u);
             }
         }
     };
     auto wait_header = [&](int c) {
         uint32_t spins = 0;
-        if (!stalled && rflu(ld_agent(progress + c)) == 0u) {
+        const uint32_t *hw = progress + rflu(ld_agent(&chan_seg_of(c)->word));
+        if (!stalled && rflu(ld_agent(hw)) == 0u) {
             STATS(const unsigned long long w0 = realtime();)
-            while (!stalled && rflu(ld_agent(progress + c)) == 0u) spin_nap(spins);
+            while (!stalled && rflu(ld_agent(hw)) == 0u) spin_nap(spins);
             STATS(waited += realtime() - w0;)
         }
     };
@@ -966,7 +974,7 @@
         __syncthreads();
         if (fatal) { status |= ST_UNSUPPORTED | ST_CORRUPT; break; }
         if (early) continue;
-        if (firstrealc > endc) { ci = endc; continue; }
+        if (firstrealc > endc) { if (TILE_FIELD(ckpt) | TILE_FIELD(ckpt_next)) status |= ST_CORRUPT; ci = endc; continue; }
         }
 
         int nrefs = 0;
@@ -1058,6 +1066,7 @@
 
         rac_init(rac, s, lane);
 
+        if (!compress && (TILE_FIELD(ckpt) | TILE_FIELD(ckpt_next))) { status |= ST_CORRUPT; break; }
         if (!compress) {
             for (int i = beginc; i <= endc; i++) {
                 const int gw = rfl(geom[i].w), gh = rfl(geom[i].h);
@@ -1306,6 +1315,28 @@
             for (int64_t i = words + lane; i < (int64_t)nleaves * words; i += 64) lw[i] = mine;
             __syncthreads();
         }
+        if (const uint32_t seg_ckpt = TILE_FIELD(ckpt)) {
+            const int seg_chan = (int)TILE_FIELD(seg_chan), seg_y0 = (int)TILE_FIELD(y0);
+            const Checkpoint ck = P.ckpts[seg_ckpt - 1u];
+            const uint32_t form = compact ? kLeafFormCompact : kLeafFormFull, n_ch = (uint32_t)nleaves * form;
+            const uint32_t ck_range = rflu(ck.range), ck_low = rflu(ck.low), ck_raw = rflu(ck.raw), ck_leaf = rflu(ck.cur_leaf);
+            const int pw = seg_chan >= 0 ? rfl(geom[seg_chan].w) : 0;
+            const bool fits = seg_chan >= beginc && seg_chan <= endc && rflu(ck.n_leaves) == (uint32_t)nleaves && rflu(ck.leaf_form) == form && ck_leaf < (uint32_t)nleaves &&
+                              ck_range > 0x10000u && ck_range <= (1u << 24) && ck_low < ck_range && rflu(ck.y) == (uint32_t)seg_y0 && seg_y0 >= 2 &&
+                              (uint64_t)ck_raw + 2ull * ((uint64_t)n_ch + 2ull * (uint64_t)pw) <= (uint64_t)s.size && (ck_raw & 1u) == 0u;
+            if (!fits) { status |= ST_CORRUPT; break; }
+            const uint16_t *src = reinterpret_cast<const uint16_t *>(s.p + ck_raw);
+            const uint32_t lstride = compact ? 16u : 32u;
+            for (uint32_t k = (uint32_t)lane; k < n_ch; k += 64u) {
+                const uint32_t l = k / form, v = (uint32_t)src[k] & 0xFFFu;
+                leaves[(size_t)l * lstride + (k - l * form)] = (uint16_t)(v ? v : 1u);
+            }
+            const int16_t *rsrc = reinterpret_cast<const int16_t *>(src + n_ch);
+            coef_t *pl = coef + geom[seg_chan].coef_off + (int64_t)(seg_y0 - 2) * pw;
+            for (int x = lane; x < 2 * pw; x += 64) st_plane<kHandOff>(pl + x, (int)rsrc[x]);
+            rac.range = ck_range; rac.low = ck_low; s.pos = rflu(ck.pos); cur_leaf = (int)ck_leaf;
+            __syncthreads();
+        }
         }
         const uint2 root_nd = narrow ? uint2{0u, 0u} : snodes_g[lane];
         const uint32_t root_w = narrow ? reinterpret_cast<const uint32_t *>(snodes_g)[lane] : 0u;
@@ -1330,13 +1361,15 @@
         };
 
         for (int i = beginc; i <= endc; i++) {
-            const int w = rfl(geom[i].w), h = rfl(geom[i].h);
+            const int w = rfl(geom[i].w);
+            const bool seg_here = (int)TILE_FIELD(seg_chan) == i;
+            const int h = seg_here && (int)TILE_FIELD(y1) < rfl(geom[i].h) ? (int)TILE_FIELD(y1) : rfl(geom[i].h);
             const int ghs = rfl(geom[i].hshift), gvs = rfl(geom[i].vshift);
             const int minv = rfl(ld_agent(&meta[i].minval)), maxv = rfl(ld_agent(&meta[i].maxval));
             if (minv == maxv) continue;
             coef_t *plane = coef + geom[i].coef_off;
             const int zero = minv > 0 ? minv : (maxv < 0 ? maxv : 0);
-            int y = resumed ? (int)resume_y : 0;
+            int y = resumed ? (int)resume_y : (seg_here ? (int)TILE_FIELD(y0) : 0);
             uint32_t ref_seen = 0;
             if (tree_size == 1 && predictor == 0 && zero == 0) {
                 for (; y < h; y++) {
@@ -1365,22 +1398,25 @@
                         if (s_limit_hit(s)) break;
                         __syncthreads();
                         if (kHandOff && nrefs) {
-                            uint32_t need = 0;
+                            uint32_t need = 0, fin_v = 0, fw = 0;
                             const uint32_t *fp = progress;
                             if (lane < nrefs) {
                                 const RefChan rc = sh.refs[lane];
                                 int ry = (y << gvs) >> rc.vshift; if (ry >= rc.h) ry = rc.h - 1;
                                 need = (uint32_t)ry + 2u;
-                                fp = progress + rc.chan;
+                                const ChanSeg cs = *chan_seg_of(rc.chan);
+                                uint32_t sg = (uint32_t)ry / cs.seg_rows; if (sg >= cs.nseg) sg = cs.nseg - 1u;
+                                fw = cs.word + sg;
+                                fin_v = sg + 1u < cs.nseg ? (sg + 1u) * cs.seg_rows + 1u : (uint32_t)rc.h + 1u;
+                                fp = progress + fw;
                             }
                             uint32_t spins = 0;
                             if (__any(ref_seen < need)) {
                                 if (ref_seen < need) ref_seen = ld_agent(fp);
                                 if (__any(ref_seen < need) && can_yield) {
                                     const int bl = __builtin_ctzll(__ballot(ref_seen < need));
-                                    const RefChan rcb = sh.refs[bl];
-                                    const uint32_t nb = (uint32_t)rdlane((int)need, bl) + P.yield_slack, fin = (uint32_t)rfl(rcb.h) + 1u;
-                                    yield_chan = (uint32_t)rfl(rcb.chan); yield_val = nb < fin ? nb : fin;
+                                    const uint32_t nb = (uint32_t)rdlane((int)need, bl) + P.yield_slack, fin = (uint32_t)rdlane((int)fin_v, bl);
+                                    yield_chan = (uint32_t)rdlane((int)fw, bl); yield_val = nb < fin ? nb : fin;
                                     resume_y = (uint32_t)y;
                                     EMU_COUNT(3);
                                     yielded = true;
@@ -1611,6 +1647,10 @@
             if (y < h) { __syncthreads(); fill_plane<kHandOff>(plane, (int64_t)y * w, (int64_t)(h - y) * w, rfl(geom[i].ctor_data) ? 0 : zero, lane); status |= ST_TRUNCATED; }
             if (lane == 0) st_agent(&meta[i].decoded, 1);
             publish(i, (uint32_t)h + 1u);
+            if ((int)TILE_FIELD(seg_chan) == i && TILE_FIELD(ckpt_next) != 0u && !(status & (ST_TRUNCATED | ST_CORRUPT)) && !s_limit_hit(s)) {
+                const Checkpoint nk = P.ckpts[TILE_FIELD(ckpt_next) - 1u];
+                if (rac.range != rflu(nk.range) || rac.low != rflu(nk.low) || s.pos != rflu(nk.pos) || (uint32_t)cur_leaf != rflu(nk.cur_leaf)) status |= ST_CORRUPT;
+            }
             if (s_limit_hit(s)) break;
         }
         if (yielded) {
@@ -1623,6 +1663,9 @@
                 rec->ctx = (uint32_t)ctx_slot; rec->ctx_leaves = ctx_leaves_units; rec->tree_size = (uint32_t)tree_size; rec->n_super = (uint32_t)n_super; rec->cur_leaf = (uint32_t)cur_leaf;
                 rec->pin = ctx_slot >= 0 ? 0u : my_pin;
                 rec->owner = simd_key + 1u;
+#ifndef FUIF_STATS
+                atomicAdd(&P.sched_stats[2], 1ull);
+#endif
             }
             drain_stores();
             if (lane == 0) st_agent(&rec->state, (uint32_t)TS_READY);
@@ -1646,9 +1689,13 @@
     __syncthreads();
     for (int c = first_c; c <= last_c; c++) {
         const int gw = rfl(geom[c].w), gh = rfl(geom[c].h);
-        const uint32_t done = (uint32_t)gh + 1u;
-        if (!kHandOff || rflu(ld_agent(progress + c)) != done) {
-            if ((int64_t)gw * gh > 0 && rfl(ld_agent(&meta[c].decoded)) == 0) fill_plane<kHandOff>(coef + geom[c].coef_off, 0, (int64_t)gw * gh, 0, lane);
+        const int seg_y0 = (int)TILE_FIELD(y0), seg_y1 = (int)TILE_FIELD(y1);
+        const bool part = c == (int)TILE_FIELD(seg_chan) && (seg_y0 > 0 || seg_y1 < gh);
+        const int r0 = part ? (seg_y0 < gh ? seg_y0 : gh) : 0, r1 = part && seg_y1 < gh ? seg_y1 : gh;
+        const uint32_t done = (uint32_t)r1 + 1u;
+        if (!kHandOff || rflu(ld_agent(progress + word_of(c))) != done) {
+            if ((int64_t)gw * gh > 0 && (part || rfl(ld_agent(&meta[c].decoded)) == 0)) fill_plane<kHandOff>(coef + geom[c].coef_off, (int64_t)r0 * gw, (int64_t)(r1 - r0) * gw, 0, lane);
+            if (part && lane == 0) st_agent(&meta[c].decoded, 1);
             publish(c, done);
         }
     }
@@ -1685,6 +1732,7 @@
     if (lane == 0 && P.prof) for (int k = 0; k < 8; k++) atomicAdd(&P.prof[(size_t)PROF_ROW * 8 + k], prof_acc[k]);
 #endif
     __syncthreads();
+#undef TILE_FIELD
     }
 #ifdef FUIF_STATS
     if (sched && lane == 0 && P.sched_stats) {
diff --git a/fuif_amd/csrc/writer.cpp b/fuif_amd/csrc/writer.cpp
--- a/fuif_amd/csrc/writer.cpp
+++ b/fuif_amd/csrc/writer.cpp
@@ -1,4 +1,5 @@
 #include <algorithm>
+#include <atomic>
 #include <cmath>
 #include <cstdlib>
 #include <cstring>
@@ -645,7 +646,29 @@
     return rc;
 }
 
-size_t encode_group(Bytes &io, Image &img, int ci, int predictor, bool compress, const GroupCoder &gc, size_t &header_pos, EncJob *defer = nullptr) {
+std::atomic<long long> g_segment_samples{-1};
+long long segment_samples() {
+    long long v = g_segment_samples.load();
+    if (v < 0) { const char *e = getenv("FUIFGPU_SEGMENT_SAMPLES"); v = e ? atoll(e) : 0; }
+    return v;
+}
+std::atomic<int> g_checkpoint_percent{-1};
+int checkpoint_percent() {
+    int v = g_checkpoint_percent.load();
+    if (v < 0) { const char *e = getenv("FUIFGPU_CHECKPOINT_PERCENT"); v = e ? atoi(e) : 5; }
+    return std::max(0, v);
+}
+int seg_rows_for(int h, int nseg) { return std::max(2, (h + nseg - 1) / nseg); }
+struct Snap {
+    int y = 0, last_leaf = 0;
+    uint32_t range = 0, low = 0;
+    size_t epos = 0;
+    std::vector<uint16_t> leaves;
+};
+
+size_t encode_group(Bytes &io, Image &img, int ci, int predictor, bool compress, const GroupCoder &gc, size_t &header_pos, EncJob *defer = nullptr,
+                    std::vector<CheckpointData> *ckpts = nullptr) {
+    if (ckpts) ckpts->clear();
     Chan &c = img.ch[ci];
     io.varint((size_t)((0 << 4) + (predictor << 1) + (compress ? 1 : 0)));
     if (c.minval <= 0) io.varint((size_t)(1 - c.minval));
@@ -737,18 +760,82 @@
             rac.range = st.range; rac.low = st.low; rac.delayed = st.delayed; rac.pending = st.pending;
         }
         if (rc != FUIFGPU_OK && gc.gpu_rc && *gc.gpu_rc == FUIFGPU_OK) *gc.gpu_rc = rc;
-    } else if (tree.size() == 1 && predictor == 0 && c.zero == 0) {
-        for (int32_t v : c.data) write_symbol(rac, leaves.data(), gc.pixel_table, c.minval, c.maxval, v);
     } else {
-        for (int y = 0; y < c.h; y++)
+        const bool fast_track = tree.size() == 1 && predictor == 0 && c.zero == 0;
+        std::vector<int> cand;
+        std::vector<char> want((size_t)c.h, 0);
+        const long long seg_samples = ckpts ? segment_samples() : 0;
+        if (seg_samples > 0 && c.h >= 4) {
+            const long long policy = std::min<long long>(((long long)c.w * c.h + seg_samples - 1) / seg_samples, c.h / 2);
+            for (long long n = 2; n <= policy; n++) if (n <= 16 || n == policy) cand.push_back((int)n);
+            for (int n : cand) { const int sr = seg_rows_for(c.h, n); for (int y = sr; y < c.h; y += sr) want[(size_t)y] = 1; }
+        }
+        std::vector<Snap> snaps;
+        int last_leaf = 0;
+        for (int y = 0; y < c.h; y++) {
+            if (!cand.empty() && want[(size_t)y]) {
+                Snap sn;
+                sn.y = y; sn.last_leaf = last_leaf; sn.range = rac.range; sn.low = rac.low;
+                sn.epos = io.b.size() + (rac.delayed >= 0 ? 1 : 0) + (size_t)rac.pending;
+                sn.leaves = leaves;
+                snaps.push_back(std::move(sn));
+            }
+            if (fast_track) {
+                for (int x = 0; x < c.w; x++) write_symbol(rac, leaves.data(), gc.pixel_table, c.minval, c.maxval, c.data[(size_t)y * c.w + x]);
+                continue;
+            }
             for (int x = 0; x < c.w; x++) {
                 int guess = props_and_guess(props.data(), c, refs, x, y, predictor);
                 int mn = c.minval - guess, mx = c.maxval - guess;
                 if (mn == mx) continue;
                 int pos = 0;
                 while (tree[pos].prop >= 0) pos = (props[tree[pos].prop] > tree[pos].split) ? tree[pos].child : tree[pos].child + 1;
+                last_leaf = tree[pos].leaf;
                 write_symbol(rac, &leaves[(size_t)tree[pos].leaf * CH_N], gc.pixel_table, mn, mx, c.data[(size_t)y * c.w + x] - guess);
             }
+        }
+        rac.flush();
+        if (!snaps.empty()) {
+            const bool compact = compact_leaves_rule(c.minval, c.maxval, predictor);
+            const uint32_t form = compact ? kLeafFormCompact : kLeafFormFull;
+            const size_t per_ckpt = 2 * ((size_t)nleaves * form + 2 * (size_t)c.w) + 16, body = io.b.size() - header_pos;
+            int nseg = 1;
+            for (int n : cand) {
+                const int sr = seg_rows_for(c.h, n), count = (c.h - 1) / sr;
+                if ((size_t)count * per_ckpt * 100 <= body * (size_t)checkpoint_percent()) nseg = n;
+            }
+            if (nseg > 1) {
+                std::vector<int> order((size_t)nleaves, 0), stack{0};
+                int next_leaf = 0;
+                while (!stack.empty()) {
+                    const int pos = stack.back(); stack.pop_back();
+                    if (tree[pos].prop < 0) order[(size_t)tree[pos].leaf] = next_leaf++;
+                    else { stack.push_back(tree[pos].child + 1); stack.push_back(tree[pos].child); }
+                }
+                const int sr = seg_rows_for(c.h, nseg);
+                for (const Snap &sn : snaps) {
+                    if (sn.y % sr) continue;
+                    CheckpointData cd;
+                    const uint32_t window = ((uint32_t)io.b[sn.epos] << 16) | ((uint32_t)io.b[sn.epos + 1] << 8) | (uint32_t)io.b[sn.epos + 2];
+                    cd.c.y = (uint32_t)sn.y; cd.c.pos = (uint32_t)(sn.epos + 3); cd.c.range = sn.range;
+                    cd.c.low = (window - sn.low) & 0xFFFFFFu;
+                    cd.c.cur_leaf = (uint32_t)order[(size_t)sn.last_leaf]; cd.c.n_leaves = (uint32_t)nleaves; cd.c.leaf_form = form; cd.c.raw = 0;
+                    if (cd.c.low >= cd.c.range) { ckpts->clear(); break; }
+                    cd.leaves.resize((size_t)nleaves * form);
+                    for (int l = 0; l < nleaves; l++) {
+                        const uint16_t *src = &sn.leaves[(size_t)l * CH_N];
+                        uint16_t *dst = &cd.leaves[(size_t)order[(size_t)l] * form];
+                        if (compact) { for (int k = 0; k < 9; k++) dst[k] = src[k]; for (int k = 0; k < 7; k++) dst[9 + k] = src[CH_MANT + k]; }
+                        else for (int k = 0; k < CH_N; k++) dst[k] = src[k];
+                    }
+                    cd.rows.resize(2 * (size_t)c.w);
+                    for (int r = 0; r < 2; r++)
+                        for (int x = 0; x < c.w; x++) cd.rows[(size_t)r * c.w + x] = (int16_t)c.data[(size_t)(sn.y - 2 + r) * c.w + x];
+                    ckpts->push_back(std::move(cd));
+                }
+            }
+        }
+        return io.b.size() - header_pos;
     }
     rac.flush();
     return io.b.size() - header_pos;
@@ -827,6 +914,15 @@
 extern "C" {
 
 void fuifgpu_free_blob(uint8_t *p) { free(p); }
+
+int fuifgpu_set_segment_samples(long long samples) {
+    g_segment_samples.store(samples < 0 ? -1 : samples);
+    return FUIFGPU_OK;
+}
+int fuifgpu_set_checkpoint_percent(int percent) {
+    g_checkpoint_percent.store(percent < 0 ? -1 : percent);
+    return FUIFGPU_OK;
+}
 
 static bool read_encode_options(const fuifgpu_encode_options *opt, fuifgpu_encode_options &o, int gpu_entropy_default) {
     memset(&o, 0, sizeof(o));
@@ -1013,7 +1109,8 @@
 void note_responsive(const Image &img, int i, size_t after, int responsive[5]) {
     for (int s = 0; s < 5; s++) if (img.downscales[s] == i) responsive[s] = (int)after;
 }
-int finish_stream(Bytes &head, const Bytes &io, int responsive[5], std::vector<GroupEntry> &group_at, bool emit_index, uint8_t **blob_out, size_t *size_out) {
+int finish_stream(Bytes &head, const Bytes &io, int responsive[5], std::vector<GroupEntry> &group_at, bool emit_index, uint8_t **blob_out, size_t *size_out,
+                  std::vector<std::vector<CheckpointData>> *ckpts_at = nullptr) {
     int rel = 0;
     for (int s = 0; s < 5; s++) {
         if (responsive[s] < 0) responsive[s] = (int)io.b.size();
@@ -1023,7 +1120,10 @@
     std::vector<uint8_t> trailer;
     if (emit_index && !group_at.empty()) {
         for (GroupEntry &g : group_at) g.start += (uint32_t)head.b.size();
-        build_index_trailer(group_at, trailer);
+        if (ckpts_at && ckpts_at->size() == group_at.size()) {
+            for (auto &g : *ckpts_at) for (CheckpointData &cd : g) cd.c.pos += (uint32_t)head.b.size();
+            build_index_trailer_v2(group_at, *ckpts_at, head.b.size() + io.b.size(), trailer);
+        } else build_index_trailer(group_at, trailer);
     }
     const size_t total = head.b.size() + io.b.size() + trailer.size();
     uint8_t *blob = (uint8_t *)malloc(total ? total : 1);
@@ -1057,6 +1157,7 @@
     begin_stream(img, nch, bit_depth, o, head, io);
     int responsive[5] = {-1, -1, -1, -1, -1};
     std::vector<GroupEntry> group_at;
+    std::vector<std::vector<CheckpointData>> ckpts_at;
     const int n = (int)img.ch.size();
     for (int i = 0; i < n; i++) {
         Chan &c = img.ch[i];
@@ -1065,17 +1166,19 @@
         size_t header_pos = 0;
         size_t before = io.b.size();
         group_at.push_back(GroupEntry{(uint32_t)before, i});
-        size_t body = encode_group(io, img, i, predictor, true, gc, header_pos);
+        ckpts_at.emplace_back();
+        size_t body = encode_group(io, img, i, predictor, true, gc, header_pos, nullptr, o.emit_index != 0 && !gc.gpu_entropy ? &ckpts_at.back() : nullptr);
         float bits = body * 8.0f, pixels = (float)c.w * c.h, ubits = 0.0f;
         if (c.maxval > c.minval) ubits = pixels * (ilog2u((uint32_t)(c.maxval - c.minval)) + 1) + 16;
         if (bits >= ubits) {
             io.b.resize(before);
+            ckpts_at.back().clear();
             encode_group(io, img, i, predictor, false, gc, header_pos);
         }
         note_responsive(img, i, io.b.size(), responsive);
     }
     if (gpu_rc != FUIFGPU_OK) return gpu_rc;
-    return finish_stream(head, io, responsive, group_at, o.emit_index != 0, blob_out, size_out);
+    return finish_stream(head, io, responsive, group_at, o.emit_index != 0, blob_out, size_out, &ckpts_at);
 }
 
 
diff --git a/include/fuifgpu.h b/include/fuifgpu.h
--- a/include/fuifgpu.h
+++ b/include/fuifgpu.h
@@ -87,6 +87,7 @@
 int fuifgpu_batch_sched_stats(fuifgpu_batch *batch, uint64_t *out8);
 
 int fuifgpu_index_parse(const uint8_t *blob, size_t size, int32_t *first_channel, uint32_t *start, int cap, int *n_groups);
+int fuifgpu_index_checkpoints(const uint8_t *blob, size_t size, int32_t *first_row, int32_t *n_checkpoints, int cap, int *n_groups);
 int fuifgpu_index_append(const uint8_t *blob, size_t size, const int32_t *first_channel, const uint32_t *start, int n_groups,
                          uint8_t **blob_out, size_t *size_out);
 int fuifgpu_batch_group_index(fuifgpu_batch *batch, int image, int32_t *first_channel, uint32_t *start, int cap, int *n_groups);
@@ -175,6 +176,8 @@
                             const int32_t *transforms, int n_transform_words, const fuifgpu_encode_options *opt,
                             uint8_t **blob_out, size_t *size_out);
 void fuifgpu_free_blob(uint8_t *blob);
+int fuifgpu_set_segment_samples(long long samples);
+int fuifgpu_set_checkpoint_percent(int percent);
 
 #ifdef __cplusplus
 }
```

Result: slower. 1251 Mpixels/s (-14.2%).
